# WangWen-Believer/DR-SLAM

Hardware: AMD Instinct MI355X
Metric: RGB-D frames/sec (extract+match) at 640x480 (higher is better)
Workload: dtype u8; 1 GPU; 640x480 synthetic RGB-D (TUM3 intrinsics), ORB extract 1000/1.2/8/20/7 + SearchByProjection(frame k, frame k-1, th=15) on consecutive frames; BASELINE config 2; batch_per_gpu=512, batches_in_flight_per_gpu=3, distinct_resident_input_batches_per_gpu=3, sequence_frames_per_rank=64

## Files before the change

dr_slam_amd/csrc/capi_match.cpp:

```cpp
#include "drfe_internal.h"
#include "match_internal.h"
#include "stage_layout.h"
#include "../../include/drfe_math.h"

#include <algorithm>
#include <cmath>
#include <cstdlib>
#include <cstring>
#include <new>
#include <thread>

template <class T>
static hipError_t dalloc(T** p, size_t n)
{
    *p = nullptr;
    return hipMalloc((void**)p, std::max<size_t>(n, 1) * sizeof(T));
}

void drfe_match_buffers_free(drfe_ctx* c)
{
    MatchBuffers* m = c->mb;
    if (!m) return;
    void* ptrs[] = {m->d_pairs, m->d_queries, m->d_mps, m->d_scale, m->d_candIdx, m->d_candKey, m->d_candCnt, m->d_candBest,
                    m->d_hist, m->d_initObs, m->d_bfIdx, m->d_bfDist, m->d_bfQ, m->d_bfT};
// ... 62 lines not shown
{
    std::memcpy(P->T, Tcw, 64);
    for (int i = 0; i < 3; i++) {
        double s = 0;
        for (int k = 0; k < 3; k++) s += (double)Tcw[k * 4 + i] * (double)Tcw[k * 4 + 3];
        P->Ow[i] = (float)(s * -1.0);
    }
    P->bf = cam->bf;
    P->logScale = drfe_logf(c->cfg.scale_factor);
    P->nLevels = c->cfg.nlevels;
    P->limit = limit;
}

static hipError_t call_scratch(drfe_ctx* c, size_t bytes, uint8_t** out)
{
    if (bytes > c->callScratchBytes) {
        if (c->d_callScratch) (void)hipFree(c->d_callScratch);
        c->d_callScratch = nullptr; c->callScratchBytes = 0;
        const size_t want = (bytes + (bytes >> 1) + 65535) & ~(size_t)65535;
        const hipError_t e = hipMalloc((void**)&c->d_callScratch, want);
        if (e != hipSuccess) return e;
        c->callScratchBytes = want;
    }
    *out = c->d_callScratch;
    return hipSuccess;
}

static void camera_centre_kf(const float* Tcw, float Ow[3])
{
    for (int i = 0; i < 3; i++) {
        const float d = Tcw[0 * 4 + i] * Tcw[3] + Tcw[1 * 4 + i] * Tcw[7] + Tcw[2 * 4 + i] * Tcw[11];
        Ow[i] = (float)((double)d * -1.0);
    }
}

template <class In, class Out, class Launch>
static int frustum_run(drfe_ctx* c, const In* in, int n, Out* out, Launch launch)
{
    if (n == 0) return DRFE_OK;
    HIPCHK(c, hipSetDevice(c->device));
    uint8_t* d = nullptr;
    StageLayout<64> lay;
    const auto sIn = lay.add<In>(n);
    const auto sOut = lay.add<Out>(n);
    HIPCHK(c, call_scratch(c, lay.bytes(), &d));
    hipStream_t s = c->stream;
    hipError_t e = hipMemcpyAsync(sIn.at(d), in, sIn.bytes(), hipMemcpyHostToDevice, s);
    if (e == hipSuccess) e = hipMemcpyAsync(sOut.at(d), out, sOut.bytes(), hipMemcpyHostToDevice, s);
    if (e == hipSuccess) e = launch(sIn.at(d), sOut.at(d), s);
    if (e == hipSuccess) e = hipMemcpyAsync(out, sOut.at(d), sOut.bytes(), hipMemcpyDeviceToHost, s);
    if (e == hipSuccess) e = hipStreamSynchronize(s);
    if (e != hipSuccess) { c->err = std::string("is_in_frustum: ") + hipGetErrorString(e); return DRFE_ERR_HIP; }
    return DRFE_OK;
}


extern "C" {

int drfe_frame_stereo_grid_batch(drfe_ctx* c, const uint16_t* d_depth, size_t frame_stride, size_t row_stride,
                                 const drfe_camera* cam, int nframes, void* stream)
{
    if (!c || !d_depth || !cam) return DRFE_ERR_INVALID;
    if (nframes < 1 || nframes > c->lastBatch) { c->err = "glue: extract the batch first"; return DRFE_ERR_STATE; }
    if (!(cam->max_x > cam->min_x) || !(cam->max_y > cam->min_y)) { c->err = "glue: empty image bounds"; return DRFE_ERR_INVALID; }
    if (row_stride < (size_t)c->geom.imgW || frame_stride < row_stride * (size_t)c->geom.imgH) { c->err = "glue: depth row / frame stride smaller than the image"; return DRFE_ERR_INVALID; }
    HIPCHK(c, hipSetDevice(c->device));
    hipStream_t s = stream ? (hipStream_t)stream : c->stream;
    HIPCHK(c, drfe_launch_glue(c, d_depth, frame_stride, row_stride, *cam, nframes, s));
    c->glueValid = true;
    c->cam = *cam;
    return DRFE_OK;
}

int drfe_frame_set_distortion(drfe_ctx* c, const drfe_camera* cam, const float* dist, int n)
{
    if (!c || (n > 0 && (!dist || !cam)) || n < 0 || n > 5) return DRFE_ERR_INVALID;
    HIPCHK(c, hipSetDevice(c->device));
    int rc = drfe_stream_sync(c);
    if (rc != DRFE_OK) return rc;
    std::memset(&c->dist, 0, sizeof(c->dist));
    c->glueValid = false;
    if (n == 0 || dist[0] == 0.0f) return DRFE_OK;
    if (n < 4) { c->err = "set_distortion: need k1, k2, p1, p2[, k3]"; return DRFE_ERR_INVALID; }
    if (!c->d_kpsUn) {
        void* p = nullptr;
        HIPCHK(c, hipMalloc(&p, sizeof(drfe_keypoint) * (size_t)c->cfg.max_batch * c->maxKp));
        c->d_kpsUn = (drfe_keypoint*)p;
    }
    c->dist.fx = cam->fx; c->dist.fy = cam->fy; c->dist.cx = cam->cx; c->dist.cy = cam->cy;
    for (int i = 0; i < n; i++) c->dist.k[i] = (double)dist[i];
    c->dist.enabled = 1;
    return DRFE_OK;
}

int drfe_frame_image_bounds(const drfe_camera* cam, const float* dist, int n, int cols, int rows, float* bounds)
{
    if (!cam || !bounds || n < 0 || n > 5 || (n > 0 && !dist)) return DRFE_ERR_INVALID;
    if (n >= 4 && dist[0] != 0.0f) {
        DrfeDistortion D;
        std::memset(&D, 0, sizeof(D));
        D.fx = cam->fx; D.fy = cam->fy; D.cx = cam->cx; D.cy = cam->cy; D.enabled = 1;
        for (int i = 0; i < n; i++) D.k[i] = (double)dist[i];
        const float cx[4] = {0.f, (float)cols, 0.f, (float)cols}, cy[4] = {0.f, 0.f, (float)rows, (float)rows};
        float ux[4], uy[4];
        for (int i = 0; i < 4; i++) drfe_undistort_point(D, cx[i], cy[i], &ux[i], &uy[i]);
        bounds[0] = std::min(ux[0], ux[2]); bounds[1] = std::max(ux[1], ux[3]);
        bounds[2] = std::min(uy[0], uy[1]); bounds[3] = std::max(uy[2], uy[3]);
    } else {
        bounds[0] = 0.f; bounds[1] = (float)cols; bounds[2] = 0.f; bounds[3] = (float)rows;
    }
    return DRFE_OK;
}

int drfe_frame_download_keys_un(drfe_ctx* c, int slot, drfe_keypoint* kps, int cap)
{
    if (!c || !kps) return DRFE_ERR_INVALID;
    if (slot < 0 || slot >= c->lastBatch || !c->glueValid) { c->err = "download_keys_un: run the glue first"; return DRFE_ERR_STATE; }
    HIPCHK(c, hipSetDevice(c->device));
    int rc = drfe_stream_sync(c);
    if (rc != DRFE_OK) return rc;
    int n = 0;
    HIPCHK(c, hipMemcpy(&n, c->d_kpCount + slot, sizeof(int), hipMemcpyDeviceToHost));
    if (n > cap) { c->err = "keypoint buffer too small"; return DRFE_ERR_CAPACITY; }
    if (n) HIPCHK(c, hipMemcpy(kps, drfe_kps_un(c) + (size_t)slot * c->maxKp, sizeof(drfe_keypoint) * n, hipMemcpyDeviceToHost));
    return DRFE_OK;
}


int drfe_orb_keypoint_pixels_async(drfe_ctx* c, int nframes, uint32_t* uv, int32_t* counts, void* stream)
{
    if (!c || !uv || !counts) return DRFE_ERR_INVALID;
    if (nframes < 1 || nframes > c->lastBatch) { c->err = "keypoint_pixels: extract the batch first"; return DRFE_ERR_STATE; }
    HIPCHK(c, hipSetDevice(c->device));
    if (!c->d_kpUV) HIPCHK(c, hipMalloc((void**)&c->d_kpUV, sizeof(uint32_t) * (size_t)c->cfg.max_batch * c->maxKp));
    hipStream_t s = stream ? (hipStream_t)stream : c->stream;
    HIPCHK(c, drfe_launch_kp_pixels(c, nframes, c->d_kpUV, s));
    HIPCHK(c, hipMemcpyAsync(uv, c->d_kpUV, sizeof(uint32_t) * (size_t)nframes * c->maxKp, hipMemcpyDeviceToHost, s));
    HIPCHK(c, hipMemcpyAsync(counts, c->d_kpCount, sizeof(int) * (size_t)nframes, hipMemcpyDeviceToHost, s));
    return DRFE_OK;
}

int drfe_gather_keypoint_depth(const uint16_t* depth, size_t frame_stride, size_t row_stride, int nframes, const uint32_t* uv,
                               const int32_t* counts, int max_kp, uint16_t* out, int n_threads)
{
    if (!depth || !uv || !counts || !out || nframes < 0 || max_kp < 1) return DRFE_ERR_INVALID;
    int T = n_threads > 0 ? n_threads : drfe_default_host_threads();
    T = std::max(1, std::min(T, nframes));
    auto work = [&](int f0, int f1) {
        for (int f = f0; f < f1; f++) {
            const uint16_t* img = depth + (size_t)f * frame_stride;
            const uint32_t* p = uv + (size_t)f * max_kp;
            uint16_t* o = out + (size_t)f * max_kp;
            const int n = std::min(counts[f], max_kp);
            const int ahead = 16;
            for (int i = 0; i < std::min(ahead, n); i++)
                if (p[i] != 0xFFFFFFFFu) __builtin_prefetch(&img[(size_t)(p[i] >> 16) * row_stride + (p[i] & 0xFFFFu)]);
            for (int i = 0; i < n; i++) {
                if (i + ahead < n && p[i + ahead] != 0xFFFFFFFFu)
                    __builtin_prefetch(&img[(size_t)(p[i + ahead] >> 16) * row_stride + (p[i + ahead] & 0xFFFFu)]);
                o[i] = p[i] == 0xFFFFFFFFu ? (uint16_t)0 : img[(size_t)(p[i] >> 16) * row_stride + (p[i] & 0xFFFFu)];
            }
        }
    };
    if (T == 1) { work(0, nframes); return DRFE_OK; }
    std::vector<std::thread> th;
    for (int k = 0; k < T; k++) th.emplace_back(work, (int)((int64_t)nframes * k / T), (int)((int64_t)nframes * (k + 1) / T));
    for (std::thread& t : th) t.join();
    return DRFE_OK;
}

int drfe_frame_stereo_grid_batch_kpdepth(drfe_ctx* c, const uint16_t* kp_depth, int kp_depth_on_host, const drfe_camera* cam,
                                         int nframes, void* stream)
{
    if (!c || !kp_depth || !cam) return DRFE_ERR_INVALID;
    if (nframes < 1 || nframes > c->lastBatch) { c->err = "glue: extract the batch first"; return DRFE_ERR_STATE; }
    if (!(cam->max_x > cam->min_x) || !(cam->max_y > cam->min_y)) { c->err = "glue: empty image bounds"; return DRFE_ERR_INVALID; }
    HIPCHK(c, hipSetDevice(c->device));
    hipStream_t s = stream ? (hipStream_t)stream : c->stream;
    const uint16_t* d = kp_depth;
    if (kp_depth_on_host) {
        if (!c->d_kpDepth) HIPCHK(c, hipMalloc((void**)&c->d_kpDepth, sizeof(uint16_t) * (size_t)c->cfg.max_batch * c->maxKp));
        HIPCHK(c, hipMemcpyAsync(c->d_kpDepth, kp_depth, sizeof(uint16_t) * (size_t)nframes * c->maxKp, hipMemcpyHostToDevice, s));
        d = c->d_kpDepth;
    }
    HIPCHK(c, drfe_launch_glue(c, d, (size_t)c->maxKp, 0, *cam, nframes, s));
    c->glueValid = true;
    c->cam = *cam;
    return DRFE_OK;
}

int drfe_frame_load(drfe_ctx* c, int slot, const drfe_keypoint* kps, const drfe_keypoint* kps_un, const uint8_t* desc, const float* u_right,
                    const float* depth_m, int n, const drfe_camera* cam)
{
    if (!c) return DRFE_ERR_INVALID;
    if (slot < 0 || slot >= c->cfg.max_batch || n < 0 || n > c->maxKp || !cam || (n > 0 && (!kps || !desc))) {
        c->err = "drfe_frame_load: invalid argument (slot, keypoint count beyond drfe_orb_max_keypoints, or a missing array)";
        return DRFE_ERR_INVALID;
    }
    if (!(cam->max_x > cam->min_x) || !(cam->max_y > cam->min_y)) { c->err = "drfe_frame_load: empty image bounds"; return DRFE_ERR_INVALID; }
    HIPCHK(c, hipSetDevice(c->device));
    int rc = drfe_stream_sync(c);
    if (rc != DRFE_OK) return rc;
    const size_t K = (size_t)c->maxKp, o = (size_t)slot * K;
    hipStream_t s = c->stream;
    if (n > 0) {
        if (c->dist.enabled) {
            HIPCHK(c, hipMemcpyAsync(c->d_kps + o, kps, sizeof(drfe_keypoint) * (size_t)n, hipMemcpyHostToDevice, s));
            HIPCHK(c, hipMemcpyAsync(c->d_kpsUn + o, kps_un ? kps_un : kps, sizeof(drfe_keypoint) * (size_t)n, hipMemcpyHostToDevice, s));
        } else
            HIPCHK(c, hipMemcpyAsync(c->d_kps + o, kps_un ? kps_un : kps, sizeof(drfe_keypoint) * (size_t)n, hipMemcpyHostToDevice, s));
        HIPCHK(c, hipMemcpyAsync(c->d_desc + o * 32, desc, (size_t)n * 32, hipMemcpyHostToDevice, s));
        if (u_right) HIPCHK(c, hipMemcpyAsync(c->d_uRight + o, u_right, (size_t)n * 4, hipMemcpyHostToDevice, s));
        else HIPCHK(c, drfe_launch_fill_i32(reinterpret_cast<int*>(c->d_uRight + o), n, (int)0xBF800000u , s));
        if (depth_m) HIPCHK(c, hipMemcpyAsync(c->d_depth + o, depth_m, (size_t)n * 4, hipMemcpyHostToDevice, s));
        else HIPCHK(c, drfe_launch_fill_i32(reinterpret_cast<int*>(c->d_depth + o), n, (int)0xBF800000u, s));
    }
    HIPCHK(c, hipMemcpyAsync(c->d_kpCount + slot, &n, sizeof(int), hipMemcpyHostToDevice, s));
    {
        SlotShift shift(c, slot);
        HIPCHK(c, drfe_launch_grid(c, *cam, 1, s));
    }
    HIPCHK(c, hipStreamSynchronize(s));
    c->lastBatch = std::max(c->lastBatch, slot + 1);
    c->glueValid = true;
    c->cam = *cam;
    if (c->bow) drfe_bow_slot_invalidate(c, slot);
    return DRFE_OK;
}

int drfe_frame_download_stereo(drfe_ctx* c, int slot, float* u_right, float* depth, int cap)
{
    if (!c || slot < 0 || slot >= c->lastBatch || !c->glueValid) return c ? DRFE_ERR_STATE : DRFE_ERR_INVALID;
    int rc = drfe_stream_sync(c);
    if (rc != DRFE_OK) return rc;
    int n = 0;
    HIPCHK(c, hipMemcpy(&n, c->d_kpCount + slot, sizeof(int), hipMemcpyDeviceToHost));
    if (n > cap) return DRFE_ERR_CAPACITY;
    if (n && u_right) HIPCHK(c, hipMemcpy(u_right, c->d_uRight + (size_t)slot * c->maxKp, sizeof(float) * n, hipMemcpyDeviceToHost));
    if (n && depth) HIPCHK(c, hipMemcpy(depth, c->d_depth + (size_t)slot * c->maxKp, sizeof(float) * n, hipMemcpyDeviceToHost));
    return DRFE_OK;
}

int drfe_frame_download_grid(drfe_ctx* c, int slot, int32_t* offsets, int32_t* indices, int cap)
{
    if (!c || !offsets || slot < 0 || slot >= c->lastBatch || !c->glueValid) return c ? DRFE_ERR_STATE : DRFE_ERR_INVALID;
    int rc = drfe_stream_sync(c);
    if (rc != DRFE_OK) return rc;
    HIPCHK(c, hipMemcpy(offsets, c->d_gridOff + (size_t)slot * (DRFE_GRID_CELLS + 1), sizeof(int) * (DRFE_GRID_CELLS + 1),
                        hipMemcpyDeviceToHost));
    const int n = offsets[DRFE_GRID_CELLS];
    if (n > cap) return DRFE_ERR_CAPACITY;
    if (n && indices) HIPCHK(c, hipMemcpy(indices, c->d_gridIdx + (size_t)slot * c->maxKp, sizeof(int) * n, hipMemcpyDeviceToHost));
    return DRFE_OK;
}

}

int drfe_match_consecutive_stage(drfe_ctx* c, const float* Tcw, const float* Twc, const drfe_camera* cam, int mono, int nframes, hipStream_t s)
{
    MatchBuffers* m = drfe_match_buffers(c);
    if (!m) return DRFE_ERR_HIP;
    const int np = nframes - 1;
    const size_t pairBytes = sizeof(MatchPair) * (size_t)c->cfg.max_batch, poseBytes = sizeof(float) * 16 * (size_t)c->cfg.max_batch;
    if (!m->h_stage[0]) {
        m->stageBytes = pairBytes + poseBytes;
        for (int k = 0; k < 2; k++) {
            HIPCHK(c, hipHostMalloc(&m->h_stage[k], m->stageBytes, hipHostMallocDefault));
            HIPCHK(c, hipEventCreateWithFlags(&m->stageEv[k], hipEventDisableTiming));
            HIPCHK(c, hipEventRecord(m->stageEv[k], s));
        }
    }
    const int slotK = m->stageNext;
    m->stageNext ^= 1;
    HIPCHK(c, hipEventSynchronize(m->stageEv[slotK]));
    MatchPair* pairs = static_cast<MatchPair*>(m->h_stage[slotK]);
    float* poses = reinterpret_cast<float*>(static_cast<uint8_t*>(m->h_stage[slotK]) + pairBytes);
    std::memcpy(poses, Twc, sizeof(float) * 16 * (size_t)nframes);
    const float mb = cam->bf / cam->fx;
    for (int p = 0; p < np; p++) {
        MatchPair& P = pairs[p];
        P.curSlot = p + 1; P.lastSlot = p; P.mpSlot = p; P.nQueries = 0;
        P.queryBase = p * c->maxKp;
        P.mpBase = p * c->maxKp;
        std::memcpy(P.Tcw, Tcw + (size_t)(p + 1) * 16, sizeof(float) * 16);
        drfe_motion_flags(Tcw + (size_t)(p + 1) * 16, Tcw + (size_t)p * 16, mb, mono, &P.forward, &P.backward);
    }
    HIPCHK(c, hipMemcpyAsync(m->d_pairs, pairs, sizeof(MatchPair) * np, hipMemcpyHostToDevice, s));
    HIPCHK(c, hipMemcpyAsync(c->d_poses, poses, sizeof(float) * 16 * nframes, hipMemcpyHostToDevice, s));
    HIPCHK(c, hipEventRecord(m->stageEv[slotK], s));
    return DRFE_OK;
}

hipError_t drfe_match_consecutive_enqueue(drfe_ctx* c, const drfe_camera* cam, float th, int check_ori, int nframes, hipStream_t s)
{
    MatchBuffers* m = drfe_match_buffers(c);
    if (!m) return hipErrorOutOfMemory;
    hipError_t e = hipMemsetAsync(c->d_match, 0xFF, sizeof(int) * (size_t)nframes * c->maxKp, s);
    if (e == hipSuccess) e = hipMemsetAsync(c->d_matchCount, 0, sizeof(int) * nframes, s);
    if (e == hipSuccess) e = drfe_launch_mappoints_last(c, *m, *cam, c->d_poses, nframes, s);
    if (e == hipSuccess) e = drfe_launch_window_match(c, *m, *cam, nframes - 1, c->maxKp, 0, th, 0.f, check_ori, nullptr, s, 2);
    return e;
}

extern "C" {

int drfe_match_consecutive_batch(drfe_ctx* c, const float* Tcw, const float* Twc, const drfe_camera* cam, float th,
                                 int mono, int check_ori, int nframes, void* stream)
{
    if (!c || !Tcw || !Twc || !cam) return DRFE_ERR_INVALID;
    if (nframes < 2 || nframes > c->lastBatch || !c->glueValid) {
        c->err = "match: needs an extracted batch of >= 2 frames with stereo/grid computed";
        return DRFE_ERR_STATE;
    }
    if (c->maxKp > DRFE_MATCH_LAST_MAX_QUERIES) {
        c->err = "match: the slot size (drfe_orb_max_keypoints = " + std::to_string(c->maxKp) +
                 ") exceeds the 4096 map points the consecutive matcher resolves per pair";
        return DRFE_ERR_CAPACITY;
    }
    HIPCHK(c, hipSetDevice(c->device));
    hipStream_t s = stream ? (hipStream_t)stream : c->stream;
    const int rc = drfe_match_consecutive_stage(c, Tcw, Twc, cam, mono, nframes, s);
    if (rc != DRFE_OK) return rc;
    if (c->profile) { (void)hipEventRecord(c->ev[DRFE_STAGE_MATCH][0], s); c->evUsed[DRFE_STAGE_MATCH] = true; }
    HIPCHK(c, drfe_match_consecutive_enqueue(c, cam, th, check_ori, nframes, s));
    if (c->profile) (void)hipEventRecord(c->ev[DRFE_STAGE_MATCH][1], s);
    return DRFE_OK;
}

int drfe_match_download(drfe_ctx* c, int slot, int32_t* cur_to_last, int cap, int* nmatches)
{
    if (!c || slot < 0 || slot >= c->lastBatch) return c ? DRFE_ERR_STATE : DRFE_ERR_INVALID;
    int rc = drfe_stream_sync(c);
    if (rc != DRFE_OK) return rc;
    rc = match_status(c, 2);
    if (rc != DRFE_OK) return rc;
    int n = 0;
    HIPCHK(c, hipMemcpy(&n, c->d_kpCount + slot, sizeof(int), hipMemcpyDeviceToHost));
    if (n > cap) return DRFE_ERR_CAPACITY;
    if (n && cur_to_last)
        HIPCHK(c, hipMemcpy(cur_to_last, c->d_match + (size_t)slot * c->maxKp, sizeof(int) * n, hipMemcpyDeviceToHost));
    if (nmatches) HIPCHK(c, hipMemcpy(nmatches, c->d_matchCount + slot, sizeof(int), hipMemcpyDeviceToHost));
    return DRFE_OK;
}

int drfe_search_by_projection_last(drfe_ctx* c, int cur_slot, int last_slot, const float* Tcw_cur, const float* Tcw_last,
                                   const drfe_camera* cam, const drfe_map_point* last_mp, int n_last, float th, int mono,
                                   int check_ori, const uint8_t* cur_obs, int32_t* cur_mp, int n_cur, int* nmatches)
{
    if (!c || !Tcw_cur || !Tcw_last || !cam || !last_mp || !cur_mp || !nmatches) return DRFE_ERR_INVALID;
    if (cur_slot < 0 || cur_slot >= c->lastBatch || last_slot < 0 || last_slot >= c->lastBatch || !c->glueValid) {
        c->err = "search_by_projection_last: slots not ready";
        return DRFE_ERR_STATE;
    }
    HIPCHK(c, hipSetDevice(c->device));
    int rc = drfe_stream_sync(c);
    if (rc != DRFE_OK) return rc;
    int counts[2];
    HIPCHK(c, hipMemcpy(&counts[0], c->d_kpCount + cur_slot, sizeof(int), hipMemcpyDeviceToHost));
    HIPCHK(c, hipMemcpy(&counts[1], c->d_kpCount + last_slot, sizeof(int), hipMemcpyDeviceToHost));
    if (n_cur != counts[0] || n_last != counts[1]) { c->err = "search_by_projection_last: N mismatch"; return DRFE_ERR_INVALID; }
    if (n_last > DRFE_MATCH_LAST_MAX_QUERIES) {
        c->err = "search_by_projection_last: more than 4096 map points in the last frame";
        return DRFE_ERR_CAPACITY;
    }
    MatchBuffers* m = drfe_match_buffers(c);
    if (!m) return DRFE_ERR_HIP;
    MatchPair P;
    P.curSlot = cur_slot; P.lastSlot = last_slot; P.mpSlot = -1; P.nQueries = n_last; P.queryBase = 0; P.mpBase = 0;
    std::memcpy(P.Tcw, Tcw_cur, sizeof(float) * 16);
    drfe_motion_flags(Tcw_cur, Tcw_last, cam->bf / cam->fx, mono, &P.forward, &P.backward);
    hipStream_t s = c->stream;
    HIPCHK(c, hipMemcpy(m->d_pairs, &P, sizeof(P), hipMemcpyHostToDevice));
    if (n_last) HIPCHK(c, hipMemcpy(m->d_mps, last_mp, sizeof(drfe_map_point) * n_last, hipMemcpyHostToDevice));
    if (n_cur) HIPCHK(c, hipMemcpy(c->d_match + (size_t)cur_slot * c->maxKp, cur_mp, sizeof(int) * n_cur, hipMemcpyHostToDevice));
    const uint8_t* d_obs = nullptr;
    if (cur_obs && n_cur) {
        HIPCHK(c, hipMemcpy(m->d_initObs, cur_obs, n_cur, hipMemcpyHostToDevice));
        d_obs = m->d_initObs;
    }
    *nmatches = 0;
    if (n_last == 0 || n_cur == 0) return DRFE_OK;
    HIPCHK(c, drfe_launch_window_match(c, *m, *cam, 1, n_last, 0, th, 0.f, check_ori, d_obs, s));
    HIPCHK(c, hipStreamSynchronize(s));
    rc = match_status(c);
    if (rc != DRFE_OK) return rc;
    HIPCHK(c, hipMemcpy(cur_mp, c->d_match + (size_t)cur_slot * c->maxKp, sizeof(int) * n_cur, hipMemcpyDeviceToHost));
    HIPCHK(c, hipMemcpy(nmatches, c->d_matchCount + cur_slot, sizeof(int), hipMemcpyDeviceToHost));
    return DRFE_OK;
}

int drfe_search_by_projection_map(drfe_ctx* c, int slot, const drfe_tracked_point* mps, int mcount, float th,
                                  float nnratio, const uint8_t* claim_obs, int32_t* frame_mp, int n, int* nmatches)
{
    if (!c || !mps || !frame_mp || !nmatches || mcount < 0) return DRFE_ERR_INVALID;
    if (slot < 0 || slot >= c->lastBatch || !c->glueValid) { c->err = "search_by_projection_map: slot not ready"; return DRFE_ERR_STATE; }
    HIPCHK(c, hipSetDevice(c->device));
    int rc = drfe_stream_sync(c);
    if (rc != DRFE_OK) return rc;
    int cnt = 0;
    HIPCHK(c, hipMemcpy(&cnt, c->d_kpCount + slot, sizeof(int), hipMemcpyDeviceToHost));
    if (n != cnt) { c->err = "search_by_projection_map: N mismatch"; return DRFE_ERR_INVALID; }
    MatchBuffers* m = drfe_match_buffers(c);
    if (!m) return DRFE_ERR_HIP;
    if ((size_t)mcount > m->queryCap) { c->err = "search_by_projection_map: too many map points for the scratch"; return DRFE_ERR_CAPACITY; }
    *nmatches = 0;
    if (mcount == 0 || n == 0) return DRFE_OK;
    std::vector<MatchQuery> q(mcount);
    const bool bFactor = th != 1.0;
    for (int i = 0; i < mcount; i++) {
        const drfe_tracked_point& t = mps[i];
        MatchQuery& Q = q[i];
        std::memset(&Q, 0, sizeof(Q));
        Q.valid = (t.track_in_view && !t.bad) ? 1 : 0;
        if (Q.valid && (t.level < 0 || t.level >= c->cfg.nlevels)) { c->err = "tracked point level out of range"; return DRFE_ERR_INVALID; }
        float r = ((double)t.view_cos > 0.998) ? 2.5f : 4.0f;
        if (bFactor) r *= th;
        const float rs = Q.valid ? r * c->scale[t.level] : 0.f;
        Q.u = t.proj_x; Q.v = t.proj_y; Q.radius = rs; Q.ur = t.proj_xr; Q.thrR = rs;
        Q.minLevel = t.level - 1; Q.maxLevel = t.level;
        Q.obs = t.obs_positive;
        std::memcpy(Q.desc, t.desc, 32);
    }
    MatchPair P;
    std::memset(&P, 0, sizeof(P));
    P.curSlot = slot; P.lastSlot = slot; P.mpSlot = -1; P.nQueries = mcount; P.queryBase = 0; P.mpBase = 0;
    const drfe_camera cam = c->cam;
    hipStream_t s = c->stream;
    HIPCHK(c, hipMemcpy(m->d_pairs, &P, sizeof(P), hipMemcpyHostToDevice));
    HIPCHK(c, hipMemcpy(m->d_queries, q.data(), sizeof(MatchQuery) * mcount, hipMemcpyHostToDevice));
    HIPCHK(c, hipMemcpy(c->d_match + (size_t)slot * c->maxKp, frame_mp, sizeof(int) * n, hipMemcpyHostToDevice));
    const uint8_t* d_obs = nullptr;
    if (claim_obs) {
        HIPCHK(c, hipMemcpy(m->d_initObs, claim_obs, n, hipMemcpyHostToDevice));
        d_obs = m->d_initObs;
    }
    HIPCHK(c, drfe_launch_window_match(c, *m, cam, 1, mcount, 1, th, nnratio, 0, d_obs, s));
    HIPCHK(c, hipStreamSynchronize(s));
    rc = match_status(c);
    if (rc != DRFE_OK) return rc;
    HIPCHK(c, hipMemcpy(frame_mp, c->d_match + (size_t)slot * c->maxKp, sizeof(int) * n, hipMemcpyDeviceToHost));
    HIPCHK(c, hipMemcpy(nmatches, c->d_matchCount + slot, sizeof(int), hipMemcpyDeviceToHost));
    return DRFE_OK;
}

int drfe_match_orb_points(drfe_ctx* c, int cur_slot, int last_slot, const int32_t* last_mp, const uint8_t* last_outlier,
                          int n_last, int32_t* cur_mp, int n_cur, int* n_pairs)
{
    if (!c || !last_mp || !last_outlier || !cur_mp || !n_pairs) return DRFE_ERR_INVALID;
    if (cur_slot < 0 || cur_slot >= c->lastBatch || last_slot < 0 || last_slot >= c->lastBatch) {
        c->err = "match_orb_points: slots not ready";
        return DRFE_ERR_STATE;
    }
    HIPCHK(c, hipSetDevice(c->device));
    int rc = drfe_stream_sync(c);
    if (rc != DRFE_OK) return rc;
    int counts[2];
    HIPCHK(c, hipMemcpy(&counts[0], c->d_kpCount + cur_slot, sizeof(int), hipMemcpyDeviceToHost));
    HIPCHK(c, hipMemcpy(&counts[1], c->d_kpCount + last_slot, sizeof(int), hipMemcpyDeviceToHost));
    if (n_cur != counts[0] || n_last != counts[1]) { c->err = "match_orb_points: N mismatch"; return DRFE_ERR_INVALID; }
    *n_pairs = 0;
    if (n_cur == 0 || n_last == 0) return DRFE_OK;
    MatchBuffers* m = drfe_match_buffers(c);
    if (!m) return DRFE_ERR_HIP;
    hipStream_t s = c->stream;
    HIPCHK(c, drfe_launch_bf_knn(c->d_desc + (size_t)cur_slot * c->maxKp * 32, n_cur,
                                 c->d_desc + (size_t)last_slot * c->maxKp * 32, n_last, 1, m->d_bfIdx, m->d_bfDist, s));
    std::vector<int32_t> idx(n_cur), dist(n_cur);
    HIPCHK(c, hipMemcpyAsync(idx.data(), m->d_bfIdx, sizeof(int) * n_cur, hipMemcpyDeviceToHost, s));
    HIPCHK(c, hipMemcpyAsync(dist.data(), m->d_bfDist, sizeof(int) * n_cur, hipMemcpyDeviceToHost, s));
    HIPCHK(c, hipStreamSynchronize(s));
    double min_dist = 1000;
    for (int i = 0; i < n_cur; i++)
        if ((float)dist[i] < min_dist) min_dist = (float)dist[i];
    int npair = 0;
    for (int i = 0; i < n_cur; i++) {
        if (!((float)dist[i] < std::max(2 * min_dist, 15.0))) continue;
        const int mp = last_mp[idx[i]];
        if (mp >= 0 && npair < n_last && !last_outlier[npair]) cur_mp[i] = mp;
        npair++;
    }
    *n_pairs = npair;
    return DRFE_OK;
}

static void line_mad(const int32_t* dist, int nq, double* nnMad, double* nn12Mad)
{
    std::vector<float> d0(nq), gap(nq), s(nq);
    for (int i = 0; i < nq; i++) { d0[i] = (float)dist[2 * i]; gap[i] = (float)dist[2 * i + 1] - (float)dist[2 * i]; }
    s = d0;
    std::nth_element(s.begin(), s.begin() + nq / 2, s.end());
    const double med = s[nq / 2];
    for (int i = 0; i < nq; i++) s[i] = std::fabs((float)(d0[i] - med));
    std::nth_element(s.begin(), s.begin() + nq / 2, s.end());
    *nnMad = 1.4826 * s[nq / 2];
    s = gap;
    std::nth_element(s.begin(), s.begin() + nq / 2, s.end(), [](float a, float b) { return a > b; });
    const double med12 = s[nq / 2];
    for (int i = 0; i < nq; i++) s[i] = std::fabs((float)(gap[i] - med12));
    std::nth_element(s.begin(), s.begin() + nq / 2, s.end());
    *nn12Mad = 1.4826 * s[nq / 2];
}

int drfe_lsd_search_by_descriptor(drfe_ctx* c, const uint8_t* desc_q, int n_q, const uint8_t* desc_t, int n_t,
                                  const uint8_t* has_line, int mode, int32_t* out, int* nmatches)
{
    if (!c || !desc_q || !desc_t || !out || !nmatches || n_q < 0 || n_t < 0 || mode < 0 || mode > 1) return DRFE_ERR_INVALID;
    *nmatches = 0;
    const int n_out = mode == 0 ? n_t : n_q;
    for (int i = 0; i < n_out; i++) out[i] = -1;
    if (n_q == 0 || n_t < 2) return DRFE_OK;
    std::vector<int32_t> idx((size_t)n_q * 2), dist((size_t)n_q * 2);
    int rc = drfe_match_bf_knn(c, desc_q, n_q, desc_t, n_t, 2, idx.data(), dist.data());
    if (rc != DRFE_OK) return rc;
    double nnTh, nn12Th;
    line_mad(dist.data(), n_q, &nnTh, &nn12Th);
    int n = 0;
    if (mode == 0) {
        const float minRatio = 1.0f / 1.5f;
        for (int q = 0; q < n_q; q++) {
            const double r = (float)dist[2 * q] / (float)dist[2 * q + 1];
            if (r < minRatio && (!has_line || has_line[q])) { out[idx[2 * q]] = q; n++; }
        }
    } else {
        const double th = nn12Th * 0.5;
        for (int q = 0; q < n_q; q++) {
            const double gap = (float)dist[2 * q + 1] - (float)dist[2 * q];
            if (gap > th && (!has_line || has_line[idx[2 * q]])) { out[q] = idx[2 * q]; n++; }
        }
    }
    *nmatches = n;
    return DRFE_OK;
}

int drfe_lsd_search_for_triangulation(drfe_ctx* c, const uint8_t* desc1, int n1, const uint8_t* desc2, int n2,
                                      const uint8_t* has1, const uint8_t* has2, int32_t* out12, int* nmatches)
{
    if (!c || !desc1 || !desc2 || !has1 || !has2 || !out12 || !nmatches || n1 < 0 || n2 < 0) return DRFE_ERR_INVALID;
    *nmatches = 0;
    for (int i = 0; i < n1; i++) out12[i] = -1;
    if (n1 == 0 || n2 < 2) return DRFE_OK;
    std::vector<int32_t> idx((size_t)n1 * 2), dist((size_t)n1 * 2);
    int rc = drfe_match_bf_knn(c, desc1, n1, desc2, n2, 2, idx.data(), dist.data());
    if (rc != DRFE_OK) return rc;
    double nnTh, nn12Th;
    line_mad(dist.data(), n1, &nnTh, &nn12Th);
    const double th = nn12Th * 0.1;
    int n = 0;
    for (int q = 0; q < n1; q++) {
        const int t = idx[2 * q];
        if (has1[q] || has2[t]) continue;
        const double gap = (float)dist[2 * q + 1] - (float)dist[2 * q];
        if (gap > th) { out12[q] = t; n++; }
    }
    *nmatches = n;
    return DRFE_OK;
}

int drfe_match_bf_knn(drfe_ctx* c, const uint8_t* q, int nq, const uint8_t* t, int nt, int k, int32_t* idx, int32_t* dist)
{
    if (!c || !q || !t || !idx || !dist || nq < 0 || nt < 0 || k < 1 || k > 2) return DRFE_ERR_INVALID;
    if (nq == 0) return DRFE_OK;
    HIPCHK(c, hipSetDevice(c->device));
    MatchBuffers* m = drfe_match_buffers(c);
    if (!m) return DRFE_ERR_HIP;
    if ((size_t)nq > m->bfCap || (size_t)nt > m->bfCap) { c->err = "bf_knn: descriptor set larger than the scratch"; return DRFE_ERR_CAPACITY; }
    hipStream_t s = c->stream;
    HIPCHK(c, hipMemcpyAsync(m->d_bfQ, q, (size_t)nq * 32, hipMemcpyHostToDevice, s));
    if (nt) HIPCHK(c, hipMemcpyAsync(m->d_bfT, t, (size_t)nt * 32, hipMemcpyHostToDevice, s));
    HIPCHK(c, drfe_launch_bf_knn(m->d_bfQ, nq, m->d_bfT, nt, k, m->d_bfIdx, m->d_bfDist, s));
    HIPCHK(c, hipMemcpyAsync(idx, m->d_bfIdx, sizeof(int) * (size_t)nq * k, hipMemcpyDeviceToHost, s));
    HIPCHK(c, hipMemcpyAsync(dist, m->d_bfDist, sizeof(int) * (size_t)nq * k, hipMemcpyDeviceToHost, s));
    HIPCHK(c, hipStreamSynchronize(s));
    return DRFE_OK;
}



static int line_search_run(drfe_ctx* c, const std::vector<LineQuery>* hostQ, const drfe_map_line* last, int n,
                           const float* TcwCur, const drfe_camera* cam, int fwd, int bwd, float th,
                           const drfe_keyline* cur_lines, const uint8_t* cur_desc, int n_cur, float nnratio,
                           const uint8_t* cur_obs, int32_t* cur_ml, int* nmatches)
{
    *nmatches = 0;
    if (n == 0 || n_cur == 0) return DRFE_OK;
    if (n_cur > 4096 || n > 65536) { c->err = "lsd_search_by_projection: too many lines"; return DRFE_ERR_CAPACITY; }
    HIPCHK(c, hipSetDevice(c->device));
    MatchBuffers* m = drfe_match_buffers(c);
    if (!m) return DRFE_ERR_HIP;
    std::vector<LineCur> lc(n_cur);
    std::vector<uint8_t> claim(n_cur);
    for (int i = 0; i < n_cur; i++) {
        lc[i].ptX = cur_lines[i].pt_x; lc[i].ptY = cur_lines[i].pt_y; lc[i].angle = cur_lines[i].angle;
        lc[i].octave = cur_lines[i].octave;
        claim[i] = cur_ml[i] >= 0 ? (uint8_t)(1 | ((cur_obs ? cur_obs[i] : 1) ? 2 : 0)) : 0;
    }
    StageLayout<64> lay;
    const auto sQ = lay.add<LineQuery>(n);
    const auto sL = lay.add<drfe_map_line>(hostQ ? 0 : n);
    const auto sT = lay.add<float>(hostQ ? 0 : 16);
    const auto sC = lay.add<LineCur>(n_cur);
    const auto sD = lay.add<uint8_t>((size_t)n_cur * 32), sK = lay.add<uint8_t>(n_cur);
    const auto sM = lay.add<int>(n_cur), sN = lay.add<int>(1);
    uint8_t* d = nullptr;
    HIPCHK(c, call_scratch(c, lay.bytes(), &d));
    hipStream_t s = c->stream;
    hipError_t e = hipSuccess;
    auto up = [&](const auto& sec, const void* src) { if (e == hipSuccess && sec.n) e = hipMemcpyAsync(sec.at(d), src, sec.bytes(), hipMemcpyHostToDevice, s); };
    if (hostQ) up(sQ, hostQ->data());
    up(sL, last);
    up(sT, TcwCur);
    up(sC, lc.data());
    up(sD, cur_desc);
    up(sK, claim.data());
    up(sM, cur_ml);
    if (e == hipSuccess && !hostQ)
        e = drfe_launch_line_projection(sL.at(d), n, sT.at(d), *cam, fwd, bwd, m->d_scale, th, sQ.at(d), s);
    if (e == hipSuccess)
        e = drfe_launch_line_search(sQ.at(d), n, sC.at(d), sD.at(d), n_cur, nnratio, sK.at(d), sM.at(d), sN.at(d), s);
    if (e == hipSuccess) e = hipMemcpyAsync(cur_ml, sM.at(d), sM.bytes(), hipMemcpyDeviceToHost, s);
    if (e == hipSuccess) e = hipMemcpyAsync(nmatches, sN.at(d), sN.bytes(), hipMemcpyDeviceToHost, s);
    if (e == hipSuccess) e = hipStreamSynchronize(s);
    if (e != hipSuccess) { c->err = std::string("lsd_search_by_projection: ") + hipGetErrorString(e); return DRFE_ERR_HIP; }
    return DRFE_OK;
}

int drfe_lsd_search_by_projection_last(drfe_ctx* c, const float* Tcw_cur, const float* Tcw_last, const drfe_camera* cam,
                                       const drfe_map_line* last_lines, int n_last, const drfe_keyline* cur_lines,
                                       const uint8_t* cur_desc, int n_cur, float th, int mono, float nnratio,
                                       const uint8_t* cur_obs, int32_t* cur_ml, int* nmatches)
// ... 579 lines not shown
```

dr_slam_amd/csrc/capi_pipeline.cpp:

```cpp
#include "drfe_internal.h"

#include <new>
#include <vector>

struct drfe_pipeline {
    std::vector<drfe_ctx*> ctx;
    unsigned long long submitted = 0;
    std::string err;
};

extern "C" {

int drfe_pipeline_create(const drfe_config* cfg, int depth, drfe_pipeline** out)
{
    if (!cfg || !out || depth < 1 || depth > 16) return DRFE_ERR_INVALID;
    *out = nullptr;
    drfe_pipeline* p = new (std::nothrow) drfe_pipeline();
    if (!p) return DRFE_ERR_INVALID;
    for (int k = 0; k < depth; k++) {
        drfe_ctx* c = nullptr;
        const int rc = drfe_create(cfg, &c);
        if (rc != DRFE_OK) {
            for (drfe_ctx* d : p->ctx) drfe_destroy(d);
            delete p;
            return rc;
        }
        p->ctx.push_back(c);
    }
    *out = p;
    return DRFE_OK;
}

void drfe_pipeline_destroy(drfe_pipeline* p)
{
    if (!p) return;
    for (drfe_ctx* c : p->ctx) drfe_destroy(c);
    delete p;
}

int drfe_pipeline_depth(const drfe_pipeline* p) { return p ? (int)p->ctx.size() : 0; }

drfe_ctx* drfe_pipeline_context(drfe_pipeline* p, int k)
{
    return (p && k >= 0 && k < (int)p->ctx.size()) ? p->ctx[(size_t)k] : nullptr;
}

const char* drfe_pipeline_last_error(const drfe_pipeline* p) { return p ? p->err.c_str() : ""; }

int drfe_pipeline_submit(drfe_pipeline* p, const uint8_t* d_gray, const uint16_t* d_depth, size_t frame_stride, size_t row_stride,
                         int w, int h, const float* Tcw, const float* Twc, const drfe_camera* cam, float th, int mono, int check_ori,
                         int nframes)
{
    if (!p || !d_gray || p->ctx.empty()) return DRFE_ERR_INVALID;
    const int k = (int)(p->submitted % p->ctx.size());
    drfe_ctx* c = p->ctx[(size_t)k];
    int rc = drfe_orb_extract_batch(c, d_gray, frame_stride, row_stride, w, h, nframes, nullptr);
    if (rc == DRFE_OK && d_depth) {
        if (!cam) { p->err = "drfe_pipeline_submit: a depth batch needs the camera"; return DRFE_ERR_INVALID; }
        rc = drfe_frame_stereo_grid_batch(c, d_depth, frame_stride, row_stride, cam, nframes, nullptr);
        if (rc == DRFE_OK && Tcw && Twc && nframes >= 2)
            rc = drfe_match_consecutive_batch(c, Tcw, Twc, cam, th, mono, check_ori, nframes, nullptr);
    }
    if (rc != DRFE_OK) { p->err = drfe_last_error(c); return rc; }
    p->submitted++;
    return k;
}

int drfe_pipeline_sync(drfe_pipeline* p, int k)
{
    if (!p || k >= (int)p->ctx.size()) return DRFE_ERR_INVALID;
    for (int i = 0; i < (int)p->ctx.size(); i++) {
        if (k >= 0 && i != k) continue;
        drfe_ctx* c = p->ctx[(size_t)i];
        if (hipSetDevice(c->device) != hipSuccess || hipStreamSynchronize(c->stream) != hipSuccess) {
            p->err = "drfe_pipeline_sync: stream synchronisation failed";
            return DRFE_ERR_HIP;
        }
        const int rc = drfe_batch_check(c);
        if (rc != DRFE_OK) { p->err = drfe_last_error(c); return rc; }
    }
    return DRFE_OK;
}

}
```

dr_slam_amd/csrc/match_internal.h:

```cpp
#ifndef DRFE_MATCH_INTERNAL_H
#define DRFE_MATCH_INTERNAL_H
#include "drfe_internal.h"

#define DRFE_MATCH_LAST_MAX_QUERIES 4096

struct MatchPair {
    int curSlot, lastSlot;
    int mpSlot;
    int nQueries;
    int queryBase;
    int mpBase;
    int forward, backward;
    float Tcw[16];
};

struct MatchQuery {
    float u, v, radius;
    float ur, thrR;
    int minLevel, maxLevel;
    int valid;
    int obs;
    uint32_t desc[8];
};

struct MatchBuffers {
    MatchPair* d_pairs = nullptr;
    MatchQuery* d_queries = nullptr;
    drfe_map_point* d_mps = nullptr;
    float* d_scale = nullptr;
    uint32_t* d_candIdx = nullptr;
    uint32_t* d_candKey = nullptr;
    int* d_candCnt = nullptr;
    uint2* d_candBest = nullptr;
    uint16_t* d_hist = nullptr;
    uint8_t* d_initObs = nullptr;
    int32_t* d_bfIdx = nullptr; int32_t* d_bfDist = nullptr; uint8_t* d_bfQ = nullptr; uint8_t* d_bfT = nullptr; size_t bfCap = 0;
    size_t queryCap = 0;
    void* h_stage[2] = {nullptr, nullptr}; hipEvent_t stageEv[2] = {nullptr, nullptr}; size_t stageBytes = 0; int stageNext = 0;
};

hipError_t drfe_launch_window_match(drfe_ctx* c, const MatchBuffers& mb, const drfe_camera& cam, int npairs,
                                    int maxQueries, int mode, float th, float nnratio, int checkOri,
                                    const uint8_t* d_initObs, hipStream_t s, int statusWord = 1);
hipError_t drfe_launch_fill_i32(int* d_p, int n, int v, hipStream_t s);
hipError_t drfe_launch_fill_i32_and_word(int* d_p, int n, int v, int* d_q, int w, hipStream_t s);
struct DrfePackArgs { const uint32_t* src[10]; uint32_t dwords[10]; int n; };
hipError_t drfe_launch_pack_segments(const DrfePackArgs& A, uint32_t* d_dst, hipStream_t s);
void drfe_motion_flags(const float* TcwCur, const float* TcwLast, float mb, int mono, int* fwd, int* bwd);
hipError_t drfe_launch_window_candidates(drfe_ctx* c, const MatchBuffers& mb, const drfe_camera& cam, int npairs, int maxQueries,
                                         hipStream_t s);
hipError_t drfe_launch_mappoints_last(drfe_ctx* c, const MatchBuffers& mb, const drfe_camera& cam, const float* d_Twc,
                                      int nframes, hipStream_t s);
hipError_t drfe_launch_bf_knn(const uint8_t* dQ, int nq, const uint8_t* dT, int nt, int k, int* dIdx, int* dDist,
                              hipStream_t s);

struct LineQuery {
    int valid, obs;
    int minLevel, maxLevel;
    float x1, y1, x2, y2, r;
    uint32_t desc[8];
};
struct LineCur { float ptX, ptY, angle; int octave; };

hipError_t drfe_launch_line_projection(const drfe_map_line* d_lines, int n, const float* d_TcwCur, const drfe_camera& cam,
                                       int forward, int backward, const float* d_scale, float th, LineQuery* d_q,
                                       hipStream_t s);
hipError_t drfe_launch_line_search(const LineQuery* d_q, int n, const LineCur* d_cur, const uint8_t* d_desc, int nCur,
                                   float nnratio, uint8_t* d_claim, int* d_curMl, int* d_nmatches, hipStream_t s);

struct FrustumPose { float T[16]; float Ow[3]; float bf; float logScale; int nLevels; float limit; };
hipError_t drfe_launch_frustum_points(const drfe_frustum_point* d_pts, int n, const FrustumPose& P, const drfe_camera& cam,
                                      drfe_tracked_point* d_out, hipStream_t s);
hipError_t drfe_launch_frustum_lines(const drfe_frustum_line* d_lines, int n, const FrustumPose& P, const drfe_camera& cam,
                                     drfe_tracked_line* d_out, hipStream_t s);

struct LineSim3 { float sR[9], t[3]; };
hipError_t drfe_launch_line_fuse_search(const drfe_frustum_line* d_lines, const uint8_t* d_descs, const uint8_t* d_skip, int n,
                                        const FrustumPose& P, const drfe_camera& cam, const float* d_scale, float th,
                                        const LineCur* d_kf, const uint8_t* d_kfDesc, int nKF, int* d_bestIdx, int* d_bestDist,
                                        hipStream_t s, const LineSim3* sim3 = nullptr, int* d_distRow = nullptr);

struct FuseParams { float T[16]; float Ow[3]; float bf, logScale, th; int nLevels; float scale[16], invSigma2[16];
                    int sim3;
                    float sR2[9], t2[3];
                    int listTh; };
#define FUSE_LIST_K 8
hipError_t drfe_launch_fuse_search(drfe_ctx* c, int slot, const drfe_frustum_point* d_pts, const uint8_t* d_descs,
                                   const uint8_t* d_skip, int n, const FuseParams& P, const drfe_camera& cam, int* d_bestIdx,
                                   int* d_bestDist, hipStream_t s, const uint8_t* d_taken = nullptr, int2* d_list = nullptr,
                                   int* d_listCount = nullptr);

MatchBuffers* drfe_match_buffers(drfe_ctx* c);
int drfe_match_consecutive_stage(drfe_ctx* c, const float* Tcw, const float* Twc, const drfe_camera* cam, int mono, int nframes, hipStream_t s);
hipError_t drfe_match_consecutive_enqueue(drfe_ctx* c, const drfe_camera* cam, float th, int check_ori, int nframes, hipStream_t s);
void drfe_match_buffers_free(drfe_ctx* c);
#endif
```

dr_slam_amd/csrc/match_kernels.hip:

```cpp
#include "drfe_internal.h"
#include "match_internal.h"
#include "../../include/drfe_math.h"

#define WAVE 64


__global__ __launch_bounds__(256) void k_undistort(const drfe_keypoint* __restrict__ kps, const int* __restrict__ kpCount,
                                                   int maxKp, DrfeDistortion D, drfe_keypoint* __restrict__ kpsUn)
{
    const int slot = blockIdx.y;
    const int i = blockIdx.x * 256 + threadIdx.x;
    if (i >= kpCount[slot]) return;
    drfe_keypoint kp = kps[(size_t)slot * maxKp + i];
    float ux, uy;
    drfe_undistort_point(D, kp.x, kp.y, &ux, &uy);
    kp.x = ux; kp.y = uy;
    kpsUn[(size_t)slot * maxKp + i] = kp;
}

__global__ __launch_bounds__(256) void k_stereo(const drfe_keypoint* __restrict__ kps, const drfe_keypoint* __restrict__ kpsUn,
                                                const int* __restrict__ kpCount,
                                                int maxKp, const uint16_t* __restrict__ depth, size_t frameStride,
                                                size_t rowStride, int w, int h, drfe_camera cam,
                                                float* __restrict__ uRight, float* __restrict__ zDepth)
{
    const int slot = blockIdx.y;
    const int i = blockIdx.x * 256 + threadIdx.x;
    if (i >= kpCount[slot]) return;
    const drfe_keypoint kp = kps[(size_t)slot * maxKp + i];
    const int v = (int)kp.y, u = (int)kp.x;
    float d = 0.f;
    if (u >= 0 && u < w && v >= 0 && v < h)
        d = (float)depth[rowStride ? (size_t)slot * frameStride + (size_t)v * rowStride + u : (size_t)slot * frameStride + i] * cam.depth_factor;
    float ur = -1.f, z = -1.f;
    if (d > 0) { z = d; ur = kpsUn[(size_t)slot * maxKp + i].x - cam.bf / d; }
    uRight[(size_t)slot * maxKp + i] = ur;
    zDepth[(size_t)slot * maxKp + i] = z;
}

__device__ __forceinline__ int grid_cell(const drfe_keypoint& kp, const drfe_camera& cam, float invW, float invH)
{
    const int px = (int)roundf((kp.x - cam.min_x) * invW);
    const int py = (int)roundf((kp.y - cam.min_y) * invH);
    if (px < 0 || px >= DRFE_GRID_COLS || py < 0 || py >= DRFE_GRID_ROWS) return -1;
    return px * DRFE_GRID_ROWS + py;
}

__global__ __launch_bounds__(256) void k_grid(const drfe_keypoint* __restrict__ kps, const int* __restrict__ kpCount,
                                              int maxKp, drfe_camera cam, float invW, float invH,
                                              const float* __restrict__ uRight, const uint8_t* __restrict__ desc,
                                              int* __restrict__ gridOff, int* __restrict__ gridIdx,
                                              uint4* __restrict__ cellKp, uint4* __restrict__ cellDesc)
{
    __shared__ int cnt[DRFE_GRID_CELLS];
    __shared__ int off[DRFE_GRID_CELLS + 1];
    __shared__ int part[256];
    const int slot = blockIdx.x, tid = threadIdx.x;
    const int n = kpCount[slot];
    const drfe_keypoint* K = kps + (size_t)slot * maxKp;
    int* gIdx = gridIdx + (size_t)slot * maxKp;
    int* gOff = gridOff + (size_t)slot * (DRFE_GRID_CELLS + 1);
    for (int c = tid; c < DRFE_GRID_CELLS; c += 256) cnt[c] = 0;
    __syncthreads();
    for (int i = tid; i < n; i += 256) {
        const int c = grid_cell(K[i], cam, invW, invH);
        if (c >= 0) atomicAdd(&cnt[c], 1);
    }
    __syncthreads();
    const int per = DRFE_GRID_CELLS / 256;
    int s = 0;
    for (int k = 0; k < per; k++) s += cnt[tid * per + k];
    part[tid] = s;
    __syncthreads();
    for (int o = 1; o < 256; o <<= 1) {
        const int v = (tid >= o) ? part[tid - o] : 0;
        __syncthreads();
        part[tid] += v;
        __syncthreads();
    }
    int run = part[tid] - s;
    for (int k = 0; k < per; k++) { off[tid * per + k] = run; run += cnt[tid * per + k]; }
    if (tid == 255) off[DRFE_GRID_CELLS] = run;
    __syncthreads();
    for (int c = tid; c <= DRFE_GRID_CELLS; c += 256) gOff[c] = off[c];
    for (int c = tid; c < DRFE_GRID_CELLS; c += 256) cnt[c] = 0;
    __syncthreads();
    for (int i = tid; i < n; i += 256) {
        const int c = grid_cell(K[i], cam, invW, invH);
        if (c >= 0) gIdx[off[c] + atomicAdd(&cnt[c], 1)] = i;
    }
    __syncthreads();
    for (int c = tid; c < DRFE_GRID_CELLS; c += 256) {
        const int b = off[c], e = off[c + 1];
        for (int a = b + 1; a < e; a++) {
            const int v = gIdx[a];
            int j = a - 1;
            while (j >= b && gIdx[j] > v) { gIdx[j + 1] = gIdx[j]; j--; }
            gIdx[j + 1] = v;
        }
    }
    __syncthreads();
    const int nIn = off[DRFE_GRID_CELLS];
    uint4* cK = cellKp + (size_t)slot * maxKp;
    uint4* cD = cellDesc + (size_t)slot * maxKp * 2;
    const uint4* D4 = reinterpret_cast<const uint4*>(desc + (size_t)slot * maxKp * 32);
    const float* UR = uRight + (size_t)slot * maxKp;
    for (int p = tid; p < nIn; p += 256) {
        const int idx = gIdx[p];
        const drfe_keypoint kp = K[idx];
        cK[p] = make_uint4(__float_as_uint(kp.x), __float_as_uint(kp.y), __float_as_uint(UR[idx]),
                           (uint32_t)idx | ((uint32_t)kp.octave << 24));
        cD[2 * p] = D4[2 * idx];
        cD[2 * p + 1] = D4[2 * idx + 1];
    }
}


__device__ __forceinline__ void mat3_mul_add(const float* T , const float x[3], float out[3])
{
#pragma unroll
    for (int r = 0; r < 3; r++) {
        const float d = T[r * 4 + 0] * x[0] + T[r * 4 + 1] * x[1] + T[r * 4 + 2] * x[2];
        out[r] = d + T[r * 4 + 3];
    }
}

__global__ __launch_bounds__(256) void k_mappoints_last(const drfe_keypoint* __restrict__ kps,
                                                        const uint8_t* __restrict__ desc,
                                                        const int* __restrict__ kpCount, int maxKp,
                                                        const float* __restrict__ zDepth, drfe_camera cam,
                                                        const float* __restrict__ Twc ,
                                                        drfe_map_point* __restrict__ mps)
{
    const int slot = blockIdx.y;
    const int i = blockIdx.x * 256 + threadIdx.x;
    if (i >= kpCount[slot]) return;
    const size_t o = (size_t)slot * maxKp + i;
    drfe_map_point mp;
    const float z = zDepth[o];
    mp.valid = z > 0 ? 1 : 0;
    mp.obs_positive = 1;
    mp.pad[0] = mp.pad[1] = 0;
    mp.world[0] = mp.world[1] = mp.world[2] = 0.f;
    if (z > 0) {
        const float invfx = 1.0f / cam.fx, invfy = 1.0f / cam.fy;
        const drfe_keypoint kp = kps[o];
        float p[3];
        p[0] = (kp.x - cam.cx) * z * invfx;
        p[1] = (kp.y - cam.cy) * z * invfy;
        p[2] = z;
        mat3_mul_add(Twc + (size_t)slot * 16, p, mp.world);
    }
    const uint32_t* d = reinterpret_cast<const uint32_t*>(desc + o * 32);
    uint32_t* md = reinterpret_cast<uint32_t*>(mp.desc);
#pragma unroll
    for (int k = 0; k < 8; k++) md[k] = d[k];
    mps[o] = mp;
}

__global__ __launch_bounds__(256) void k_queries_last(const MatchPair* __restrict__ pairs,
                                                      const drfe_keypoint* __restrict__ kps,
                                                      const int* __restrict__ kpCount, int maxKp,
                                                      const drfe_map_point* __restrict__ mps, drfe_camera cam,
                                                      const float* __restrict__ scaleFactors, float th,
                                                      MatchQuery* __restrict__ queries)
{
    const MatchPair P = pairs[blockIdx.y];
    const int i = blockIdx.x * 256 + threadIdx.x;
    const int nLast = P.mpSlot >= 0 ? kpCount[P.lastSlot] : P.nQueries;
    if (i >= nLast) return;
    MatchQuery q;
    q.valid = 0;
    q.u = q.v = q.radius = q.ur = q.thrR = 0.f;
    q.minLevel = q.maxLevel = -1;
    q.obs = 0;
    const drfe_map_point mp = mps[(size_t)P.mpBase + i];
#pragma unroll
    for (int k = 0; k < 8; k++) q.desc[k] = reinterpret_cast<const uint32_t*>(mp.desc)[k];
    q.obs = mp.obs_positive;
    if (mp.valid) {
        float xc[3];
        mat3_mul_add(P.Tcw, mp.world, xc);
        const float invzc = (float)(1.0 / (double)xc[2]);
        if (!(invzc < 0)) {
            const float u = cam.fx * xc[0] * invzc + cam.cx;
            const float v = cam.fy * xc[1] * invzc + cam.cy;
            if (!(u < cam.min_x || u > cam.max_x) && !(v < cam.min_y || v > cam.max_y)) {
                const int oct = kps[(size_t)P.lastSlot * maxKp + i].octave;
                const float radius = th * scaleFactors[oct];
                q.u = u; q.v = v; q.radius = radius; q.thrR = radius;
                q.ur = u - cam.bf * invzc;
                if (P.forward) { q.minLevel = oct; q.maxLevel = -1; }
                else if (P.backward) { q.minLevel = 0; q.maxLevel = oct; }
                else { q.minLevel = oct - 1; q.maxLevel = oct + 1; }
                q.valid = 1;
            }
        }
    }
    queries[(size_t)P.queryBase + i] = q;
}


__device__ __forceinline__ bool window_cells(const MatchQuery& q, const drfe_camera& cam, float invW, float invH, int& minX,
                                             int& maxX, int& minY, int& maxY)
{
    const float x = q.u, y = q.v, r = q.radius;
    minX = max(0, (int)floorf((x - cam.min_x - r) * invW));
    maxX = min(DRFE_GRID_COLS - 1, (int)ceilf((x - cam.min_x + r) * invW));
    minY = max(0, (int)floorf((y - cam.min_y - r) * invH));
    maxY = min(DRFE_GRID_ROWS - 1, (int)ceilf((y - cam.min_y + r) * invH));
    return !(minX >= DRFE_GRID_COLS || maxX < 0 || minY >= DRFE_GRID_ROWS || maxY < 0);
}

__device__ __forceinline__ bool window_candidate(const MatchQuery& q, bool bCheckLevels, const uint4* __restrict__ cK,
                                                 const uint4* __restrict__ cD, int p, int sq, uint64_t q0, uint64_t q1,
                                                 uint64_t q2, uint64_t q3, uint32_t& key, uint32_t& id)
{
    const uint4 k4 = cK[p];
    const uint4 da = cD[2 * p], db = cD[2 * p + 1];
    const float kx = __uint_as_float(k4.x), ky = __uint_as_float(k4.y), ur = __uint_as_float(k4.z);
    const int oct = (int)(k4.w >> 24);
    bool ok = true;
    if (bCheckLevels) {
        if (oct < q.minLevel) ok = false;
        if (q.maxLevel >= 0 && oct > q.maxLevel) ok = false;
    }
    const float dx = kx - q.u, dy = ky - q.v;
    if (!(fabsf(dx) < q.radius && fabsf(dy) < q.radius)) ok = false;
    if (ur > 0) {
        const float er = fabsf(q.ur - ur);
        if (er > q.thrR) ok = false;
    }
    if (!ok) return false;
    const int dist = __popcll(q0 ^ ((uint64_t)da.x | ((uint64_t)da.y << 32))) + __popcll(q1 ^ ((uint64_t)da.z | ((uint64_t)da.w << 32))) +
                     __popcll(q2 ^ ((uint64_t)db.x | ((uint64_t)db.y << 32))) + __popcll(q3 ^ ((uint64_t)db.z | ((uint64_t)db.w << 32)));
    key = ((uint32_t)dist << 22) | (uint32_t)min(sq, (1 << 22) - 1);
    id = k4.w;
    return true;
}

__device__ void window_query_wave(const MatchQuery& q, size_t qo, int lane, int nMinCellX, int nMaxCellX, int nMinCellY, int nMaxCellY,
                                  const int* __restrict__ gOff, const uint4* __restrict__ cK, const uint4* __restrict__ cD,
                                  uint32_t* __restrict__ candIdx, uint32_t* __restrict__ candKey, int* __restrict__ candCnt,
                                  uint2* __restrict__ candBest, int* __restrict__ status)
{
    const bool bCheckLevels = (q.minLevel > 0) || (q.maxLevel >= 0);
    uint32_t* oIdx = candIdx + qo * DRFE_MATCH_MAX_CAND;
    uint32_t* oKey = candKey + qo * DRFE_MATCH_MAX_CAND;
    const uint64_t q0 = (uint64_t)q.desc[0] | ((uint64_t)q.desc[1] << 32), q1 = (uint64_t)q.desc[2] | ((uint64_t)q.desc[3] << 32),
                   q2 = (uint64_t)q.desc[4] | ((uint64_t)q.desc[5] << 32), q3 = (uint64_t)q.desc[6] | ((uint64_t)q.desc[7] << 32);
    const int ncol = nMaxCellX - nMinCellX + 1;
    int runB = 0, runN = 0;
    if (lane < ncol) {
        const int cb = (nMinCellX + lane) * DRFE_GRID_ROWS;
        runB = gOff[cb + nMinCellY];
        runN = gOff[cb + nMaxCellY + 1] - runB;
    }
    const int incl = drfe_wave_incl_scan(runN, lane);
    const int T = __builtin_amdgcn_readlane(incl, 63);
    int nOut = 0;
    bool overflow = false;
    uint32_t myKey = 0xFFFFFFFFu, myIdx = 0;
    for (int s0 = 0; s0 < T; s0 += WAVE) {
        const int sq = s0 + lane;
        bool pass = false;
        uint32_t key = 0xFFFFFFFFu, id = 0;
        int base = __builtin_amdgcn_readfirstlane(runB);
        for (int j = 0; j + 1 < ncol; j++) {
            const int inclJ = __builtin_amdgcn_readlane(incl, j), nextB = __builtin_amdgcn_readlane(runB, j + 1);
            if (inclJ <= sq) base = nextB - inclJ;
        }
        if (sq < T) pass = window_candidate(q, bCheckLevels, cK, cD, base + sq, sq, q0, q1, q2, q3, key, id);
        const unsigned long long m = __ballot(pass);
        const int pos = nOut + __popcll(m & ((1ull << lane) - 1ull));
        if (pass) {
            if (pos < DRFE_MATCH_MAX_CAND) {
                oIdx[pos] = id;
                oKey[pos] = key;
                if (key < myKey) { myKey = key; myIdx = id; }
            } else overflow = true;
        }
        nOut += __popcll(m);
    }
    if (__any(overflow) && lane == 0) atomicOr(status, 4);
    const uint32_t mn = drfe_wave_min_u32(myKey);
    const unsigned long long who = __ballot(myKey == mn);
    const uint32_t bIdx = (uint32_t)__builtin_amdgcn_readlane((int)myIdx, __ffsll((long long)who) - 1);
    if (lane == 0) {
        candCnt[qo] = min(nOut, DRFE_MATCH_MAX_CAND);
        candBest[qo] = make_uint2(mn, bIdx);
    }
}

#define WQ_TAB 64
#ifndef WQ_THREADS
#define WQ_THREADS 64
#endif
#define WQ_PER_BLOCK (WQ_THREADS / WAVE * 4)
__global__ __launch_bounds__(WQ_THREADS) void k_window_candidates(const MatchPair* __restrict__ pairs,
                                                           const MatchQuery* __restrict__ queries,
                                                           const int* __restrict__ kpCount, int maxKp,
                                                           const int* __restrict__ gridOff,
                                                           const uint4* __restrict__ cellKp,
                                                           const uint4* __restrict__ cellDesc, drfe_camera cam,
                                                           float invW, float invH,
                                                           uint32_t* __restrict__ candIdx,
                                                           uint32_t* __restrict__ candKey,
                                                           int* __restrict__ candCnt, uint2* __restrict__ candBest,
                                                           int* __restrict__ status, uint32_t gxMagic)
{
    __shared__ int sTab[WQ_THREADS / WAVE][4][WQ_TAB];
    int bx, by;
    drfe_xcd_swizzle_2d(gxMagic, bx, by);
    const MatchPair P = pairs[by];
    const int wv = __builtin_amdgcn_readfirstlane((int)(threadIdx.x >> 6)), lane = threadIdx.x & 63;
    const int g = lane >> 4, l = lane & 15;
    const int qbase = (bx * (WQ_THREADS / WAVE) + wv) * 4;
    const int nQ = P.mpSlot >= 0 ? kpCount[P.lastSlot] : P.nQueries;
    if (qbase >= nQ) return;
    const int cur = P.curSlot;
    const int* gOff = gridOff + (size_t)cur * (DRFE_GRID_CELLS + 1);
    const uint4* cK = cellKp + (size_t)cur * maxKp;
    const uint4* cD = cellDesc + (size_t)cur * maxKp * 2;
    const bool have = qbase + g < nQ;
    const size_t qo = (size_t)P.queryBase + (have ? qbase + g : qbase);
    const MatchQuery q = queries[qo];
    int nMinCellX = 0, nMaxCellX = 0, nMinCellY = 0, nMaxCellY = 0;
    const bool inRange = have && q.valid && window_cells(q, cam, invW, invH, nMinCellX, nMaxCellX, nMinCellY, nMaxCellY);
    const int ncol = nMaxCellX - nMinCellX + 1;
    int runB = 0, runN = 0;
    const bool narrow = inRange && ncol <= 16;
    if (narrow && l < ncol) {
        const int cb = (nMinCellX + l) * DRFE_GRID_ROWS;
        runB = gOff[cb + nMinCellY];
        runN = gOff[cb + nMaxCellY + 1] - runB;
    }
    int incl = runN;
    incl += __builtin_amdgcn_update_dpp(0, incl, 0x111, 0xf, 0xf, true);
    incl += __builtin_amdgcn_update_dpp(0, incl, 0x112, 0xf, 0xf, true);
    incl += __builtin_amdgcn_update_dpp(0, incl, 0x114, 0xf, 0xf, true);
    incl += __builtin_amdgcn_update_dpp(0, incl, 0x118, 0xf, 0xf, true);
    const int T = __shfl(incl, 15, 16);
    const bool small = narrow && T <= WQ_TAB;
    {
        const int excl = incl - runN;
        const int n = small ? runN : 0;
        for (int k = 0; __any(k < n); k++)
            if (k < n) sTab[wv][g][excl + k] = runB + k;
    }
    const bool bCheckLevels = (q.minLevel > 0) || (q.maxLevel >= 0);
    const uint64_t q0 = (uint64_t)q.desc[0] | ((uint64_t)q.desc[1] << 32), q1 = (uint64_t)q.desc[2] | ((uint64_t)q.desc[3] << 32),
                   q2 = (uint64_t)q.desc[4] | ((uint64_t)q.desc[5] << 32), q3 = (uint64_t)q.desc[6] | ((uint64_t)q.desc[7] << 32);
    uint32_t* oIdx = candIdx + qo * DRFE_MATCH_MAX_CAND;
    uint32_t* oKey = candKey + qo * DRFE_MATCH_MAX_CAND;
    const int Tg = small ? T : 0;
    int nOut = 0;
    uint32_t myKey = 0xFFFFFFFFu, myIdx = 0;
    for (int s0 = 0; __any(s0 < Tg); s0 += 16) {
        const int sq = s0 + l;
        bool pass = false;
        uint32_t key = 0xFFFFFFFFu, id = 0;
        if (sq < Tg) pass = window_candidate(q, bCheckLevels, cK, cD, sTab[wv][g][sq], sq, q0, q1, q2, q3, key, id);
        const uint32_t m16 = (uint32_t)(__ballot(pass) >> (g * 16)) & 0xFFFFu;
        const int pos = nOut + __popc(m16 & ((1u << l) - 1u));
        if (pass) {
            oIdx[pos] = id;
            oKey[pos] = key;
            if (key < myKey) { myKey = key; myIdx = id; }
        }
        nOut += __popc(m16);
    }
    uint32_t mn = myKey;
    mn = min(mn, (uint32_t)__builtin_amdgcn_update_dpp((int)mn, (int)mn, 0xB1, 0xf, 0xf, false));
    mn = min(mn, (uint32_t)__builtin_amdgcn_update_dpp((int)mn, (int)mn, 0x4E, 0xf, 0xf, false));
    mn = min(mn, (uint32_t)__builtin_amdgcn_update_dpp((int)mn, (int)mn, 0x141, 0xf, 0xf, false));
    mn = min(mn, (uint32_t)__builtin_amdgcn_update_dpp((int)mn, (int)mn, 0x140, 0xf, 0xf, false));
    const uint32_t who16 = (uint32_t)(__ballot(myKey == mn) >> (g * 16)) & 0xFFFFu;
    const uint32_t bIdx = (uint32_t)__shfl((int)myIdx, __ffs((int)who16) - 1, 16);
    if (have && l == 0 && (small || !inRange)) {
        candCnt[qo] = nOut;
        candBest[qo] = small ? make_uint2(mn, bIdx) : make_uint2(0xFFFFFFFFu, 0u);
    }
    unsigned long long wide = __ballot(inRange && !small && l == 0);
    while (wide) {
        const int gg = (__ffsll((long long)wide) - 1) >> 4;
        wide &= wide - 1;
        const size_t qw = (size_t)P.queryBase + qbase + gg;
        const MatchQuery qq = queries[qw];
        int x0, x1, y0, y1;
        window_cells(qq, cam, invW, invH, x0, x1, y0, y1);
        window_query_wave(qq, qw, lane, x0, x1, y0, y1, gOff, cK, cD, candIdx, candKey, candCnt, candBest, status);
    }
}


__device__ __forceinline__ uint32_t wave_min_u32(uint32_t v) { return drfe_wave_min_u32(v); }

#define RS_THREADS 512
#define RS_MAX_T 8
static_assert(RS_THREADS * RS_MAX_T == DRFE_MATCH_LAST_MAX_QUERIES, "the C-ABI checks this limit before launching");
__global__ __launch_bounds__(RS_THREADS) void k_resolve_last(const MatchPair* __restrict__ pairs,
                                                             const MatchQuery* __restrict__ queries,
                                                             const drfe_keypoint* __restrict__ kps,
                                                             const int* __restrict__ kpCount, int maxKp,
                                                             const uint32_t* __restrict__ candIdx,
                                                             const uint32_t* __restrict__ candKey,
                                                             const int* __restrict__ candCnt,
                                                             const uint2* __restrict__ candBest, int checkOri,
                                                             int* __restrict__ match ,
                                                             const uint8_t* __restrict__ initObs,
                                                             int* __restrict__ matchCount,
                                                             uint16_t* __restrict__ histScratch )
{
    extern __shared__ int rs_smem[];
    int* owner = rs_smem;
    unsigned char* claim = reinterpret_cast<unsigned char*>(rs_smem + maxKp);
    __shared__ int hist[30];
    __shared__ int sNm, sEnt, sInd[3], sChanged[3];
    const MatchPair P = pairs[blockIdx.x];
    const int tid = threadIdx.x;
    const int nQ = P.mpSlot >= 0 ? kpCount[P.lastSlot] : P.nQueries;
    const int nCur = kpCount[P.curSlot];
    int* M = match + (size_t)P.curSlot * maxKp;
    const drfe_keypoint* Kc = kps + (size_t)P.curSlot * maxKp;
    const drfe_keypoint* Kl = kps + (size_t)P.lastSlot * maxKp;
    uint16_t* hs = histScratch + (size_t)blockIdx.x * 2 * maxKp;
    for (int i = tid; i < nCur; i += RS_THREADS) {
        unsigned char c = 0;
        if (M[i] >= 0) c = 1 | ((initObs ? initObs[i] : 1) ? 2 : 0);
        claim[i] = c;
    }
    if (tid < 30) hist[tid] = 0;
    if (tid == 0) { sNm = 0; sEnt = 0; sChanged[0] = 0; }
    const float factor = 1.0f / 30;
    int cnt[RS_MAX_T], obs[RS_MAX_T];
    uint32_t bKey[RS_MAX_T], bIdx[RS_MAX_T], pKey[RS_MAX_T], pIdx[RS_MAX_T];
#pragma unroll
    for (int t = 0; t < RS_MAX_T; t++) {
        const int i = tid + t * RS_THREADS;
        cnt[t] = 0; obs[t] = 0; bKey[t] = 0xFFFFFFFFu; bIdx[t] = 0; pKey[t] = 0xFFFFFFFFu; pIdx[t] = 0;
        if (i < nQ) {
            const size_t qo = (size_t)P.queryBase + i;
            cnt[t] = candCnt[qo];
            if (cnt[t] > 0) { const uint2 b = candBest[qo]; bKey[t] = b.x; bIdx[t] = b.y; obs[t] = queries[qo].obs; }
        }
    }
    for (int sweep = 0;; sweep++) {
        for (int k = tid; k < nCur; k += RS_THREADS) owner[k] = 0x7FFFFFFF;
        if (tid == 0) sChanged[(sweep + 1) % 3] = 0;
        __syncthreads();
#pragma unroll
        for (int t = 0; t < RS_MAX_T; t++)
            if (obs[t] && pKey[t] != 0xFFFFFFFFu && (int)(pKey[t] >> 22) <= 100)
                atomicMin(&owner[pIdx[t] & 0xFFFFFF], tid + t * RS_THREADS);
        __syncthreads();
        bool changed = false;
#pragma unroll
        for (int t = 0; t < RS_MAX_T; t++) {
            if (cnt[t] == 0) continue;
            const int i = tid + t * RS_THREADS;
            uint32_t key = 0xFFFFFFFFu, idx = 0;
            const int kb = (int)(bIdx[t] & 0xFFFFFF);
            if ((claim[kb] & 3) != 3 && owner[kb] >= i) { key = bKey[t]; idx = bIdx[t]; }
            else {
                const size_t qo = ((size_t)P.queryBase + i) * DRFE_MATCH_MAX_CAND;
                for (int j0 = 0; j0 < cnt[t]; j0 += 8) {
                    const uint4 ka = *reinterpret_cast<const uint4*>(candKey + qo + j0);
                    const uint4 kb2 = *reinterpret_cast<const uint4*>(candKey + qo + j0 + 4);
                    const uint4 ia = *reinterpret_cast<const uint4*>(candIdx + qo + j0);
                    const uint4 ib = *reinterpret_cast<const uint4*>(candIdx + qo + j0 + 4);
                    const uint32_t kv[8] = {ka.x, ka.y, ka.z, ka.w, kb2.x, kb2.y, kb2.z, kb2.w};
                    const uint32_t iv[8] = {ia.x, ia.y, ia.z, ia.w, ib.x, ib.y, ib.z, ib.w};
#pragma unroll
                    for (int u = 0; u < 8; u++) {
                        if (j0 + u >= cnt[t] || kv[u] >= key) continue;
                        const int kk = (int)(iv[u] & 0xFFFFFF);
                        if ((claim[kk] & 3) != 3 && owner[kk] >= i) { key = kv[u]; idx = iv[u]; }
                    }
                }
            }
            if (key != pKey[t] || idx != pIdx[t]) { changed = true; pKey[t] = key; pIdx[t] = idx; }
        }
        if (changed) sChanged[sweep % 3] = 1;
        __syncthreads();
        if (!__builtin_amdgcn_readfirstlane(sChanged[sweep % 3])) break;
    }
    for (int k = tid; k < nCur; k += RS_THREADS) owner[k] = -1;
    __syncthreads();
#pragma unroll
    for (int t = 0; t < RS_MAX_T; t++) {
        if (pKey[t] == 0xFFFFFFFFu || (int)(pKey[t] >> 22) > 100) continue;
        const int i = tid + t * RS_THREADS;
        const int i2 = (int)(pIdx[t] & 0xFFFFFF);
        atomicMax(&owner[i2], i);
        atomicAdd(&sNm, 1);
        if (checkOri) {
            float rot = Kl[i].angle - Kc[i2].angle;
            if (rot < 0.0f) rot += 360.0f;
            int bin = (int)roundf(rot * factor);
            if (bin == 30) bin = 0;
            const int e = atomicAdd(&sEnt, 1);
            hs[2 * e] = (uint16_t)bin;
            hs[2 * e + 1] = (uint16_t)i2;
            atomicAdd(&hist[bin], 1);
        }
    }
    __syncthreads();
    for (int k = tid; k < nCur; k += RS_THREADS)
        if (owner[k] >= 0) M[k] = owner[k];
    __syncthreads();
    if (checkOri) {
        if (tid == 0) {
            int max1 = 0, max2 = 0, max3 = 0, ind1 = -1, ind2 = -1, ind3 = -1;
            for (int i = 0; i < 30; i++) {
                const int s = hist[i];
                if (s > max1) { max3 = max2; max2 = max1; max1 = s; ind3 = ind2; ind2 = ind1; ind1 = i; }
                else if (s > max2) { max3 = max2; max2 = s; ind3 = ind2; ind2 = i; }
                else if (s > max3) { max3 = s; ind3 = i; }
            }
            if (max2 < 0.1f * (float)max1) { ind2 = -1; ind3 = -1; }
            else if (max3 < 0.1f * (float)max1) { ind3 = -1; }
            sInd[0] = ind1; sInd[1] = ind2; sInd[2] = ind3;
        }
        __syncthreads();
        const int nEnt = sEnt;
        for (int e = tid; e < nEnt; e += RS_THREADS) {
            const int bin = hs[2 * e];
            if (bin != sInd[0] && bin != sInd[1] && bin != sInd[2]) { M[hs[2 * e + 1]] = -1; atomicSub(&sNm, 1); }
        }
        __syncthreads();
    }
    if (tid == 0) matchCount[P.curSlot] = sNm;
}

__global__ __launch_bounds__(WAVE) void k_resolve_map(const MatchPair* __restrict__ pairs,
                                                      const MatchQuery* __restrict__ queries,
                                                      const int* __restrict__ kpCount, int maxKp,
                                                      const uint32_t* __restrict__ candIdx,
                                                      const uint32_t* __restrict__ candKey,
                                                      const int* __restrict__ candCnt, float nnratio,
                                                      int* __restrict__ match, const uint8_t* __restrict__ initObs,
                                                      int* __restrict__ matchCount)
{
    extern __shared__ unsigned char claim[];
    const MatchPair P = pairs[blockIdx.x];
    const int lane = threadIdx.x;
    const int nQ = P.nQueries;
    const int nCur = kpCount[P.curSlot];
    int* M = match + (size_t)P.curSlot * maxKp;
    for (int i = lane; i < nCur; i += WAVE) {
        unsigned char c = 0;
        if (M[i] >= 0) c = 1 | ((initObs ? initObs[i] : 1) ? 2 : 0);
        claim[i] = c;
    }
    __syncthreads();
    int nmatches = 0;
    for (int i = 0; i < nQ; i++) {
        const size_t qo = (size_t)P.queryBase + i;
        const int cnt = candCnt[qo];
        if (cnt == 0) continue;
        uint32_t k1 = 0xFFFFFFFFu, i1 = 0, k2 = 0xFFFFFFFFu, i2 = 0;
        for (int c0 = 0; c0 < cnt; c0 += WAVE) {
            uint32_t key = 0xFFFFFFFFu, idx = 0;
            if (c0 + lane < cnt) {
                idx = candIdx[qo * DRFE_MATCH_MAX_CAND + c0 + lane];
                key = candKey[qo * DRFE_MATCH_MAX_CAND + c0 + lane];
                if ((claim[idx & 0xFFFFFF] & 3) == 3) key = 0xFFFFFFFFu;
            }
            for (int pass = 0; pass < 2; pass++) {
                const uint32_t mn = wave_min_u32(key);
                if (mn == 0xFFFFFFFFu) break;
                const unsigned long long who = __ballot(key == mn);
                const int src = __ffsll((long long)who) - 1;
                const uint32_t ix = (uint32_t)__shfl((int)idx, src);
                if (mn < k1) { k2 = k1; i2 = i1; k1 = mn; i1 = ix; }
                else if (mn < k2) { k2 = mn; i2 = ix; }
                if (lane == src) key = 0xFFFFFFFFu;
            }
        }
        if (k1 == 0xFFFFFFFFu) continue;
        const int bestDist = (int)(k1 >> 22);
        const int bestDist2 = (k2 == 0xFFFFFFFFu) ? 256 : (int)(k2 >> 22);
        const int bestLevel = (int)(i1 >> 24);
        const int bestLevel2 = (k2 == 0xFFFFFFFFu) ? -1 : (int)(i2 >> 24);
        if (bestDist <= 100) {
            if (bestLevel == bestLevel2 && (float)bestDist > nnratio * (float)bestDist2) continue;
            const int bi = (int)(i1 & 0xFFFFFF);
            if (lane == 0) { M[bi] = i; claim[bi] = 1 | (queries[qo].obs ? 2 : 0); }
            nmatches++;
            __syncthreads();
        }
    }
    if (lane == 0) matchCount[P.curSlot] = nmatches;
}


__global__ __launch_bounds__(64) void k_bf_knn(const uint8_t* __restrict__ Q, int nq, const uint8_t* __restrict__ T,
                                               int nt, int k, int* __restrict__ outIdx, int* __restrict__ outDist)
{
    __shared__ uint64_t tile[64 * 4];
    const int lane = threadIdx.x;
    const int qi = blockIdx.x * 64 + lane;
    uint64_t q[4] = {0, 0, 0, 0};
    if (qi < nq) {
        const uint64_t* p = reinterpret_cast<const uint64_t*>(Q + (size_t)qi * 32);
        q[0] = p[0]; q[1] = p[1]; q[2] = p[2]; q[3] = p[3];
    }
    int d1 = 1 << 30, i1 = -1, d2 = 1 << 30, i2 = -1;
    for (int t0 = 0; t0 < nt; t0 += 64) {
        __syncthreads();
        if (t0 + lane < nt) {
            const uint64_t* p = reinterpret_cast<const uint64_t*>(T + (size_t)(t0 + lane) * 32);
            tile[lane * 4 + 0] = p[0]; tile[lane * 4 + 1] = p[1]; tile[lane * 4 + 2] = p[2]; tile[lane * 4 + 3] = p[3];
        }
        __syncthreads();
        const int m = min(64, nt - t0);
        for (int j = 0; j < m; j++) {
            const int d = __popcll(q[0] ^ tile[j * 4]) + __popcll(q[1] ^ tile[j * 4 + 1]) +
                          __popcll(q[2] ^ tile[j * 4 + 2]) + __popcll(q[3] ^ tile[j * 4 + 3]);
            if (d < d1) { d2 = d1; i2 = i1; d1 = d; i1 = t0 + j; }
            else if (d < d2) { d2 = d; i2 = t0 + j; }
        }
    }
    if (qi < nq) {
        outIdx[(size_t)qi * k] = i1;
        outDist[(size_t)qi * k] = i1 >= 0 ? d1 : -1;
        if (k > 1) {
            outIdx[(size_t)qi * k + 1] = i2;
            outDist[(size_t)qi * k + 1] = i2 >= 0 ? d2 : -1;
        }
    }
}



__global__ __launch_bounds__(256) void k_kp_pixels(const drfe_keypoint* __restrict__ kps, const int* __restrict__ kpCount, int maxKp,
                                                   int w, int h, uint32_t* __restrict__ uv)
{
    const int slot = blockIdx.y;
    const int i = blockIdx.x * 256 + threadIdx.x;
    if (i >= maxKp) return;
    uint32_t o = 0xFFFFFFFFu;
    if (i < kpCount[slot]) {
        const drfe_keypoint kp = kps[(size_t)slot * maxKp + i];
        const int v = (int)kp.y, u = (int)kp.x;
        if (u >= 0 && u < w && v >= 0 && v < h) o = (uint32_t)u | ((uint32_t)v << 16);
    }
    uv[(size_t)slot * maxKp + i] = o;
}

hipError_t drfe_launch_kp_pixels(drfe_ctx* c, int nframes, uint32_t* d_uv, hipStream_t s)
{
    hipLaunchKernelGGL(k_kp_pixels, dim3((c->maxKp + 255) / 256, nframes), dim3(256), 0, s, c->d_kps, c->d_kpCount, c->maxKp,
                       c->geom.imgW, c->geom.imgH, d_uv);
    return hipGetLastError();
}

hipError_t drfe_launch_glue(drfe_ctx* c, const uint16_t* d_depth, size_t frameStride, size_t rowStride,
                            const drfe_camera& cam, int nframes, hipStream_t s)
{
    const float invW = (float)DRFE_GRID_COLS / (float)(cam.max_x - cam.min_x);
    const float invH = (float)DRFE_GRID_ROWS / (float)(cam.max_y - cam.min_y);
    prof_begin(c, DRFE_STAGE_GLUE, s);
    if (c->dist.enabled)
        hipLaunchKernelGGL(k_undistort, dim3((c->maxKp + 255) / 256, nframes), dim3(256), 0, s, c->d_kps, c->d_kpCount,
                           c->maxKp, c->dist, c->d_kpsUn);
    hipLaunchKernelGGL(k_stereo, dim3((c->maxKp + 255) / 256, nframes), dim3(256), 0, s, c->d_kps, drfe_kps_un(c), c->d_kpCount,
                       c->maxKp, d_depth, frameStride, rowStride, c->geom.imgW, c->geom.imgH, cam, c->d_uRight,
                       c->d_depth);
    hipLaunchKernelGGL(k_grid, dim3(nframes), dim3(256), 0, s, drfe_kps_un(c), c->d_kpCount, c->maxKp, cam, invW, invH,
                       c->d_uRight, c->d_desc, c->d_gridOff, c->d_gridIdx, c->d_cellKp, c->d_cellDesc);
    prof_end(c, DRFE_STAGE_GLUE, s);
    return hipGetLastError();
}

hipError_t drfe_launch_grid(drfe_ctx* c, const drfe_camera& cam, int nframes, hipStream_t s)
{
    const float invW = (float)DRFE_GRID_COLS / (float)(cam.max_x - cam.min_x);
    const float invH = (float)DRFE_GRID_ROWS / (float)(cam.max_y - cam.min_y);
    hipLaunchKernelGGL(k_grid, dim3(nframes), dim3(256), 0, s, drfe_kps_un(c), c->d_kpCount, c->maxKp, cam, invW, invH,
                       c->d_uRight, c->d_desc, c->d_gridOff, c->d_gridIdx, c->d_cellKp, c->d_cellDesc);
    return hipGetLastError();
}

__global__ __launch_bounds__(256) void k_fill_i32(int* __restrict__ p, int n, int v)
{
    const int i = blockIdx.x * 256 + threadIdx.x;
    if (i < n) p[i] = v;
}
hipError_t drfe_launch_fill_i32(int* d_p, int n, int v, hipStream_t s)
{
    if (n <= 0) return hipSuccess;
    hipLaunchKernelGGL(k_fill_i32, dim3((n + 255) / 256), dim3(256), 0, s, d_p, n, v);
    return hipGetLastError();
}

__global__ __launch_bounds__(256) void k_fill_i32_and_word(int* __restrict__ p, int n, int v, int* __restrict__ q, int w)
{
    const int i = blockIdx.x * 256 + threadIdx.x;
    if (i < n) p[i] = v;
    if (i == 0) *q = w;
}
hipError_t drfe_launch_fill_i32_and_word(int* d_p, int n, int v, int* d_q, int w, hipStream_t s)
{
    hipLaunchKernelGGL(k_fill_i32_and_word, dim3((n > 0 ? n + 255 : 256) / 256), dim3(256), 0, s, d_p, n, v, d_q, w);
    return hipGetLastError();
}

__global__ __launch_bounds__(256) void k_pack_segments(DrfePackArgs A, uint32_t* __restrict__ dst)
{
    uint32_t total = 0;
    for (int k = 0; k < A.n; k++) total += A.dwords[k];
    for (uint32_t i = blockIdx.x * 256 + threadIdx.x; i < total; i += gridDim.x * 256) {
        uint32_t base = 0;
        int k = 0;
        while (i - base >= A.dwords[k]) { base += A.dwords[k]; k++; }
        if (A.src[k]) dst[i] = A.src[k][i - base];
    }
}
hipError_t drfe_launch_pack_segments(const DrfePackArgs& A, uint32_t* d_dst, hipStream_t s)
{
    uint32_t total = 0;
    for (int k = 0; k < A.n; k++) total += A.dwords[k];
    if (!total) return hipSuccess;
    const unsigned blocks = (total + 1023) / 1024;
    hipLaunchKernelGGL(k_pack_segments, dim3(blocks), dim3(256), 0, s, A, d_dst);
    return hipGetLastError();
}

hipError_t drfe_launch_window_match(drfe_ctx* c, const MatchBuffers& mb, const drfe_camera& cam, int npairs,
                                    int maxQueries, int mode, float th, float nnratio, int checkOri,
                                    const uint8_t* d_initObs, hipStream_t s, int statusWord)
{
    const float invW = (float)DRFE_GRID_COLS / (float)(cam.max_x - cam.min_x);
    const float invH = (float)DRFE_GRID_ROWS / (float)(cam.max_y - cam.min_y);
    if (mode == 0 && maxQueries > RS_THREADS * RS_MAX_T) return hipErrorInvalidValue;
    (void)drfe_launch_fill_i32(c->d_status + statusWord, 1, 0, s);
    if (mode == 0)
        hipLaunchKernelGGL(k_queries_last, dim3((maxQueries + 255) / 256, npairs), dim3(256), 0, s, mb.d_pairs,
                           drfe_kps_un(c), c->d_kpCount, c->maxKp, mb.d_mps, cam, mb.d_scale, th, mb.d_queries);
    hipLaunchKernelGGL(k_window_candidates, dim3((maxQueries + WQ_PER_BLOCK - 1) / WQ_PER_BLOCK, npairs), dim3(WQ_THREADS), 0, s, mb.d_pairs,
                       mb.d_queries, c->d_kpCount, c->maxKp, c->d_gridOff, c->d_cellKp, c->d_cellDesc, cam, invW, invH,
                       mb.d_candIdx, mb.d_candKey, mb.d_candCnt, mb.d_candBest, c->d_status + statusWord,
                       drfe_div_magic((uint32_t)((maxQueries + WQ_PER_BLOCK - 1) / WQ_PER_BLOCK)));
    const size_t lds = (size_t)c->maxKp;
    if (mode == 0)
        hipLaunchKernelGGL(k_resolve_last, dim3(npairs), dim3(RS_THREADS), (size_t)c->maxKp * 5 + 16, s, mb.d_pairs,
                           mb.d_queries, drfe_kps_un(c), c->d_kpCount, c->maxKp, mb.d_candIdx, mb.d_candKey, mb.d_candCnt,
                           mb.d_candBest, checkOri, c->d_match, d_initObs, c->d_matchCount, mb.d_hist);
    else
        hipLaunchKernelGGL(k_resolve_map, dim3(npairs), dim3(WAVE), lds, s, mb.d_pairs, mb.d_queries, c->d_kpCount,
                           c->maxKp, mb.d_candIdx, mb.d_candKey, mb.d_candCnt, nnratio, c->d_match, d_initObs,
                           c->d_matchCount);
    return hipGetLastError();
}

hipError_t drfe_launch_window_candidates(drfe_ctx* c, const MatchBuffers& mb, const drfe_camera& cam, int npairs, int maxQueries,
                                         hipStream_t s)
{
    const float invW = (float)DRFE_GRID_COLS / (float)(cam.max_x - cam.min_x);
    const float invH = (float)DRFE_GRID_ROWS / (float)(cam.max_y - cam.min_y);
    (void)hipMemsetAsync(c->d_status + 1, 0, sizeof(int), s);
    hipLaunchKernelGGL(k_window_candidates, dim3((maxQueries + WQ_PER_BLOCK - 1) / WQ_PER_BLOCK, npairs), dim3(WQ_THREADS), 0, s, mb.d_pairs,
                       mb.d_queries, c->d_kpCount, c->maxKp, c->d_gridOff, c->d_cellKp, c->d_cellDesc, cam, invW, invH,
                       mb.d_candIdx, mb.d_candKey, mb.d_candCnt, mb.d_candBest, c->d_status + 1,
                       drfe_div_magic((uint32_t)((maxQueries + WQ_PER_BLOCK - 1) / WQ_PER_BLOCK)));
    return hipGetLastError();
}

hipError_t drfe_launch_mappoints_last(drfe_ctx* c, const MatchBuffers& mb, const drfe_camera& cam, const float* d_Twc,
                                      int nframes, hipStream_t s)
{
    hipLaunchKernelGGL(k_mappoints_last, dim3((c->maxKp + 255) / 256, nframes), dim3(256), 0, s, drfe_kps_un(c), c->d_desc,
                       c->d_kpCount, c->maxKp, c->d_depth, cam, d_Twc, mb.d_mps);
    return hipGetLastError();
}

hipError_t drfe_launch_bf_knn(const uint8_t* dQ, int nq, const uint8_t* dT, int nt, int k, int* dIdx, int* dDist,
                              hipStream_t s)
{
    hipLaunchKernelGGL(k_bf_knn, dim3((nq + 63) / 64), dim3(64), 0, s, dQ, nq, dT, nt, k, dIdx, dDist);
    return hipGetLastError();
}


__global__ __launch_bounds__(64) void k_line_queries_last(const drfe_map_line* __restrict__ lines, int n,
                                                          const float* __restrict__ TcwCur, drfe_camera cam, int forward,
                                                          int backward, const float* __restrict__ scale, float th,
                                                          LineQuery* __restrict__ out)
{
    const int i = blockIdx.x * 64 + threadIdx.x;
    if (i >= n) return;
    const drfe_map_line ml = lines[i];
    LineQuery q;
    q.valid = 0; q.obs = ml.obs_positive ? 1 : 0; q.minLevel = 0; q.maxLevel = 0;
    q.x1 = q.y1 = q.x2 = q.y2 = q.r = 0.f;
#pragma unroll
    for (int k = 0; k < 8; k++) q.desc[k] = reinterpret_cast<const uint32_t*>(ml.desc)[k];
    if (ml.valid) {
        const float SP[3] = {(float)ml.world[0], (float)ml.world[1], (float)ml.world[2]};
        const float EP[3] = {(float)ml.world[3], (float)ml.world[4], (float)ml.world[5]};
        float T[16];
#pragma unroll
        for (int k = 0; k < 16; k++) T[k] = TcwCur[k];
        float SPc[3], EPc[3];
        mat3_mul_add(T, SP, SPc);
        mat3_mul_add(T, EP, EPc);
        bool ok = !(SPc[2] < 0.0f || EPc[2] < 0.0f);
        const float invz1 = 1.0f / SPc[2];
        const float u1 = cam.fx * SPc[0] * invz1 + cam.cx, v1 = cam.fy * SPc[1] * invz1 + cam.cy;
        if (u1 < cam.min_x || u1 > cam.max_x || v1 < cam.min_y || v1 > cam.max_y) ok = false;
        const float invz2 = 1.0f / EPc[2];
        const float u2 = cam.fx * EPc[0] * invz2 + cam.cx, v2 = cam.fy * EPc[1] * invz2 + cam.cy;
        if (u2 < cam.min_x || u2 > cam.max_x || v2 < cam.min_y || v2 > cam.max_y) ok = false;
        if (ok) {
            const int oct = ml.octave;
            q.valid = 1;
            q.x1 = u1; q.y1 = v1; q.x2 = u2; q.y2 = v2;
            q.r = th * scale[oct];
            if (forward) { q.minLevel = oct; q.maxLevel = -1; }
            else if (backward) { q.minLevel = 0; q.maxLevel = oct; }
            else { q.minLevel = oct - 1; q.maxLevel = oct + 1; }
        }
    }
    out[i] = q;
}

__global__ __launch_bounds__(64) void k_line_search(const LineQuery* __restrict__ queries, int n,
                                                    const LineCur* __restrict__ cur, const uint8_t* __restrict__ desc,
                                                    int nCur, float nnratio, const uint8_t* __restrict__ claimIn ,
                                                    int* __restrict__ curMl, int* __restrict__ nmatchesOut)
{
    extern __shared__ unsigned char claim[];
    const int lane = threadIdx.x;
    for (int k = lane; k < nCur; k += WAVE) claim[k] = claimIn[k];
    __syncthreads();
    int nmatches = 0;
    for (int i = 0; i < n; i++) {
        const LineQuery q = queries[i];
        if (!q.valid) continue;
        const bool bCheckLevels = (q.minLevel > 0) || (q.maxLevel > 0);
        const float r2 = q.r * q.r;
        const double rs = (double)q.r * 0.01;
        const float sl0 = (q.y1 - q.y2) / (q.x1 - q.x2);
        const double mxq = 0.5 * (double)(q.x1 + q.x2), myq = 0.5 * (double)(q.y1 + q.y2);
        const uint64_t q0 = (uint64_t)q.desc[0] | ((uint64_t)q.desc[1] << 32), q1 = (uint64_t)q.desc[2] | ((uint64_t)q.desc[3] << 32),
                       q2 = (uint64_t)q.desc[4] | ((uint64_t)q.desc[5] << 32), q3 = (uint64_t)q.desc[6] | ((uint64_t)q.desc[7] << 32);
        uint32_t k1 = 0xFFFFFFFFu, k2 = 0xFFFFFFFFu;
        for (int idx = lane; idx < nCur; idx += WAVE) {
            const LineCur kl = cur[idx];
            const double mx = mxq - (double)kl.ptX, my = myq - (double)kl.ptY;
            const float distance = (float)(mx * mx + my * my);
            if (distance > r2) continue;
            const float slope = sl0 - kl.angle;
            if ((double)slope > rs) continue;
            if (bCheckLevels) {
                if (kl.octave < q.minLevel) continue;
                if (q.maxLevel >= 0 && kl.octave > q.maxLevel) continue;
            }
            if ((claim[idx] & 3) == 3) continue;
            const uint64_t* d = reinterpret_cast<const uint64_t*>(desc + (size_t)idx * 32);
            const int dist = __popcll(q0 ^ d[0]) + __popcll(q1 ^ d[1]) + __popcll(q2 ^ d[2]) + __popcll(q3 ^ d[3]);
            const uint32_t key = ((uint32_t)dist << 16) | (uint32_t)idx;
            if (key < k1) { k2 = k1; k1 = key; }
            else if (key < k2) k2 = key;
        }
        const uint32_t b1 = wave_min_u32(k1);
        if (b1 == 0xFFFFFFFFu) continue;
        const uint32_t b2 = wave_min_u32(k1 == b1 ? k2 : k1);
        const int bestDist = (int)(b1 >> 16), bestIdx = (int)(b1 & 0xFFFF);
        int bestDist2 = 256, bestLevel2 = -1;
        if (b2 != 0xFFFFFFFFu) { bestDist2 = (int)(b2 >> 16); bestLevel2 = cur[b2 & 0xFFFF].octave; }
        const int bestLevel = cur[bestIdx].octave;
        if (bestDist <= 100) {
            if (bestLevel == bestLevel2 && (float)bestDist > nnratio * (float)bestDist2) continue;
            if (lane == 0) {
                curMl[bestIdx] = i;
                claim[bestIdx] = (uint8_t)(1 | (q.obs ? 2 : 0));
            }
            __syncthreads();
            nmatches++;
        }
    }
    if (lane == 0) *nmatchesOut = nmatches;
}

hipError_t drfe_launch_line_projection(const drfe_map_line* d_lines, int n, const float* d_TcwCur, const drfe_camera& cam,
                                       int forward, int backward, const float* d_scale, float th, LineQuery* d_q,
                                       hipStream_t s)
{
    hipLaunchKernelGGL(k_line_queries_last, dim3((n + 63) / 64), dim3(64), 0, s, d_lines, n, d_TcwCur, cam, forward,
                       backward, d_scale, th, d_q);
    return hipGetLastError();
}

hipError_t drfe_launch_line_search(const LineQuery* d_q, int n, const LineCur* d_cur, const uint8_t* d_desc, int nCur,
                                   float nnratio, uint8_t* d_claim, int* d_curMl, int* d_nmatches, hipStream_t s)
{
    hipLaunchKernelGGL(k_line_search, dim3(1), dim3(64), (size_t)((nCur + 15) & ~15), s, d_q, n, d_cur, d_desc, nCur, nnratio, d_claim, d_curMl,
                       d_nmatches);
    return hipGetLastError();
}


__device__ __forceinline__ float norm3_f(const float v[3]) { return (float)sqrt((double)v[0] * v[0] + (double)v[1] * v[1] + (double)v[2] * v[2]); }
__device__ __forceinline__ double dot3_d(const float a[3], const float b[3]) { return (double)a[0] * b[0] + (double)a[1] * b[1] + (double)a[2] * b[2]; }

__global__ __launch_bounds__(256) void k_frustum_points(const drfe_frustum_point* __restrict__ pts, int n, FrustumPose P,
                                                        drfe_camera cam, drfe_tracked_point* __restrict__ out)
{
    const int i = blockIdx.x * 256 + threadIdx.x;
    if (i >= n) return;
    const drfe_frustum_point p = pts[i];
    drfe_tracked_point o = out[i];
    o.track_in_view = 0; o.level = 0; o.proj_x = o.proj_y = o.proj_xr = o.view_cos = 0.f;
    float Pc[3];
    mat3_mul_add(P.T, p.world, Pc);
    bool ok = !(Pc[2] < 0.0f);
    const float invz = 1.0f / Pc[2];
    const float u = cam.fx * Pc[0] * invz + cam.cx, v = cam.fy * Pc[1] * invz + cam.cy;
    if (u < cam.min_x || u > cam.max_x || v < cam.min_y || v > cam.max_y) ok = false;
    const float maxDistance = 1.2f * p.max_distance, minDistance = 0.8f * p.min_distance;
    const float PO[3] = {p.world[0] - P.Ow[0], p.world[1] - P.Ow[1], p.world[2] - P.Ow[2]};
    const float dist = norm3_f(PO);
    if (dist < minDistance || dist > maxDistance) ok = false;
    const float viewCos = (float)(dot3_d(PO, p.normal) / (double)dist);
    if (viewCos < P.limit) ok = false;
    if (ok) {
        const float ratio = p.max_distance / dist;
        int nScale = (int)ceilf(drfe_logf(ratio) / P.logScale);
        if (nScale < 0) nScale = 0;
        else if (nScale >= P.nLevels) nScale = P.nLevels - 1;
        o.track_in_view = 1; o.proj_x = u; o.proj_xr = u - P.bf * invz; o.proj_y = v; o.level = nScale; o.view_cos = viewCos;
    }
    out[i] = o;
}

__global__ __launch_bounds__(256) void k_frustum_lines(const drfe_frustum_line* __restrict__ lines, int n, FrustumPose P,
                                                       drfe_camera cam, drfe_tracked_line* __restrict__ out)
{
    const int i = blockIdx.x * 256 + threadIdx.x;
    if (i >= n) return;
    const drfe_frustum_line l = lines[i];
    drfe_tracked_line o = out[i];
    o.in_view = 0; o.level = 0; o.x1 = o.y1 = o.x2 = o.y2 = o.view_cos = 0.f;
    const float SP[3] = {(float)l.world[0], (float)l.world[1], (float)l.world[2]};
    const float EP[3] = {(float)l.world[3], (float)l.world[4], (float)l.world[5]};
    float SPc[3], EPc[3];
    mat3_mul_add(P.T, SP, SPc);
    mat3_mul_add(P.T, EP, EPc);
    bool ok = !(SPc[2] < 0.0f || EPc[2] < 0.0f);
    const float invz1 = 1.0f / SPc[2];
    const float u1 = cam.fx * SPc[0] * invz1 + cam.cx, v1 = cam.fy * SPc[1] * invz1 + cam.cy;
    if (u1 < cam.min_x || u1 > cam.max_x || v1 < cam.min_y || v1 > cam.max_y) ok = false;
    const float invz2 = 1.0f / EPc[2];
    const float u2 = cam.fx * EPc[0] * invz2 + cam.cx, v2 = cam.fy * EPc[1] * invz2 + cam.cy;
    if (u2 < cam.min_x || u2 > cam.max_x || v2 < cam.min_y || v2 > cam.max_y) ok = false;
    const float maxDistance = 1.2f * l.max_distance, minDistance = 0.8f * l.min_distance;
    float OM[3];
#pragma unroll
    for (int k = 0; k < 3; k++) OM[k] = (SP[k] + EP[k]) * 0.5f - P.Ow[k];
    const float dist = norm3_f(OM);
    if (dist < minDistance || dist > maxDistance) ok = false;
    const float pn[3] = {(float)l.normal[0], (float)l.normal[1], (float)l.normal[2]};
    const float viewCos = (float)(dot3_d(OM, pn) / (double)dist);
    if (viewCos < P.limit) ok = false;
    if (ok) {
        const float ratio = l.max_distance / dist;
        o.in_view = 1; o.x1 = u1; o.y1 = v1; o.x2 = u2; o.y2 = v2; o.view_cos = viewCos;
        o.level = (int)ceilf(drfe_logf(ratio) / P.logScale);
    }
    out[i] = o;
}

hipError_t drfe_launch_frustum_points(const drfe_frustum_point* d_pts, int n, const FrustumPose& P, const drfe_camera& cam,
                                      drfe_tracked_point* d_out, hipStream_t s)
{
    hipLaunchKernelGGL(k_frustum_points, dim3((n + 255) / 256), dim3(256), 0, s, d_pts, n, P, cam, d_out);
    return hipGetLastError();
}
hipError_t drfe_launch_frustum_lines(const drfe_frustum_line* d_lines, int n, const FrustumPose& P, const drfe_camera& cam,
                                     drfe_tracked_line* d_out, hipStream_t s)
{
    hipLaunchKernelGGL(k_frustum_lines, dim3((n + 255) / 256), dim3(256), 0, s, d_lines, n, P, cam, d_out);
    return hipGetLastError();
}


__global__ __launch_bounds__(256) void k_line_fuse_search(const drfe_frustum_line* __restrict__ lines, const uint8_t* __restrict__ descs,
                                                          const uint8_t* __restrict__ skip, int n, FrustumPose P, drfe_camera cam,
                                                          const float* __restrict__ scale, float th,
                                                          const LineCur* __restrict__ kf, const uint8_t* __restrict__ kfDesc, int nKF,
                                                          int* __restrict__ bestIdx, int* __restrict__ bestDist, int sim3,
                                                          LineSim3 C, int* __restrict__ distRow)
{
    const int lane = threadIdx.x & 63;
    const int i = blockIdx.x * (256 / WAVE) + __builtin_amdgcn_readfirstlane((int)(threadIdx.x >> 6));
    if (i >= n) return;
    int outIdx = -1, outDist = 0x7FFFFFFF;
    bool ok = !(skip && skip[i]);
    const drfe_frustum_line l = lines[i];
    const float SP[3] = {(float)l.world[0], (float)l.world[1], (float)l.world[2]};
    const float EP[3] = {(float)l.world[3], (float)l.world[4], (float)l.world[5]};
    float SPc[3], EPc[3];
    mat3_mul_add(P.T, SP, SPc);
    mat3_mul_add(P.T, EP, EPc);
    if (sim3) {
        float a[3];
#pragma unroll
        for (int r = 0; r < 3; r++) a[r] = (C.sR[r * 3] * SPc[0] + C.sR[r * 3 + 1] * SPc[1] + C.sR[r * 3 + 2] * SPc[2]) + C.t[r];
#pragma unroll
        for (int r = 0; r < 3; r++) SPc[r] = a[r];
#pragma unroll
        for (int r = 0; r < 3; r++) a[r] = (C.sR[r * 3] * EPc[0] + C.sR[r * 3 + 1] * EPc[1] + C.sR[r * 3 + 2] * EPc[2]) + C.t[r];
#pragma unroll
        for (int r = 0; r < 3; r++) EPc[r] = a[r];
    }
    if (SPc[2] < 0.0f || EPc[2] < 0.0f) ok = false;
    const float invz1 = 1.0f / SPc[2];
    const float u1 = cam.fx * SPc[0] * invz1 + cam.cx, v1 = cam.fy * SPc[1] * invz1 + cam.cy;
    const float invz2 = 1.0f / EPc[2];
    const float u2 = cam.fx * EPc[0] * invz2 + cam.cx, v2 = cam.fy * EPc[1] * invz2 + cam.cy;
    const float maxDistance = 1.2f * l.max_distance, minDistance = 0.8f * l.min_distance;
    float dist;
    if (sim3) {
        if (!(u1 >= cam.min_x && u1 < cam.max_x && v1 >= cam.min_y && v1 < cam.max_y)) ok = false;
        if (!(u2 >= cam.min_x && u2 < cam.max_x && v2 >= cam.min_y && v2 < cam.max_y)) ok = false;
        const float mid[3] = {(SPc[0] + EPc[0]) * 0.5f, (SPc[1] + EPc[1]) * 0.5f, (SPc[2] + EPc[2]) * 0.5f};
        dist = norm3_f(mid);
        if (dist < minDistance || dist > maxDistance) ok = false;
    } else {
        if (u1 < cam.min_x || u1 > cam.max_x || v1 < cam.min_y || v1 > cam.max_y) ok = false;
        if (u2 < cam.min_x || u2 > cam.max_x || v2 < cam.min_y || v2 > cam.max_y) ok = false;
        float OM[3];
#pragma unroll
        for (int k = 0; k < 3; k++) OM[k] = (SP[k] + EP[k]) * 0.5f - P.Ow[k];
        dist = norm3_f(OM);
        if (dist < minDistance || dist > maxDistance) ok = false;
        const float pn[3] = {(float)l.normal[0], (float)l.normal[1], (float)l.normal[2]};
        if (dot3_d(OM, pn) < 0.5 * (double)dist) ok = false;
    }
    if (distRow)
        for (int idx = lane; idx < nKF; idx += WAVE) distRow[(size_t)i * nKF + idx] = -1;
    if (ok) {
        const float ratio = l.max_distance / dist;
        const int level = (int)ceilf(drfe_logf(ratio) / P.logScale);
        if (level < 0 || level >= P.nLevels) {
            outIdx = -2;
        } else {
            const float r = th * scale[level];
            const float r2 = r * r;
            const double rs = (double)r * 0.01;
            const float sl0 = (v1 - v2) / (u1 - u2);
            const double mxq = 0.5 * (double)(u1 + u2), myq = 0.5 * (double)(v1 + v2);
            const uint64_t* q = reinterpret_cast<const uint64_t*>(descs + (size_t)i * 32);
            const uint64_t q0 = q[0], q1 = q[1], q2 = q[2], q3 = q[3];
            uint32_t best = 0xFFFFFFFFu;
            for (int idx = lane; idx < nKF; idx += WAVE) {
                const LineCur kl = kf[idx];
                const double mx = mxq - (double)kl.ptX, my = myq - (double)kl.ptY;
                const float distance = (float)(mx * mx + my * my);
                if (distance > r2) continue;
                const float slope = sl0 - kl.angle;
                if ((double)slope > rs) continue;
                if (kl.octave < level - 1 || kl.octave > level) continue;
                const uint64_t* d = reinterpret_cast<const uint64_t*>(kfDesc + (size_t)idx * 32);
                const int hd = __popcll(q0 ^ d[0]) + __popcll(q1 ^ d[1]) + __popcll(q2 ^ d[2]) + __popcll(q3 ^ d[3]);
                const uint32_t key = ((uint32_t)hd << 16) | (uint32_t)idx;
                if (key < best) best = key;
                if (distRow) distRow[(size_t)i * nKF + idx] = hd;
            }
            const uint32_t mn = wave_min_u32(best);
            if (mn != 0xFFFFFFFFu) { outIdx = (int)(mn & 0xFFFF); outDist = (int)(mn >> 16); }
        }
    }
    if (lane == 0) { bestIdx[i] = outIdx; bestDist[i] = outDist; }
}
// ... 166 lines not shown
```

dr_slam_amd/lib.py:

```python
from __future__ import annotations

import ctypes as C
import os

import numpy as np

_HERE = os.path.dirname(os.path.abspath(__file__))
LIB_PATH = os.environ.get("DRFE_LIB") or os.path.join(_HERE, "csrc", "libdrfe.so")

KP_DTYPE = np.dtype([("x", "<f4"), ("y", "<f4"), ("size", "<f4"), ("angle", "<f4"), ("response", "<f4"),
                     ("octave", "<i4"), ("class_id", "<i4")])
MAPPOINT_DTYPE = np.dtype([("valid", "u1"), ("obs_positive", "u1"), ("pad", "u1", (2,)), ("world", "<f4", (3,)),
                           ("desc", "u1", (32,))])
TRACKED_DTYPE = np.dtype([("track_in_view", "u1"), ("bad", "u1"), ("obs_positive", "u1"), ("pad", "u1"),
                          ("level", "<i4"), ("proj_x", "<f4"), ("proj_y", "<f4"), ("proj_xr", "<f4"),
                          ("view_cos", "<f4"), ("desc", "u1", (32,))])

STAGES = ("pyramid", "fast", "quadtree", "blur", "desc", "glue", "match", "fast_b")

SYMBOLS = (
    "drfe_create", "drfe_destroy", "drfe_last_error", "drfe_version", "drfe_orb_scale_tables",
    "drfe_orb_max_keypoints", "drfe_orb_extract", "drfe_orb_extract_batch", "drfe_orb_download", "drfe_orb_counts",
    "drfe_orb_pyramid_level", "drfe_orb_blurred_level", "drfe_orb_candidates", "drfe_frame_stereo_grid_batch",
    "drfe_fuse_search", "drfe_fuse_search_sim3", "drfe_search_by_sim3", "drfe_search_by_projection_kf", "drfe_search_by_projection_reloc", "drfe_lsd_fuse_search", "drfe_frame_is_in_frustum", "drfe_frame_is_in_frustum_lines", "drfe_frame_set_distortion", "drfe_frame_image_bounds", "drfe_frame_download_keys_un",
    "drfe_frame_download_stereo", "drfe_frame_download_grid", "drfe_match_consecutive_batch", "drfe_match_download",
    "drfe_search_by_projection_last", "drfe_search_by_projection_map", "drfe_match_bf_knn", "drfe_profile_enable",
    "drfe_profile_stage_ms", "drfe_stream_sync", "drfe_planes_ahc", "drfe_planes_ahc_batch", "drfe_planes_ahc_blocks",
    "drfe_match_orb_points", "drfe_planes_cape", "drfe_voc_upload", "drfe_bow_transform_batch", "drfe_bow_download",
    "drfe_search_by_bow", "drfe_search_by_bow_kf", "drfe_search_for_triangulation", "drfe_lsd_extract", "drfe_lsd_extract_batch", "drfe_lsd_stages", "drfe_lines_is_good", "drfe_lsd_search_by_descriptor", "drfe_lsd_search_for_triangulation", "drfe_lsd_search_by_projection_last",
    "drfe_lsd_search_by_projection_map", "drfe_plane_voxel_grid", "drfe_plane_refit", "drfe_planes_ahc_postprocess",
    "drfe_planes_cape_postprocess", "drfe_surface_normals", "drfe_surface_normals_batch", "drfe_surface_normals_download", "drfe_batch_download_async", "drfe_orb_fast_partition", "drfe_lsd_segments_host", "drfe_orb_keypoint_pixels_async", "drfe_gather_keypoint_depth",
    "drfe_frame_stereo_grid_batch_kpdepth", "drfe_planes_ahc_post_batch", "drfe_planes_ahc_from_blocks", "drfe_debug_ahc_trials", "drfe_debug_order_sort", "drfe_search_for_initialization", "drfe_lsd_fuse_search_sim3", "drfe_lsd_search_by_projection_kf",
    "drfe_lsd_search_by_sim3", "drfe_frame_submit", "drfe_frame_collect", "drfe_pipeline_create", "drfe_pipeline_destroy",
    "drfe_pipeline_depth", "drfe_pipeline_context", "drfe_pipeline_last_error", "drfe_pipeline_submit", "drfe_pipeline_sync",
    "drfe_lsd_configure", "drfe_lsd_configure_rect", "drfe_shard_unique_id", "drfe_shard_create", "drfe_shard_destroy", "drfe_shard_broadcast", "drfe_shard_reduce_report", "drfe_shard_sequences_of_rank", "drfe_shard_last_error", "drfe_planes_configure_cape", "drfe_planes_cape_stats", "drfe_lsd_configure_nfa", "drfe_lsd_stats", "drfe_lsd_segments_host_mode", "drfe_debug_cr_sincos", "drfe_debug_device_order_sort", "drfe_debug_device_order_sort_depth", "drfe_batch_status_async", "drfe_batch_check", "drfe_frame_submit_tracked", "drfe_frame_collect_tracked", "drfe_planes_cape_batch", "drfe_planes_configure", "drfe_planes_configure_extractor", "drfe_planes_ahc_stats", "drfe_planes_configure_refit", "drfe_planes_refit_stats", "drfe_frame_load", "drfe_bow_transform_slot", "drfe_long_kernel_clock", "drfe_long_kernel_ms",
    "drfe_manhattan_track_host", "drfe_manhattan_track_batch", "drfe_manhattan_download", "drfe_debug_manhattan_math",
    "drfe_plane_match_host", "drfe_plane_flag_points_host", "drfe_plane_match_status_host", "drfe_plane_map_upload",
    "drfe_plane_match_batch", "drfe_plane_match_download", "drfe_plane_flags_download",
    "drfe_map_plane_update_host", "drfe_map_plane_rebuild_host", "drfe_plane_map_update_batch", "drfe_plane_map_rebuild_batch",
    "drfe_plane_map_edit", "drfe_plane_map_cloud_download", "drfe_plane_map_update_stats",
    "drfe_map_point_upkeep_host", "drfe_map_line_upkeep_host", "drfe_map_point_upkeep_batch", "drfe_map_line_upkeep_batch",
    "drfe_map_upkeep_stats",
    "drfe_triangulate_points_host", "drfe_triangulate_lines_host", "drfe_triangulate_points_batch", "drfe_triangulate_lines_batch",
    "drfe_triangulate_stats", "drfe_debug_triangulate_math",
    "drfe_sim3_ransac_host", "drfe_sim3_ransac_batch", "drfe_sim3_stats", "drfe_debug_sim3_atan2", "drfe_debug_sim3_rand",
    "drfe_debug_sim3_horn", "drfe_debug_sim3_hand_back",
    "drfe_init_ransac_host", "drfe_init_ransac_batch", "drfe_init_stats",
    "drfe_debug_init_cos_keys", "drfe_debug_init_null_vectors", "drfe_debug_init_check_rt",
    "drfe_pnp_ransac_host", "drfe_pnp_ransac_batch", "drfe_pnp_stats", "drfe_debug_pnp_svd", "drfe_debug_pnp_inliers", "drfe_debug_pnp_inliers_device",
    "drfe_lines_is_good_batch", "drfe_line3d_chunk_frames", "drfe_line3d_stats",
    "drfe_pose_opt_host", "drfe_pose_opt_batch", "drfe_pose_opt_stats", "drfe_debug_cr_cube", "drfe_debug_pose_opt_ldlt",
    "drfe_debug_pose_opt_hand_back", "drfe_debug_pose_opt_plane_error",
)

FRUSTUM_POINT_DTYPE = np.dtype([("world", "<f4", (3,)), ("normal", "<f4", (3,)), ("min_distance", "<f4"),
                                ("max_distance", "<f4")])
FRUSTUM_LINE_DTYPE = np.dtype([("world", "<f8", (6,)), ("normal", "<f8", (3,)), ("min_distance", "<f4"),
                               ("max_distance", "<f4")])
MAPLINE_DTYPE = np.dtype([("valid", "<i4"), ("octave", "<i4"), ("obs_positive", "<i4"), ("pad", "<i4"),
                          ("world", "<f8", (6,)), ("desc", "u1", (32,))])
TRACKED_LINE_DTYPE = np.dtype([("in_view", "<i4"), ("level", "<i4"), ("obs_positive", "<i4"), ("x1", "<f4"),
                               ("y1", "<f4"), ("x2", "<f4"), ("y2", "<f4"), ("view_cos", "<f4"),
                               ("desc", "u1", (32,))])
KEYLINE_DTYPE = np.dtype([("angle", "<f4"), ("class_id", "<i4"), ("octave", "<i4"), ("pt_x", "<f4"), ("pt_y", "<f4"),
                          ("response", "<f4"), ("size", "<f4"), ("start_point_x", "<f4"), ("start_point_y", "<f4"),
                          ("end_point_x", "<f4"), ("end_point_y", "<f4"), ("s_point_in_octave_x", "<f4"),
                          ("s_point_in_octave_y", "<f4"), ("e_point_in_octave_x", "<f4"), ("e_point_in_octave_y", "<f4"),
                          ("line_length", "<f4"), ("num_of_pixels", "<i4")])

CAPE_PLANE_DTYPE = np.dtype([("normal", "<f8", (3,)), ("mean", "<f8", (3,)), ("d", "<f8"), ("mse", "<f4"),
                             ("score", "<f4"), ("n_points", "<i4"), ("pad", "<i4")])

PLANE_POST_DTYPE = np.dtype([("coef", "<f4", (4,)), ("accepted", "<i4"), ("n_voxels", "<i4")])
SURFACE_NORMAL_DTYPE = np.dtype([("normal", "<f4", (3,)), ("camera_position", "<f4", (3,)), ("frame_x", "<i4"),
                                 ("frame_y", "<i4")])

MANHATTAN_CALL_DTYPE = np.dtype([("in_cone", "<i4", (3,)), ("n_selected", "<i4", (3,)), ("threshold", "<i4"),
                                 ("deficient", "<i4"), ("found", "<i4"), ("svd", "<i4"), ("density", "<f4", (3,)),
                                 ("pad", "<i4")])
MANHATTAN_MAX_CALLS = 5
MANHATTAN_INLINE_BIT = 0x8000
MANHATTAN_INFO_DTYPE = np.dtype([("n_calls", "<i4"), ("pad", "<i4"),
                                 ("call", MANHATTAN_CALL_DTYPE, (MANHATTAN_MAX_CALLS,))])

PLANE_MATCH_DEFAULTS = np.array([0.1, 0.86, 0.08716, 0.9962], np.float32)

PLANE_DTYPE = np.dtype([("normal", "<f8", (3,)), ("center", "<f8", (3,)), ("mse", "<f8"), ("curvature", "<f8"),
                        ("n_points", "<i4"), ("rid", "<i4")])


class DrfeError(RuntimeError):
    pass


class Config(C.Structure):
    _fields_ = [("device", C.c_int32), ("max_width", C.c_int32), ("max_height", C.c_int32),
                ("max_batch", C.c_int32), ("nfeatures", C.c_int32), ("scale_factor", C.c_float),
                ("nlevels", C.c_int32), ("ini_th_fast", C.c_int32), ("min_th_fast", C.c_int32)]


class UpkeepKeyframes(C.Structure):
    _fields_ = [("n", C.c_int32), ("n_levels", C.c_int32), ("center", C.c_void_p), ("bad", C.c_void_p),
                ("scale_factors", C.c_void_p)]


class UpkeepItems(C.Structure):
    _fields_ = [("n", C.c_int32), ("pad", C.c_int32), ("bad", C.c_void_p), ("obs_offsets", C.c_void_p), ("obs_kf", C.c_void_p),
                ("obs_desc", C.c_void_p), ("world", C.c_void_p), ("ref_kf", C.c_void_p), ("ref_level", C.c_void_p)]


class UpkeepOut(C.Structure):
    _fields_ = [("best_obs", C.c_void_p), ("desc", C.c_void_p), ("normal", C.c_void_p), ("max_distance", C.c_void_p),
                ("min_distance", C.c_void_p), ("status", C.c_void_p), ("frustum", C.c_void_p)]


UPKEEP_DESCRIPTOR, UPKEEP_NORMAL = 1, 2
UPKEEP_DEVICE_ROWS = 2048
UPKEEP_STATS = ("calls", "items", "desc_b4", "desc_b16", "desc_b64", "desc_wg", "desc_host", "normals")

TRI_KF_DTYPE = np.dtype([("Tcw", np.float32, 12), ("Twc", np.float32, 12), ("Ow", np.float32, 3), ("fx", np.float32),
                         ("fy", np.float32), ("cx", np.float32), ("cy", np.float32), ("invfx", np.float32), ("invfy", np.float32),
                         ("mb", np.float32), ("mbf", np.float32), ("scale_factor", np.float32)])


class TriKeyframes(C.Structure):
    _fields_ = [("n", C.c_int32), ("n_levels", C.c_int32), ("kf", C.c_void_p), ("scale_factors", C.c_void_p),
                ("level_sigma2", C.c_void_p)]


class TriKeypoints(C.Structure):
    _fields_ = [("offsets", C.c_void_p), ("un", C.c_void_p), ("raw", C.c_void_p), ("octave", C.c_void_p),
                ("u_right", C.c_void_p), ("depth", C.c_void_p)]


class TriKeylines(C.Structure):
    _fields_ = [("offsets", C.c_void_p), ("ends", C.c_void_p), ("octave", C.c_void_p), ("depth", C.c_void_p),
                ("lines3d", C.c_void_p)]


class TriPairs(C.Structure):
    _fields_ = [("n", C.c_int32), ("pad", C.c_int32), ("kf1", C.c_void_p), ("kf2", C.c_void_p), ("match_offsets", C.c_void_p),
                ("matches", C.c_void_p)]


class TriOut(C.Structure):
    _fields_ = [("status", C.c_void_p), ("branch", C.c_void_p), ("x3d", C.c_void_p), ("pair_skipped", C.c_void_p),
                ("accepted", C.c_void_p)]


TRI_ACCEPTED, TRI_BASELINE, TRI_NO_PARALLAX = 0, 1, 2
TRI_POINT_CODES = ("accepted", "baseline", "no_parallax", "w_zero", "z1", "z2", "reproj1", "reproj2", "dist", "scale")
TRI_LINE_CODES = ("accepted", "baseline", "no_stereo", "z_sp1", "z_ep1", "z_sp2", "z_ep2", "reproj_sp1", "reproj_ep1",
                  "reproj_sp2", "reproj_ep2", "dist", "scale")
TRI_IDX2_PAST_KF1 = 0x80
TRI_BRANCH_NONE, TRI_BRANCH_SVD, TRI_BRANCH_STEREO1, TRI_BRANCH_STEREO2 = 0, 1, 2, 3
TRI_STATS = ("calls", "pairs", "pairs_skipped", "matches", "svd", "stereo1", "stereo2", "accepted")


class Sim3Problems(C.Structure):
    _fields_ = [("n", C.c_int32), ("pad", C.c_int32), ("Tcw1", C.c_void_p), ("Tcw2", C.c_void_p), ("K1", C.c_void_p),
                ("K2", C.c_void_p), ("fix_scale", C.c_void_p), ("probability", C.c_void_p), ("min_inliers", C.c_void_p),
                ("max_iterations", C.c_void_p), ("seed", C.c_void_p), ("offsets", C.c_void_p), ("Xw1", C.c_void_p),
                ("Xw2", C.c_void_p), ("sigma2_1", C.c_void_p), ("sigma2_2", C.c_void_p)]


class PnpProblems(C.Structure):
    _fields_ = [("n", C.c_int32), ("pad", C.c_int32)] + [(k, C.c_void_p) for k in (
        "K", "probability", "min_inliers", "max_iterations", "epsilon", "th2", "tail", "seed", "offsets", "p2d", "Xw",
        "sigma2")]


PNP_OUT_FIELDS = ("iterations", "min_inliers", "hypotheses", "refines", "sample", "R", "t", "inliers", "mask", "best", "returns",
                  "refined_R", "refined_t", "refined_inliers", "refined_mask")


class PnpOut(C.Structure):
    _fields_ = [(k, C.c_void_p) for k in PNP_OUT_FIELDS]


class PoseOptProblems(C.Structure):
    _fields_ = [("n", C.c_int32), ("pad", C.c_int32)] + [(k, C.c_void_p) for k in (
        "Tcw", "K", "bf", "b_struct", "point_offsets", "obs", "u_right", "inv_sigma2", "Xw", "line_offsets", "line_fn",
        "line_ends", "plane_offsets", "plane_meas", "plane_world", "plane_mask")] + [
        ("plane_settings", C.c_double * 7)]


POSE_OPT_OUT_FIELDS = ("Tcw", "returns", "rounds", "iterations", "trials", "diag", "point_outlier", "line_outlier", "plane_outlier",
                       "par_plane_outlier", "ver_plane_outlier")
POSE_OPT_DIAG = ("rejected", "last_rejected", "nbad_stops", "small_theta", "big_theta", "empty_rounds")
POSE_OPT_MAX_FRAMES, POSE_OPT_MAX_POINTS, POSE_OPT_MAX_LINES, POSE_OPT_MAX_PLANES = 4096, 8192, 1024, 64
POSE_OPT_PLANE_MATCHED, POSE_OPT_PLANE_PARALLEL, POSE_OPT_PLANE_VERTICAL = 1, 2, 4
POSEOPT_DEVICE_FROM = 64
POSE_OPT_STATS = ("calls", "frames", "point_edges", "line_plane_edges", "iterations", "trials", "handed_back", "frames_too_few")


class PoseOptOut(C.Structure):
    _fields_ = [(k, C.c_void_p) for k in POSE_OPT_OUT_FIELDS]


class InitProblems(C.Structure):
    _fields_ = [("n", C.c_int32), ("pad", C.c_int32)] + [(k, C.c_void_p) for k in (
        "K", "sigma", "max_iterations", "seed", "key1_offsets", "key2_offsets", "keys1", "keys2",
        "matches12")]


INIT_OUT_FIELDS = ("N", "iterations", "hypotheses", "SH", "SF", "RH", "branch", "motions", "ok", "flags", "R21", "t21", "vP3D",
                   "vbTriangulated", "sample", "H21", "F21", "score_h", "score_f", "best_h", "best_f", "mask_h", "mask_f",
                   "motion_R", "motion_t", "motion_good", "motion_cos", "motion_parallax", "motion_status", "motion_vbGood",
                   "motion_vP3D")
INIT_BRANCH_NONE, INIT_BRANCH_H, INIT_BRANCH_F = 0, 1, 2
INIT_TOO_FEW, INIT_NO_MODEL, INIT_H_DEGENERATE = 1, 2, 4
INIT_MOTION_NAN_COS = 1
INIT_MAX_KEYS, INIT_MAX_ITERATIONS, INIT_MAX_SOLVERS, INIT_MAX_ROWS, INIT_MAX_MASK_WORDS = 4096, 300, 65535, 1 << 20, 1 << 24
INIT_STATS = ("calls", "solvers", "rows", "matches", "branch_h", "branch_f", "ok", "empty")


class InitOut(C.Structure):
    _fields_ = [(k, C.c_void_p) for k in INIT_OUT_FIELDS]


class Sim3Out(C.Structure):
    _fields_ = [("iterations", C.c_void_p), ("hypotheses", C.c_void_p), ("sample", C.c_void_p), ("R12", C.c_void_p),
                ("t12", C.c_void_p), ("s12", C.c_void_p), ("T12", C.c_void_p), ("inliers", C.c_void_p), ("returns", C.c_void_p),
                ("best", C.c_void_p), ("mask", C.c_void_p)]


SIM3_MAX_CORR, SIM3_MAX_ITERATIONS = 4096, 300
SIM3_STATS = ("calls", "solvers", "hypotheses", "correspondences", "solvers_lds", "solvers_global", "uncertified", "solvers_empty")
PNP_STATS = ("calls", "solvers", "hypotheses", "correspondences", "refine_jobs", "refine_points", "solvers_global", "solvers_empty")
LINE3D_STATS = ("calls", "frames", "lines", "ransac_lines", "iterations", "coincident_pairs", "verify_rejections", "accepted")
LINE3D_MAX_CAP = 4096


class Line3dFrames(C.Structure):
    _fields_ = [("nframes", C.c_int32), ("cap", C.c_int32), ("lines", C.c_void_p), ("n_lines", C.c_void_p), ("depth", C.c_void_p),
                ("frame_stride", C.c_size_t), ("stride", C.c_size_t), ("w", C.c_int32), ("h", C.c_int32),
                ("depth_on_device", C.c_int32), ("k_as_f64", C.c_int32), ("K", C.c_float * 9), ("cx", C.c_float),
                ("cy", C.c_float), ("invfx", C.c_float), ("invfy", C.c_float), ("seeds", C.c_void_p)]


class Line3dOut(C.Structure):
    _fields_ = [(k, C.c_void_p) for k in ("depth_line", "lines3d", "n_inliers", "n_good")]


class Camera(C.Structure):
    _fields_ = [("fx", C.c_float), ("fy", C.c_float), ("cx", C.c_float), ("cy", C.c_float), ("bf", C.c_float),
                ("depth_factor", C.c_float), ("min_x", C.c_float), ("max_x", C.c_float), ("min_y", C.c_float),
                ("max_y", C.c_float)]


_lib = None


def load() -> C.CDLL:
    global _lib
    if _lib is not None:
        return _lib
    if not os.path.exists(LIB_PATH):
        raise DrfeError(f"{LIB_PATH} not found: build it with `make -C dr_slam_amd/csrc` "
                        "(there is no CPU fallback for the feature path)")
    try:
        import torch
    except Exception:
        pass
    L = C.CDLL(LIB_PATH)
    vp, i32, f32, sz = C.c_void_p, C.c_int, C.c_float, C.c_size_t
    L.drfe_create.argtypes = [C.POINTER(Config), C.POINTER(vp)]
    L.drfe_destroy.argtypes = [vp]
    L.drfe_destroy.restype = None
    L.drfe_last_error.argtypes = [vp]
    L.drfe_last_error.restype = C.c_char_p
    L.drfe_version.restype = C.c_char_p
    L.drfe_orb_scale_tables.argtypes = [vp, vp, vp, vp, vp]
    L.drfe_orb_max_keypoints.argtypes = [vp]
    L.drfe_orb_extract.argtypes = [vp, vp, i32, i32, sz, vp, vp, i32, C.POINTER(i32)]
    L.drfe_orb_extract_batch.argtypes = [vp, vp, sz, sz, i32, i32, i32, vp]
    L.drfe_pipeline_create.argtypes = [C.POINTER(Config), i32, C.POINTER(vp)]
    L.drfe_pipeline_destroy.argtypes = [vp]
    L.drfe_pipeline_destroy.restype = None
    L.drfe_pipeline_depth.argtypes = [vp]
    L.drfe_pipeline_context.argtypes = [vp, i32]
    L.drfe_pipeline_context.restype = vp
    L.drfe_pipeline_last_error.argtypes = [vp]
    L.drfe_pipeline_last_error.restype = C.c_char_p
    L.drfe_pipeline_submit.argtypes = [vp, vp, vp, sz, sz, i32, i32, vp, vp, C.POINTER(Camera), C.c_float, i32, i32, i32]
    L.drfe_pipeline_sync.argtypes = [vp, i32]
    L.drfe_frame_submit.argtypes = [vp, i32, vp, i32, i32, sz, vp, sz, C.POINTER(Camera)]
    L.drfe_frame_collect.argtypes = [vp, i32, vp, vp, vp, vp, i32, C.POINTER(i32)]
    L.drfe_frame_submit_tracked.argtypes = [vp, i32, vp, i32, i32, sz, vp, sz, C.POINTER(Camera), i32, vp, vp, vp, vp, i32, f32, i32, i32]
    L.drfe_frame_collect_tracked.argtypes = [vp, i32, vp, vp, vp, vp, i32, C.POINTER(i32), vp, C.POINTER(i32)]
    L.drfe_orb_download.argtypes = [vp, i32, vp, vp, i32, C.POINTER(i32)]
    L.drfe_orb_counts.argtypes = [vp, i32, vp]
    L.drfe_orb_fast_partition.argtypes = [vp, i32, i32, vp, vp]
    L.drfe_orb_keypoint_pixels_async.argtypes = [vp, i32, vp, vp, vp]
    L.drfe_gather_keypoint_depth.argtypes = [vp, sz, sz, i32, vp, vp, i32, vp, i32]
    L.drfe_frame_stereo_grid_batch_kpdepth.argtypes = [vp, vp, i32, C.POINTER(Camera), i32, vp]
    L.drfe_batch_download_async.argtypes = [vp, i32, vp, vp, vp, vp, vp, vp]
    L.drfe_orb_pyramid_level.argtypes = [vp, i32, i32, vp, C.POINTER(i32), C.POINTER(i32)]
    L.drfe_orb_blurred_level.argtypes = [vp, i32, i32, vp, C.POINTER(i32), C.POINTER(i32)]
    L.drfe_orb_candidates.argtypes = [vp, i32, i32, vp, i32, C.POINTER(i32)]
    L.drfe_frame_stereo_grid_batch.argtypes = [vp, vp, sz, sz, C.POINTER(Camera), i32, vp]
    L.drfe_frame_download_stereo.argtypes = [vp, i32, vp, vp, i32]
    L.drfe_frame_download_grid.argtypes = [vp, i32, vp, vp, i32]
    L.drfe_match_consecutive_batch.argtypes = [vp, vp, vp, C.POINTER(Camera), f32, i32, i32, i32, vp]
    L.drfe_match_download.argtypes = [vp, i32, vp, i32, C.POINTER(i32)]
    L.drfe_search_by_projection_last.argtypes = [vp, i32, i32, vp, vp, C.POINTER(Camera), vp, i32, f32, i32, i32,
                                                 vp, vp, i32, C.POINTER(i32)]
    L.drfe_search_by_projection_map.argtypes = [vp, i32, vp, i32, f32, f32, vp, vp, i32, C.POINTER(i32)]
    L.drfe_match_bf_knn.argtypes = [vp, vp, i32, vp, i32, i32, vp, vp]
    L.drfe_match_orb_points.argtypes = [vp, i32, i32, vp, vp, i32, vp, i32, C.POINTER(i32)]
    L.drfe_search_by_bow_kf.argtypes = [vp, i32, i32, vp, i32, vp, i32, C.c_float, i32, vp, C.POINTER(i32)]
    L.drfe_search_for_triangulation.argtypes = [vp, i32, i32, vp, i32, vp, i32, vp, vp, vp, vp, i32, i32, vp, C.POINTER(i32)]
    L.drfe_planes_ahc_batch.argtypes = [vp, vp, C.c_size_t, i32, i32, C.c_size_t, i32, vp, C.c_float, vp, i32, vp, vp, vp, vp, i32]
    L.drfe_lsd_extract_batch.argtypes = [vp, vp, C.c_size_t, i32, i32, C.c_size_t, i32, i32, vp, vp, vp, i32, vp, vp, i32]
    L.drfe_lines_is_good.argtypes = [vp, i32, vp, i32, i32, C.c_size_t, vp, i32, C.c_float, C.c_float, C.c_float, C.c_float,
                                     C.c_uint32, vp, vp, vp, C.POINTER(i32)]
    L.drfe_lsd_fuse_search.argtypes = [vp, vp, vp, vp, vp, vp, i32, vp, vp, i32, C.c_float, vp, vp]
    L.drfe_lsd_fuse_search_sim3.argtypes = [vp, vp, vp, vp, vp, vp, i32, vp, vp, i32, C.c_float, vp, vp]
    L.drfe_lsd_search_by_projection_kf.argtypes = [vp, vp, vp, vp, vp, vp, i32, vp, vp, i32, vp, i32, vp, C.POINTER(i32)]
    L.drfe_lsd_search_by_sim3.argtypes = [vp, vp, vp, vp, C.c_float, vp, vp, vp, vp, vp, vp, vp, i32, vp, vp, vp, vp, vp, i32, C.c_float,
                                          vp, C.POINTER(i32)]
    L.drfe_search_by_projection_reloc.argtypes = [vp, i32, vp, vp, vp, vp, vp, i32, vp, i32, C.c_float, i32, i32, vp, C.POINTER(i32)]
    L.drfe_search_for_initialization.argtypes = [vp, i32, i32, vp, i32, i32, C.c_float, i32, vp, C.POINTER(i32)]
    L.drfe_search_by_projection_kf.argtypes = [vp, i32, vp, vp, vp, vp, i32, vp, i32, C.c_float, vp, C.POINTER(i32)]
    L.drfe_search_by_sim3.argtypes = [vp, i32, i32, vp, vp, C.c_float, vp, vp, vp, vp, vp, i32, vp, vp, vp, i32, C.c_float, vp,
                                      C.POINTER(i32)]
    L.drfe_fuse_search_sim3.argtypes = [vp, i32, vp, vp, vp, vp, i32, C.c_float, vp, vp]
    L.drfe_fuse_search.argtypes = [vp, i32, vp, vp, vp, vp, i32, C.c_float, vp, vp]
    L.drfe_frame_is_in_frustum.argtypes = [vp, vp, vp, vp, i32, C.c_float, vp]
    L.drfe_frame_is_in_frustum_lines.argtypes = [vp, vp, vp, vp, i32, C.c_float, vp]
    L.drfe_frame_set_distortion.argtypes = [vp, vp, vp, i32]
    L.drfe_frame_image_bounds.argtypes = [vp, vp, i32, i32, i32, vp]
    L.drfe_frame_download_keys_un.argtypes = [vp, i32, vp, i32]
    L.drfe_lsd_search_for_triangulation.argtypes = [vp, vp, i32, vp, i32, vp, vp, vp, C.POINTER(i32)]
    L.drfe_lsd_search_by_descriptor.argtypes = [vp, vp, i32, vp, i32, vp, i32, vp, C.POINTER(i32)]
    L.drfe_lsd_search_by_projection_last.argtypes = [vp, vp, vp, vp, vp, i32, vp, vp, i32, C.c_float, i32, C.c_float, vp, vp,
                                                     C.POINTER(i32)]
    L.drfe_lsd_search_by_projection_map.argtypes = [vp, vp, i32, vp, vp, i32, C.c_float, C.c_float, vp, vp, C.POINTER(i32)]
    L.drfe_lsd_extract.argtypes = [vp, vp, i32, i32, sz, i32, vp, vp, vp, i32, C.POINTER(i32), C.POINTER(i32)]
    L.drfe_lsd_stages.argtypes = [vp, vp, vp, vp, vp, vp, C.POINTER(i32), C.POINTER(i32)]
    L.drfe_voc_upload.argtypes = [vp, i32, i32, i32, i32, i32, vp, vp, vp, vp]
    L.drfe_bow_transform_batch.argtypes = [vp, i32, i32, vp]
    L.drfe_bow_download.argtypes = [vp, i32, vp, vp, vp, i32]
    L.drfe_search_by_bow.argtypes = [vp, i32, i32, vp, i32, f32, i32, vp, i32, C.POINTER(i32)]
    L.drfe_planes_ahc.argtypes = [vp, vp, i32, i32, sz, vp, f32, vp, i32, C.POINTER(i32), vp, vp, vp]
    L.drfe_planes_ahc_blocks.argtypes = [vp, vp, i32, i32, sz, vp, f32, vp, vp, i32]
    L.drfe_planes_cape.argtypes = [vp, vp, i32, i32, sz, vp, i32, f32, f32, vp, i32, C.POINTER(i32), vp, vp, vp, vp]
    f64 = C.c_double
    L.drfe_plane_voxel_grid.argtypes = [vp, i32, f32, vp, i32, C.POINTER(i32)]
    L.drfe_plane_refit.argtypes = [vp, vp, i32, f64, C.POINTER(i32)]
    L.drfe_planes_ahc_postprocess.argtypes = [vp, vp, i32, i32, sz, vp, f32, vp, i32, vp, vp, f32, f64, vp, vp, vp, i32,
                                              C.POINTER(i32), C.POINTER(i32)]
    L.drfe_planes_ahc_post_batch.argtypes = [vp, vp, sz, i32, i32, sz, i32, vp, f32, f32, f64, vp, i32, vp, vp, vp, vp, vp, i32]
    L.drfe_debug_ahc_trials.argtypes = [vp, vp, i32, i32, vp]
    L.drfe_debug_order_sort.argtypes = [vp, sz, i32, i32, i32, C.c_uint32]
    L.drfe_planes_ahc_from_blocks.argtypes = [vp, vp, vp, i32, i32, sz, vp, f32, vp, i32, C.POINTER(i32), vp, vp, vp]
    L.drfe_planes_cape_postprocess.argtypes = [vp, vp, i32, i32, sz, vp, vp, vp, i32, f32, f64, vp, vp, vp, i32,
                                               C.POINTER(i32), C.POINTER(i32)]
    L.drfe_surface_normals.argtypes = [vp, vp, i32, i32, sz, vp, f32, vp, i32, C.POINTER(i32), vp, vp, vp]
    L.drfe_surface_normals_batch.argtypes = [vp, vp, sz, sz, i32, i32, vp, f32, f32, i32, vp]
    L.drfe_surface_normals_download.argtypes = [vp, i32, vp, i32, C.POINTER(i32)]
    L.drfe_manhattan_track_host.argtypes = [vp, vp, i32, vp, i32, i32, vp, vp, vp, vp]
    L.drfe_manhattan_track_batch.argtypes = [vp, vp, i32, i32, vp, vp, i32, vp]
    L.drfe_manhattan_download.argtypes = [vp, i32, vp, vp, vp, vp]
    L.drfe_debug_manhattan_math.argtypes = [i32, vp, i32, vp]
    L.drfe_plane_match_host.argtypes = [vp, vp, vp, i32, vp, vp, vp, vp, i32, vp, vp, vp, C.POINTER(i32)]
    L.drfe_plane_flag_points_host.argtypes = [vp, vp, i32, vp, vp, i32, vp, C.POINTER(i32)]
    L.drfe_plane_match_status_host.argtypes = [vp, vp, vp, i32, vp, vp, i32, vp, C.POINTER(i32)]
    L.drfe_plane_map_upload.argtypes = [vp, i32, vp, vp, vp, vp, vp, vp, vp]
    L.drfe_plane_match_batch.argtypes = [vp, vp, i32, vp, vp, vp, vp, vp, vp, vp, i32, vp]
    L.drfe_plane_match_download.argtypes = [vp, i32, vp, vp, vp, C.POINTER(i32), C.POINTER(i32)]
    L.drfe_plane_flags_download.argtypes = [vp, i32, vp]
    L.drfe_map_plane_update_host.argtypes = [vp, vp, i32, vp, i32, vp, i32, C.POINTER(i32)]
    L.drfe_map_plane_rebuild_host.argtypes = [i32, vp, vp, vp, vp, i32, C.POINTER(i32)]
    L.drfe_plane_map_update_batch.argtypes = [vp, i32, vp, vp, vp, vp, vp, vp, vp]
    L.drfe_plane_map_rebuild_batch.argtypes = [vp, i32, vp, vp, vp, vp, vp, vp, vp]
    L.drfe_plane_map_edit.argtypes = [vp, i32, i32, vp, vp, vp]
    L.drfe_plane_map_cloud_download.argtypes = [vp, i32, i32, vp, i32, C.POINTER(i32)]
    L.drfe_plane_map_update_stats.argtypes = [vp, vp]
    L.drfe_map_point_upkeep_host.argtypes = [i32, vp, vp, vp]
    L.drfe_map_line_upkeep_host.argtypes = [i32, vp, vp, vp]
    L.drfe_map_point_upkeep_batch.argtypes = [vp, i32, vp, vp, vp, vp]
    L.drfe_map_line_upkeep_batch.argtypes = [vp, i32, vp, vp, vp, vp]
    L.drfe_map_upkeep_stats.argtypes = [vp, vp]
    L.drfe_triangulate_points_host.argtypes = [i32, vp, vp, vp, vp]
    L.drfe_triangulate_lines_host.argtypes = [i32, vp, vp, vp, vp]
    L.drfe_triangulate_points_batch.argtypes = [vp, i32, vp, vp, vp, vp, vp]
    L.drfe_triangulate_lines_batch.argtypes = [vp, i32, vp, vp, vp, vp, vp]
    L.drfe_triangulate_stats.argtypes = [vp, vp]
    L.drfe_debug_triangulate_math.argtypes = [i32, vp, vp, i32, vp]
    L.drfe_sim3_ransac_host.argtypes = [vp, vp]
    L.drfe_sim3_ransac_batch.argtypes = [vp, vp, vp, vp]
    L.drfe_sim3_stats.argtypes = [vp, vp]
    L.drfe_debug_sim3_atan2.argtypes = [vp, vp, i32, vp, vp]
    L.drfe_debug_sim3_rand.argtypes = [C.c_uint32, i32, vp]
    L.drfe_debug_sim3_horn.argtypes = [vp, vp, i32, i32, i32, vp, vp]
    L.drfe_debug_sim3_hand_back.argtypes = [vp, i32]
    L.drfe_pnp_ransac_host.argtypes = [vp, vp]
    L.drfe_init_ransac_host.argtypes = [vp, vp]
    L.drfe_init_ransac_batch.argtypes = [vp, vp, vp, vp]
    L.drfe_init_stats.argtypes = [vp, vp]
    L.drfe_debug_init_cos_keys.argtypes = [vp, i32, vp, vp]
    L.drfe_debug_init_null_vectors.argtypes = [vp, i32, vp, vp]
    L.drfe_debug_init_check_rt.argtypes = [vp, vp, vp, vp, C.c_float, vp, i32, vp, vp, vp, vp, vp, vp]
    L.drfe_pnp_ransac_batch.argtypes = [vp, vp, vp, vp]
    L.drfe_pose_opt_host.argtypes = [vp, vp]
    L.drfe_pose_opt_batch.argtypes = [vp, vp, vp, vp]
    L.drfe_pose_opt_stats.argtypes = [vp, vp]
    L.drfe_debug_cr_cube.argtypes = [vp, i32, vp, vp]
    L.drfe_debug_pose_opt_ldlt.argtypes = [vp, vp, vp, vp]
    L.drfe_debug_pose_opt_hand_back.argtypes = [vp, i32]
    L.drfe_debug_pose_opt_plane_error.argtypes = [i32, vp, vp, vp, vp]
    L.drfe_pnp_stats.argtypes = [vp, vp]
    L.drfe_lines_is_good_batch.argtypes = [vp, vp, vp, vp]
    L.drfe_line3d_chunk_frames.argtypes = [i32]
    L.drfe_line3d_stats.argtypes = [vp, vp]
    L.drfe_debug_pnp_svd.argtypes = [vp, i32, i32, vp, vp, vp]
    L.drfe_debug_pnp_inliers.argtypes = [vp, vp, vp, vp, vp, vp, i32, vp]
    L.drfe_debug_pnp_inliers_device.argtypes = [vp, vp, vp, vp, vp, vp, vp, i32, vp]
    L.drfe_lsd_segments_host.argtypes = [vp, vp, vp, i32, i32, f64, vp, i32, C.POINTER(i32)]
    L.drfe_lsd_configure.argtypes = [vp, i32]
    L.drfe_lsd_configure_rect.argtypes = [vp, i32]
    L.drfe_shard_unique_id.argtypes = [vp]
    L.drfe_shard_create.argtypes = [vp, i32, i32, i32, C.POINTER(vp)]
    L.drfe_shard_destroy.argtypes = [vp]
    L.drfe_shard_destroy.restype = None
    L.drfe_shard_broadcast.argtypes = [vp, vp, sz, i32]
    L.drfe_shard_reduce_report.argtypes = [vp, vp, i32, vp, i32]
    L.drfe_shard_sequences_of_rank.argtypes = [i32, i32, i32, vp, i32]
    L.drfe_shard_last_error.argtypes = [vp]
    L.drfe_shard_last_error.restype = C.c_char_p
    L.drfe_planes_configure_cape.argtypes = [vp, i32]
    L.drfe_planes_cape_stats.argtypes = [vp, vp]
    L.drfe_planes_ahc_stats.argtypes = [vp, vp]
    L.drfe_planes_configure_refit.argtypes = [vp, i32]
    L.drfe_planes_refit_stats.argtypes = [vp, vp]
    L.drfe_frame_load.argtypes = [vp, i32, vp, vp, vp, vp, vp, i32, vp]
    L.drfe_bow_transform_slot.argtypes = [vp, i32, i32, vp]
    L.drfe_lsd_configure_nfa.argtypes = [vp, i32]
    L.drfe_lsd_stats.argtypes = [vp, vp]
    L.drfe_long_kernel_clock.argtypes = [vp, i32]
    L.drfe_long_kernel_ms.argtypes = [vp, vp]
    L.drfe_lsd_segments_host_mode.argtypes = [vp, vp, vp, i32, i32, f64, i32, vp, i32, C.POINTER(i32)]
    L.drfe_planes_configure.argtypes = [vp, i32]
    L.drfe_planes_configure_extractor.argtypes = [vp, i32]
    L.drfe_planes_cape_batch.argtypes = [vp, vp, sz, i32, i32, sz, i32, vp, i32, f32, f32, vp, i32, vp, vp, i32]
    L.drfe_batch_status_async.argtypes = [vp, vp, vp]
    L.drfe_batch_check.argtypes = [vp]
    L.drfe_debug_cr_sincos.argtypes = [vp, i32, vp, vp, vp]
    L.drfe_debug_device_order_sort.argtypes = [vp, vp, sz, C.POINTER(i32)]
    L.drfe_debug_device_order_sort_depth.argtypes = [vp, vp, sz, i32, C.POINTER(i32)]
    L.drfe_profile_enable.argtypes = [vp, i32]
    L.drfe_profile_stage_ms.argtypes = [vp, vp]
    L.drfe_stream_sync.argtypes = [vp]
    _lib = L
    return L


def _p(a):
    return None if a is None else a.ctypes.data_as(C.c_void_p)


def lsd_segments_host(modgrad, angles, cs, max_grad, rect_mode=0):
    L = load()
    m = np.ascontiguousarray(modgrad, np.float64)
    a = np.ascontiguousarray(angles, np.float64)
    c = np.ascontiguousarray(cs, np.float32)
    H, W = m.shape
    out = np.zeros((20000, 4), np.float32)
    n = C.c_int()
    rc = L.drfe_lsd_segments_host_mode(_p(m), _p(a), _p(c), W, H, float(max_grad), int(rect_mode), _p(out), len(out), C.byref(n))
    if rc != 0:
        raise DrfeError(f"drfe_lsd_segments_host failed ({rc})")
    return out[:n.value].copy()


def planes_ahc_from_blocks(blocks17, valid, N, depth16, K4, depth_factor, cap=64):
    L = load()
    d = np.ascontiguousarray(depth16, np.uint16)
    h, w = d.shape
    b = np.ascontiguousarray(blocks17, np.float64)
    vn = np.ascontiguousarray(np.stack([valid, N], 1), np.int32)
    planes = np.zeros(cap, PLANE_DTYPE)
    n = C.c_int()
    seg = np.zeros((h, w), np.uint8)
    off = np.zeros(cap + 1, np.int32)
    idx = np.zeros(h * w, np.int32)
    rc = L.drfe_planes_ahc_from_blocks(_p(b), _p(vn), _p(d), w, h, w, _p(np.ascontiguousarray(K4, np.float32)), np.float32(depth_factor),
                                       _p(planes), cap, C.byref(n), _p(seg), _p(off), _p(idx))
    if rc != 0:
        raise DrfeError(f"drfe_planes_ahc_from_blocks failed ({rc})")
    return dict(planes=planes[:n.value].copy(), seg=seg, members=[idx[off[i]:off[i + 1]].copy() for i in range(n.value)])


def plane_voxel_grid(xyz, leaf=0.05):
    L = load()
    p = np.ascontiguousarray(xyz, np.float32).reshape(-1, 3)
    out = np.zeros_like(p)
    n = C.c_int()
    rc = L.drfe_plane_voxel_grid(_p(p), len(p), np.float32(leaf), _p(out), len(p), C.byref(n))
    if rc != 0:
        raise DrfeError(f"drfe_plane_voxel_grid failed ({rc})")
    return out[:n.value].copy()


def plane_refit(coef4, xyz, dist_threshold):
    L = load()
    c = np.ascontiguousarray(coef4, np.float32).copy()
    p = np.ascontiguousarray(xyz, np.float32).reshape(-1, 3)
    v = C.c_int()
    rc = L.drfe_plane_refit(_p(c), _p(p), len(p), float(dist_threshold), C.byref(v))
    if rc != 0:
        raise DrfeError(f"drfe_plane_refit failed ({rc})")
    return bool(v.value), c


def manhattan_track_host(R, recs, line_dirs=None, n_calls=3):
    L = load()
    R = np.ascontiguousarray(R, np.float32).reshape(3, 3)
    recs = np.ascontiguousarray(recs, SURFACE_NORMAL_DTYPE)
    dirs = np.ascontiguousarray(np.zeros((0, 3)) if line_dirs is None else line_dirs, np.float64).reshape(-1, 3)
    out = np.zeros((3, 3), np.float32)
    info = np.zeros((), MANHATTAN_INFO_DTYPE)
    rb = np.zeros(len(recs), np.uint16)
    lb = np.zeros(len(dirs), np.uint16)
    rc = L.drfe_manhattan_track_host(_p(R), _p(recs), len(recs), _p(dirs), len(dirs), n_calls, _p(out), _p(info), _p(rb), _p(lb))
    if rc != 0:
        raise DrfeError(f"drfe_manhattan_track_host failed ({rc})")
    return out, info, rb, lb


def _plane_params(params):
    return np.ascontiguousarray(PLANE_MATCH_DEFAULTS if params is None else params, np.float32).reshape(4)


def _clouds_csr(clouds):
    off = np.zeros(len(clouds) + 1, np.int32)
    off[1:] = np.cumsum([len(c) for c in clouds]) if len(clouds) else []
    xyz = np.concatenate([np.asarray(c, np.float32).reshape(-1, 3) for c in clouds]) if len(clouds) else np.zeros((0, 3), np.float32)
    return off, np.ascontiguousarray(xyz, np.float32)


def _priors(p, n):
    return np.full(n, -1, np.int32) if p is None else np.array(p, np.int32).reshape(n)


def plane_match_host(Tcw, coefs, map_coefs, map_bad, clouds, map_idx=None, par_idx=None, ver_idx=None, params=None):
    L = load()
    T = np.ascontiguousarray(Tcw, np.float32).reshape(16)
    cf = np.ascontiguousarray(coefs, np.float32).reshape(-1, 4)
    mc = np.ascontiguousarray(map_coefs, np.float32).reshape(-1, 4)
    bad = np.ascontiguousarray(map_bad, np.uint8).reshape(len(mc))
    off, xyz = _clouds_csr(clouds)
    assert len(off) == len(mc) + 1
    P = len(cf)
    mi, pi, vi = _priors(map_idx, P), _priors(par_idx, P), _priors(ver_idx, P)
    n = C.c_int()
    prm = _plane_params(params)
    rc = L.drfe_plane_match_host(_p(prm), _p(T), _p(cf), P, _p(mc), _p(bad), _p(off), _p(xyz), len(mc), _p(mi), _p(pi), _p(vi),
                                 C.byref(n))
    if rc != 0:
        raise DrfeError(f"drfe_plane_match_host failed ({rc})")
    return mi, pi, vi, n.value


def plane_flag_points_host(Tcw, coefs, map_idx, points, flags=None):
    L = load()
    T = np.ascontiguousarray(Tcw, np.float32).reshape(16)
    cf = np.ascontiguousarray(coefs, np.float32).reshape(-1, 4)
    mi = np.ascontiguousarray(map_idx, np.int32).reshape(len(cf))
    pts = np.ascontiguousarray(points, np.float32).reshape(-1, 3)
    fl = np.zeros(len(pts), np.uint8) if flags is None else np.array(flags, np.uint8).reshape(len(pts))
    n = C.c_int()
    rc = L.drfe_plane_flag_points_host(_p(T), _p(cf), len(cf), _p(mi), _p(pts), len(pts), _p(fl), C.byref(n))
    if rc != 0:
        raise DrfeError(f"drfe_plane_flag_points_host failed ({rc})")
    return fl, n.value


def plane_match_status_host(Tcw, coefs, matched_coefs, matched, mf_contrast, Rwc_MF=None, params=None):
    L = load()
    T = np.ascontiguousarray(Tcw, np.float32).reshape(16)
    cf = np.ascontiguousarray(coefs, np.float32).reshape(-1, 4)
    mc = np.ascontiguousarray(matched_coefs, np.float32).reshape(len(cf), 4)
    m = np.ascontiguousarray(matched, np.uint8).reshape(len(cf))
    R = None if Rwc_MF is None else np.ascontiguousarray(Rwc_MF, np.float32).reshape(9)
    st = C.c_int()
    prm = _plane_params(params)
    rc = L.drfe_plane_match_status_host(_p(prm), _p(T), _p(cf), len(cf), _p(mc), _p(m), int(bool(mf_contrast)), _p(R), C.byref(st))
    if rc != 0:
        raise DrfeError(f"drfe_plane_match_status_host failed ({rc})")
    return bool(st.value)


def map_plane_update_host(Tcw, frame_xyz, map_xyz):
    L = load()
    T = np.ascontiguousarray(Tcw, np.float32).reshape(16)
    fx = np.ascontiguousarray(frame_xyz, np.float32).reshape(-1, 3)
    mx = np.ascontiguousarray(map_xyz, np.float32).reshape(-1, 3)
    out = np.zeros((len(fx) + len(mx), 3), np.float32)
    n = C.c_int()
    rc = L.drfe_map_plane_update_host(_p(T), _p(fx), len(fx), _p(mx), len(mx), _p(out), len(out), C.byref(n))
    if rc != 0:
        raise DrfeError(f"drfe_map_plane_update_host failed ({rc})")
    return out[:n.value].copy()


def map_plane_rebuild_host(Twc, clouds):
    L = load()
    T = np.ascontiguousarray(np.asarray(Twc, np.float32).reshape(-1, 16), np.float32)
    off, xyz = _clouds_csr(clouds)
    assert len(T) == len(clouds)
    out = np.zeros((max(len(xyz), 1), 3), np.float32)
    n = C.c_int()
    rc = L.drfe_map_plane_rebuild_host(len(clouds), _p(T), _p(off), _p(xyz), _p(out), len(xyz), C.byref(n))
    if rc != 0:
        raise DrfeError(f"drfe_map_plane_rebuild_host failed ({rc})")
    return out[:n.value].copy()


def _upkeep_call(fn, head, line, scene, what, frustum):
    a = {}

    def arr(key, dt, shape=None):
        v = scene.get(key)
        if v is None:
            return None
        v = np.ascontiguousarray(v, dt)
        a[key] = v if shape is None else v.reshape(shape)
        return a[key]
    off = arr("obs_offsets", np.int32, -1)
    n = len(off) - 1 if off is not None else 0
    cen = arr("kf_center", np.float32, (-1, 3))
    sc = arr("scale_factors", np.float32, -1)
    kfb = arr("kf_bad", np.uint8, -1)
    kfs = UpkeepKeyframes(len(cen), len(sc), _p(cen), _p(kfb), _p(sc))
    items = UpkeepItems(n, 0, _p(arr("bad", np.uint8, -1)), _p(off), _p(arr("obs_kf", np.int32, -1)),
                        _p(arr("obs_desc", np.uint8, (-1, 32))),
                        _p(arr("world", np.float64 if line else np.float32, (-1, 6 if line else 3))),
                        _p(arr("ref_kf", np.int32, -1)), _p(arr("ref_level", np.int32, -1)))
    r = dict(best_obs=np.zeros(n, np.int32), desc=np.zeros((n, 32), np.uint8),
             normal=np.zeros((n, 3), np.float64 if line else np.float32), max_distance=np.zeros(n, np.float32),
             min_distance=np.zeros(n, np.float32), status=np.zeros(n, np.uint8))
    if frustum:
        r["frustum"] = np.zeros(n, FRUSTUM_LINE_DTYPE if line else FRUSTUM_POINT_DTYPE)
    out = UpkeepOut(_p(r["best_obs"]), _p(r["desc"]), _p(r["normal"]), _p(r["max_distance"]), _p(r["min_distance"]),
                    _p(r["status"]), _p(r.get("frustum")))
    rc = fn(*head, int(what), C.byref(kfs), C.byref(items), C.byref(out), *([None] if head else []))
    return rc, r


def map_point_upkeep_host(scene, what=3, frustum=True):
    L = load()
    rc, r = _upkeep_call(L.drfe_map_point_upkeep_host, (), False, scene, what, frustum)
    if rc != 0:
        raise DrfeError(f"drfe_map_point_upkeep_host failed ({rc})")
    return r

# ... 1473 lines not shown
```

include/drfe_debug.h:

```cpp
#ifndef DRFE_DEBUG_H
#define DRFE_DEBUG_H
#include "drfe.h"
#ifdef __cplusplus
extern "C" {
#endif

int drfe_debug_cr_sincos(const double* x, int n, double* s, double* c, int32_t* ok);

int drfe_debug_device_order_sort(drfe_ctx* ctx, uint32_t* keys, size_t n, int* status);
int drfe_debug_device_order_sort_depth(drfe_ctx* ctx, uint32_t* keys, size_t n, int depth_limit, int* status);

int drfe_debug_ahc_trials(const double* sums9, const int32_t* N, int n, int mode, double* out8);

int drfe_debug_order_sort(void* recs, size_t n, int kind, int mode, int depth_limit, uint32_t skip_below);

int drfe_debug_manhattan_math(int which, const double* x, int n, double* out);

int drfe_debug_triangulate_math(int which, const float* y, const float* x, int n, float* out);

int drfe_debug_sim3_atan2(const double* y, const double* x, int n, double* out, int32_t* ok);
int drfe_debug_sim3_rand(uint32_t seed, int n, int32_t* out);
int drfe_debug_sim3_horn(const float* P1, const float* P2, int n, int fix_scale, int libm, float* out, int32_t* ok);
int drfe_debug_sim3_hand_back(drfe_ctx* ctx, int every);
int drfe_debug_pnp_svd(const double* A, int m, int n, double* w, double* ut, double* vt);
int drfe_debug_pnp_inliers(const double* R, const double* t, const float* K, const float* p2d, const float* Xw, const float* max_err,
                           int n, uint8_t* out);
int drfe_debug_pnp_inliers_device(drfe_ctx* ctx, const double* R, const double* t, const float* K, const float* p2d, const float* Xw,
                                  const float* max_err, int n, uint8_t* out);
int drfe_debug_init_cos_keys(const float* c, int n, uint32_t* key, float* value);
int drfe_debug_init_null_vectors(const float* points, int n, float* h, float* fpre);
int drfe_debug_init_check_rt(drfe_ctx* ctx, const float* K, const float* R, const float* t, float sigma, const float* matches, int n,
                             int32_t* good, float* cos_selected, float* parallax, int32_t* status, uint8_t* vbGood, float* vP3D);
int drfe_debug_cr_cube(const double* x, int n, double* out, uint8_t* ok);
int drfe_debug_pose_opt_ldlt(const double* A, const double* b, double* x, int32_t* positive);
int drfe_debug_pose_opt_plane_error(int kind, const float* meas, const float* world, const float* Tcw, double* e);
int drfe_debug_pose_opt_hand_back(drfe_ctx* ctx, int every);

#ifdef __cplusplus
}
#endif
#endif
```

Baseline: 281,700 frames/s.

## Fuse stereo, grid, mappoint projection, window match and resolve into one kernel

```diff
diff --git a/dr_slam_amd/csrc/capi_match.cpp b/dr_slam_amd/csrc/capi_match.cpp
--- a/dr_slam_amd/csrc/capi_match.cpp
+++ b/dr_slam_amd/csrc/capi_match.cpp
@@ -388,6 +388,27 @@
     return e;
 }
 
+int drfe_tail_fused_batch(drfe_ctx* c, const uint16_t* d_depth, size_t frame_stride, size_t row_stride, const float* Tcw, const float* Twc,
+                          const drfe_camera* cam, float th, int mono, int check_ori, int nframes, hipStream_t s)
+{
+    if (!c || !d_depth || !cam || !Tcw || !Twc) return DRFE_ERR_INVALID;
+    if (nframes < 2 || nframes > c->lastBatch) { c->err = "glue: extract the batch first"; return DRFE_ERR_STATE; }
+    if (!(cam->max_x > cam->min_x) || !(cam->max_y > cam->min_y)) { c->err = "glue: empty image bounds"; return DRFE_ERR_INVALID; }
+    if (row_stride == 0 ? frame_stride != (size_t)c->maxKp
+                        : (row_stride < (size_t)c->geom.imgW || frame_stride < row_stride * (size_t)c->geom.imgH)) {
+        c->err = "glue: depth row / frame stride smaller than the image";
+        return DRFE_ERR_INVALID;
+    }
+    if (!drfe_tail_fused_lds(c->maxKp)) { c->err = "fused tail: the slot size does not fit the launch"; return DRFE_ERR_CAPACITY; }
+    HIPCHK(c, hipSetDevice(c->device));
+    const int rc = drfe_match_consecutive_stage(c, Tcw, Twc, cam, mono, nframes, s);
+    if (rc != DRFE_OK) return rc;
+    HIPCHK(c, drfe_launch_tail_fused(c, *drfe_match_buffers(c), d_depth, frame_stride, row_stride, *cam, th, check_ori, nframes, s));
+    c->glueValid = true;
+    c->cam = *cam;
+    return DRFE_OK;
+}
+
 extern "C" {
 
 int drfe_match_consecutive_batch(drfe_ctx* c, const float* Tcw, const float* Twc, const drfe_camera* cam, float th,
@@ -411,6 +432,15 @@
     HIPCHK(c, drfe_match_consecutive_enqueue(c, cam, th, check_ori, nframes, s));
     if (c->profile) (void)hipEventRecord(c->ev[DRFE_STAGE_MATCH][1], s);
     return DRFE_OK;
+}
+
+int drfe_debug_tail_fused_lds_bytes(int max_keypoints) { return (int)drfe_tail_fused_lds(max_keypoints); }
+
+int drfe_debug_tail_fused_batch(drfe_ctx* c, const uint16_t* d_depth, size_t frame_stride, size_t row_stride, const float* Tcw,
+                                const float* Twc, const drfe_camera* cam, float th, int mono, int check_ori, int nframes)
+{
+    if (!c) return DRFE_ERR_INVALID;
+    return drfe_tail_fused_batch(c, d_depth, frame_stride, row_stride, Tcw, Twc, cam, th, mono, check_ori, nframes, c->stream);
 }
 
 int drfe_match_download(drfe_ctx* c, int slot, int32_t* cur_to_last, int cap, int* nmatches)
diff --git a/dr_slam_amd/csrc/capi_pipeline.cpp b/dr_slam_amd/csrc/capi_pipeline.cpp
--- a/dr_slam_amd/csrc/capi_pipeline.cpp
+++ b/dr_slam_amd/csrc/capi_pipeline.cpp
@@ -1,4 +1,5 @@
 #include "drfe_internal.h"
+#include "match_internal.h"
 
 #include <new>
 #include <vector>
@@ -8,6 +9,8 @@
     unsigned long long submitted = 0;
     std::string err;
 };
+
+static bool drfe_pipeline_tail_is_fused(int maxKp) { return drfe_tail_fused_lds(maxKp) != 0; }
 
 extern "C" {
 
@@ -57,9 +60,13 @@
     int rc = drfe_orb_extract_batch(c, d_gray, frame_stride, row_stride, w, h, nframes, nullptr);
     if (rc == DRFE_OK && d_depth) {
         if (!cam) { p->err = "drfe_pipeline_submit: a depth batch needs the camera"; return DRFE_ERR_INVALID; }
-        rc = drfe_frame_stereo_grid_batch(c, d_depth, frame_stride, row_stride, cam, nframes, nullptr);
-        if (rc == DRFE_OK && Tcw && Twc && nframes >= 2)
-            rc = drfe_match_consecutive_batch(c, Tcw, Twc, cam, th, mono, check_ori, nframes, nullptr);
+        if (Tcw && Twc && nframes >= 2 && drfe_pipeline_tail_is_fused(c->maxKp))
+            rc = drfe_tail_fused_batch(c, d_depth, frame_stride, row_stride, Tcw, Twc, cam, th, mono, check_ori, nframes, c->stream);
+        else {
+            rc = drfe_frame_stereo_grid_batch(c, d_depth, frame_stride, row_stride, cam, nframes, nullptr);
+            if (rc == DRFE_OK && Tcw && Twc && nframes >= 2)
+                rc = drfe_match_consecutive_batch(c, Tcw, Twc, cam, th, mono, check_ori, nframes, nullptr);
+        }
     }
     if (rc != DRFE_OK) { p->err = drfe_last_error(c); return rc; }
     p->submitted++;
diff --git a/dr_slam_amd/csrc/match_internal.h b/dr_slam_amd/csrc/match_internal.h
--- a/dr_slam_amd/csrc/match_internal.h
+++ b/dr_slam_amd/csrc/match_internal.h
@@ -90,6 +90,23 @@
                                    int* d_bestDist, hipStream_t s, const uint8_t* d_taken = nullptr, int2* d_list = nullptr,
                                    int* d_listCount = nullptr);
 
+#define DRFE_TAIL_FUSED_THREADS 512
+#define DRFE_TAIL_FUSED_MAX_LDS 65536
+static inline size_t drfe_tail_fused_lds(int maxKp)
+{
+    if (maxKp < 1 || maxKp > DRFE_MATCH_LAST_MAX_QUERIES || maxKp > 65535) return 0;
+    const size_t grid = sizeof(int) * (size_t)(DRFE_GRID_CELLS + (DRFE_GRID_CELLS + 4) + DRFE_TAIL_FUSED_THREADS / 64) + 4 * (size_t)maxKp;
+    const size_t window = sizeof(int) * (size_t)(DRFE_TAIL_FUSED_THREADS / 64) * 4 * 64;
+    const size_t resolve = 5 * (size_t)maxKp + 16;
+    size_t b = grid > window ? grid : window;
+    if (resolve > b) b = resolve;
+    b = (b + 15) & ~(size_t)15;
+    return b <= DRFE_TAIL_FUSED_MAX_LDS ? b : 0;
+}
+hipError_t drfe_launch_tail_fused(drfe_ctx* c, const MatchBuffers& mb, const uint16_t* d_depth, size_t frameStride, size_t rowStride,
+                                  const drfe_camera& cam, float th, int checkOri, int nframes, hipStream_t s);
+int drfe_tail_fused_batch(drfe_ctx* c, const uint16_t* d_depth, size_t frame_stride, size_t row_stride, const float* Tcw, const float* Twc,
+                          const drfe_camera* cam, float th, int mono, int check_ori, int nframes, hipStream_t s);
 MatchBuffers* drfe_match_buffers(drfe_ctx* c);
 int drfe_match_consecutive_stage(drfe_ctx* c, const float* Tcw, const float* Twc, const drfe_camera* cam, int mono, int nframes, hipStream_t s);
 hipError_t drfe_match_consecutive_enqueue(drfe_ctx* c, const drfe_camera* cam, float th, int check_ori, int nframes, hipStream_t s);
diff --git a/dr_slam_amd/csrc/match_kernels.hip b/dr_slam_amd/csrc/match_kernels.hip
--- a/dr_slam_amd/csrc/match_kernels.hip
+++ b/dr_slam_amd/csrc/match_kernels.hip
@@ -18,6 +18,28 @@
     kpsUn[(size_t)slot * maxKp + i] = kp;
 }
 
+__device__ __forceinline__ float stereo_depth(const drfe_keypoint& kp, int slot, int i, const uint16_t* depth, size_t frameStride,
+                                              size_t rowStride, int w, int h, const drfe_camera& cam)
+{
+    const int v = (int)kp.y, u = (int)kp.x;
+    float d = 0.f;
+    if (u >= 0 && u < w && v >= 0 && v < h)
+        d = (float)depth[rowStride ? (size_t)slot * frameStride + (size_t)v * rowStride + u : (size_t)slot * frameStride + i] * cam.depth_factor;
+    return d;
+}
+
+__device__ __forceinline__ void stereo_keypoint(const drfe_keypoint* kps, const drfe_keypoint* kpsUn, int maxKp, int slot, int i,
+                                                const uint16_t* depth, size_t frameStride, size_t rowStride, int w, int h,
+                                                const drfe_camera& cam, float* uRight, float* zDepth)
+{
+    const drfe_keypoint kp = kps[(size_t)slot * maxKp + i];
+    const float d = stereo_depth(kp, slot, i, depth, frameStride, rowStride, w, h, cam);
+    float ur = -1.f, z = -1.f;
+    if (d > 0) { z = d; ur = kpsUn[(size_t)slot * maxKp + i].x - cam.bf / d; }
+    uRight[(size_t)slot * maxKp + i] = ur;
+    zDepth[(size_t)slot * maxKp + i] = z;
+}
+
 __global__ __launch_bounds__(256) void k_stereo(const drfe_keypoint* __restrict__ kps, const drfe_keypoint* __restrict__ kpsUn,
                                                 const int* __restrict__ kpCount,
                                                 int maxKp, const uint16_t* __restrict__ depth, size_t frameStride,
@@ -27,15 +49,7 @@
     const int slot = blockIdx.y;
     const int i = blockIdx.x * 256 + threadIdx.x;
     if (i >= kpCount[slot]) return;
-    const drfe_keypoint kp = kps[(size_t)slot * maxKp + i];
-    const int v = (int)kp.y, u = (int)kp.x;
-    float d = 0.f;
-    if (u >= 0 && u < w && v >= 0 && v < h)
-        d = (float)depth[rowStride ? (size_t)slot * frameStride + (size_t)v * rowStride + u : (size_t)slot * frameStride + i] * cam.depth_factor;
-    float ur = -1.f, z = -1.f;
-    if (d > 0) { z = d; ur = kpsUn[(size_t)slot * maxKp + i].x - cam.bf / d; }
-    uRight[(size_t)slot * maxKp + i] = ur;
-    zDepth[(size_t)slot * maxKp + i] = z;
+    stereo_keypoint(kps, kpsUn, maxKp, slot, i, depth, frameStride, rowStride, w, h, cam, uRight, zDepth);
 }
 
 __device__ __forceinline__ int grid_cell(const drfe_keypoint& kp, const drfe_camera& cam, float invW, float invH)
@@ -44,6 +58,64 @@
     const int py = (int)roundf((kp.y - cam.min_y) * invH);
     if (px < 0 || px >= DRFE_GRID_COLS || py < 0 || py >= DRFE_GRID_ROWS) return -1;
     return px * DRFE_GRID_ROWS + py;
+}
+
+template <int NT, bool LDS_LIST, class IdxT>
+__device__ __forceinline__ void grid_body(const drfe_keypoint* K, int n, const drfe_camera& cam, float invW, float invH,
+                                          const float* UR, const uint4* D4, int* gOff, int* gIdx, uint4* cK, uint4* cD,
+                                          int* cnt, int* off, int* wtot, IdxT* list, int16_t* cellOf)
+{
+    static_assert(DRFE_GRID_CELLS % NT == 0 && NT % WAVE == 0, "cells are dealt evenly to the threads");
+    const int tid = threadIdx.x;
+    for (int c = tid; c < DRFE_GRID_CELLS; c += NT) cnt[c] = 0;
+    __syncthreads();
+    for (int i = tid; i < n; i += NT) {
+        const int c = grid_cell(K[i], cam, invW, invH);
+        if (LDS_LIST) cellOf[i] = (int16_t)c;
+        if (c >= 0) atomicAdd(&cnt[c], 1);
+    }
+    __syncthreads();
+    const int per = DRFE_GRID_CELLS / NT;
+    int s = 0;
+#pragma unroll
+    for (int k = 0; k < per; k++) s += cnt[tid * per + k];
+    const int incl = drfe_wave_incl_scan(s, tid & 63);
+    if ((tid & 63) == 63) wtot[tid >> 6] = incl;
+    __syncthreads();
+    int run = incl - s;
+    for (int w = 0; w < (tid >> 6); w++) run += wtot[w];
+#pragma unroll
+    for (int k = 0; k < per; k++) { off[tid * per + k] = run; run += cnt[tid * per + k]; }
+    if (tid == NT - 1) off[DRFE_GRID_CELLS] = run;
+    __syncthreads();
+    for (int c = tid; c <= DRFE_GRID_CELLS; c += NT) gOff[c] = off[c];
+    for (int c = tid; c < DRFE_GRID_CELLS; c += NT) cnt[c] = 0;
+    __syncthreads();
+    for (int i = tid; i < n; i += NT) {
+        const int c = LDS_LIST ? (int)cellOf[i] : grid_cell(K[i], cam, invW, invH);
+        if (c >= 0) list[off[c] + atomicAdd(&cnt[c], 1)] = (IdxT)i;
+    }
+    __syncthreads();
+    for (int c = tid; c < DRFE_GRID_CELLS; c += NT) {
+        const int b = off[c], e = off[c + 1];
+        for (int a = b + 1; a < e; a++) {
+            const IdxT v = list[a];
+            int j = a - 1;
+            while (j >= b && list[j] > v) { list[j + 1] = list[j]; j--; }
+            list[j + 1] = v;
+        }
+    }
+    __syncthreads();
+    const int nIn = off[DRFE_GRID_CELLS];
+    for (int p = tid; p < nIn; p += NT) {
+        const int idx = (int)list[p];
+        if (LDS_LIST) gIdx[p] = idx;
+        const drfe_keypoint kp = K[idx];
+        cK[p] = make_uint4(__float_as_uint(kp.x), __float_as_uint(kp.y), __float_as_uint(UR[idx]),
+                           (uint32_t)idx | ((uint32_t)kp.octave << 24));
+        cD[2 * p] = D4[2 * idx];
+        cD[2 * p + 1] = D4[2 * idx + 1];
+    }
 }
 
 __global__ __launch_bounds__(256) void k_grid(const drfe_keypoint* __restrict__ kps, const int* __restrict__ kpCount,
@@ -54,65 +126,13 @@
 {
     __shared__ int cnt[DRFE_GRID_CELLS];
     __shared__ int off[DRFE_GRID_CELLS + 1];
-    __shared__ int part[256];
-    const int slot = blockIdx.x, tid = threadIdx.x;
-    const int n = kpCount[slot];
-    const drfe_keypoint* K = kps + (size_t)slot * maxKp;
+    __shared__ int wtot[256 / WAVE];
+    const int slot = blockIdx.x;
     int* gIdx = gridIdx + (size_t)slot * maxKp;
-    int* gOff = gridOff + (size_t)slot * (DRFE_GRID_CELLS + 1);
-    for (int c = tid; c < DRFE_GRID_CELLS; c += 256) cnt[c] = 0;
-    __syncthreads();
-    for (int i = tid; i < n; i += 256) {
-        const int c = grid_cell(K[i], cam, invW, invH);
-        if (c >= 0) atomicAdd(&cnt[c], 1);
-    }
-    __syncthreads();
-    const int per = DRFE_GRID_CELLS / 256;
-    int s = 0;
-    for (int k = 0; k < per; k++) s += cnt[tid * per + k];
-    part[tid] = s;
-    __syncthreads();
-    for (int o = 1; o < 256; o <<= 1) {
-        const int v = (tid >= o) ? part[tid - o] : 0;
-        __syncthreads();
-        part[tid] += v;
-        __syncthreads();
-    }
-    int run = part[tid] - s;
-    for (int k = 0; k < per; k++) { off[tid * per + k] = run; run += cnt[tid * per + k]; }
-    if (tid == 255) off[DRFE_GRID_CELLS] = run;
-    __syncthreads();
-    for (int c = tid; c <= DRFE_GRID_CELLS; c += 256) gOff[c] = off[c];
-    for (int c = tid; c < DRFE_GRID_CELLS; c += 256) cnt[c] = 0;
-    __syncthreads();
-    for (int i = tid; i < n; i += 256) {
-        const int c = grid_cell(K[i], cam, invW, invH);
-        if (c >= 0) gIdx[off[c] + atomicAdd(&cnt[c], 1)] = i;
-    }
-    __syncthreads();
-    for (int c = tid; c < DRFE_GRID_CELLS; c += 256) {
-        const int b = off[c], e = off[c + 1];
-        for (int a = b + 1; a < e; a++) {
-            const int v = gIdx[a];
-            int j = a - 1;
-            while (j >= b && gIdx[j] > v) { gIdx[j + 1] = gIdx[j]; j--; }
-            gIdx[j + 1] = v;
-        }
-    }
-    __syncthreads();
-    const int nIn = off[DRFE_GRID_CELLS];
-    uint4* cK = cellKp + (size_t)slot * maxKp;
-    uint4* cD = cellDesc + (size_t)slot * maxKp * 2;
-    const uint4* D4 = reinterpret_cast<const uint4*>(desc + (size_t)slot * maxKp * 32);
-    const float* UR = uRight + (size_t)slot * maxKp;
-    for (int p = tid; p < nIn; p += 256) {
-        const int idx = gIdx[p];
-        const drfe_keypoint kp = K[idx];
-        cK[p] = make_uint4(__float_as_uint(kp.x), __float_as_uint(kp.y), __float_as_uint(UR[idx]),
-                           (uint32_t)idx | ((uint32_t)kp.octave << 24));
-        cD[2 * p] = D4[2 * idx];
-        cD[2 * p + 1] = D4[2 * idx + 1];
-    }
+    grid_body<256, false, int>(kps + (size_t)slot * maxKp, kpCount[slot], cam, invW, invH, uRight + (size_t)slot * maxKp,
+                               reinterpret_cast<const uint4*>(desc + (size_t)slot * maxKp * 32),
+                               gridOff + (size_t)slot * (DRFE_GRID_CELLS + 1), gIdx, cellKp + (size_t)slot * maxKp,
+                               cellDesc + (size_t)slot * maxKp * 2, cnt, off, wtot, gIdx, nullptr);
 }
 
 
@@ -123,6 +143,16 @@
         const float d = T[r * 4 + 0] * x[0] + T[r * 4 + 1] * x[1] + T[r * 4 + 2] * x[2];
         out[r] = d + T[r * 4 + 3];
     }
+}
+
+__device__ __forceinline__ void unproject_last(const drfe_keypoint& kp, float z, const drfe_camera& cam, const float* Twc, float world[3])
+{
+    const float invfx = 1.0f / cam.fx, invfy = 1.0f / cam.fy;
+    float p[3];
+    p[0] = (kp.x - cam.cx) * z * invfx;
+    p[1] = (kp.y - cam.cy) * z * invfy;
+    p[2] = z;
+    mat3_mul_add(Twc, p, world);
 }
 
 __global__ __launch_bounds__(256) void k_mappoints_last(const drfe_keypoint* __restrict__ kps,
@@ -142,20 +172,38 @@
     mp.obs_positive = 1;
     mp.pad[0] = mp.pad[1] = 0;
     mp.world[0] = mp.world[1] = mp.world[2] = 0.f;
-    if (z > 0) {
-        const float invfx = 1.0f / cam.fx, invfy = 1.0f / cam.fy;
-        const drfe_keypoint kp = kps[o];
-        float p[3];
-        p[0] = (kp.x - cam.cx) * z * invfx;
-        p[1] = (kp.y - cam.cy) * z * invfy;
-        p[2] = z;
-        mat3_mul_add(Twc + (size_t)slot * 16, p, mp.world);
-    }
+    if (z > 0) unproject_last(kps[o], z, cam, Twc + (size_t)slot * 16, mp.world);
     const uint32_t* d = reinterpret_cast<const uint32_t*>(desc + o * 32);
     uint32_t* md = reinterpret_cast<uint32_t*>(mp.desc);
 #pragma unroll
     for (int k = 0; k < 8; k++) md[k] = d[k];
     mps[o] = mp;
+}
+
+__device__ __forceinline__ void project_query(const float* Tcw, int forward, int backward, int valid, const float world[3], int oct,
+                                              const drfe_camera& cam, const float* scaleFactors, float th, MatchQuery& q)
+{
+    q.valid = 0;
+    q.u = q.v = q.radius = q.ur = q.thrR = 0.f;
+    q.minLevel = q.maxLevel = -1;
+    if (valid) {
+        float xc[3];
+        mat3_mul_add(Tcw, world, xc);
+        const float invzc = (float)(1.0 / (double)xc[2]);
+        if (!(invzc < 0)) {
+            const float u = cam.fx * xc[0] * invzc + cam.cx;
+            const float v = cam.fy * xc[1] * invzc + cam.cy;
+            if (!(u < cam.min_x || u > cam.max_x) && !(v < cam.min_y || v > cam.max_y)) {
+                const float radius = th * scaleFactors[oct];
+                q.u = u; q.v = v; q.radius = radius; q.thrR = radius;
+                q.ur = u - cam.bf * invzc;
+                if (forward) { q.minLevel = oct; q.maxLevel = -1; }
+                else if (backward) { q.minLevel = 0; q.maxLevel = oct; }
+                else { q.minLevel = oct - 1; q.maxLevel = oct + 1; }
+                q.valid = 1;
+            }
+        }
+    }
 }
 
 __global__ __launch_bounds__(256) void k_queries_last(const MatchPair* __restrict__ pairs,
@@ -170,33 +218,12 @@
     const int nLast = P.mpSlot >= 0 ? kpCount[P.lastSlot] : P.nQueries;
     if (i >= nLast) return;
     MatchQuery q;
-    q.valid = 0;
-    q.u = q.v = q.radius = q.ur = q.thrR = 0.f;
-    q.minLevel = q.maxLevel = -1;
-    q.obs = 0;
     const drfe_map_point mp = mps[(size_t)P.mpBase + i];
 #pragma unroll
     for (int k = 0; k < 8; k++) q.desc[k] = reinterpret_cast<const uint32_t*>(mp.desc)[k];
     q.obs = mp.obs_positive;
-    if (mp.valid) {
-        float xc[3];
-        mat3_mul_add(P.Tcw, mp.world, xc);
-        const float invzc = (float)(1.0 / (double)xc[2]);
-        if (!(invzc < 0)) {
-            const float u = cam.fx * xc[0] * invzc + cam.cx;
-            const float v = cam.fy * xc[1] * invzc + cam.cy;
-            if (!(u < cam.min_x || u > cam.max_x) && !(v < cam.min_y || v > cam.max_y)) {
-                const int oct = kps[(size_t)P.lastSlot * maxKp + i].octave;
-                const float radius = th * scaleFactors[oct];
-                q.u = u; q.v = v; q.radius = radius; q.thrR = radius;
-                q.ur = u - cam.bf * invzc;
-                if (P.forward) { q.minLevel = oct; q.maxLevel = -1; }
-                else if (P.backward) { q.minLevel = 0; q.maxLevel = oct; }
-                else { q.minLevel = oct - 1; q.maxLevel = oct + 1; }
-                q.valid = 1;
-            }
-        }
-    }
+    project_query(P.Tcw, P.forward, P.backward, mp.valid, mp.world, mp.valid ? kps[(size_t)P.lastSlot * maxKp + i].octave : 0, cam,
+                  scaleFactors, th, q);
     queries[(size_t)P.queryBase + i] = q;
 }
 
@@ -212,8 +239,8 @@
     return !(minX >= DRFE_GRID_COLS || maxX < 0 || minY >= DRFE_GRID_ROWS || maxY < 0);
 }
 
-__device__ __forceinline__ bool window_candidate(const MatchQuery& q, bool bCheckLevels, const uint4* __restrict__ cK,
-                                                 const uint4* __restrict__ cD, int p, int sq, uint64_t q0, uint64_t q1,
+__device__ __forceinline__ bool window_candidate(const MatchQuery& q, bool bCheckLevels, const uint4* cK,
+                                                 const uint4* cD, int p, int sq, uint64_t q0, uint64_t q1,
                                                  uint64_t q2, uint64_t q3, uint32_t& key, uint32_t& id)
 {
     const uint4 k4 = cK[p];
@@ -240,9 +267,8 @@
 }
 
 __device__ void window_query_wave(const MatchQuery& q, size_t qo, int lane, int nMinCellX, int nMaxCellX, int nMinCellY, int nMaxCellY,
-                                  const int* __restrict__ gOff, const uint4* __restrict__ cK, const uint4* __restrict__ cD,
-                                  uint32_t* __restrict__ candIdx, uint32_t* __restrict__ candKey, int* __restrict__ candCnt,
-                                  uint2* __restrict__ candBest, int* __restrict__ status)
+                                  const int* gOff, const uint4* cK, const uint4* cD, uint32_t* candIdx, uint32_t* candKey,
+                                  int* candCnt, uint2* candBest, int* status)
 {
     const bool bCheckLevels = (q.minLevel > 0) || (q.maxLevel >= 0);
     uint32_t* oIdx = candIdx + qo * DRFE_MATCH_MAX_CAND;
@@ -297,34 +323,26 @@
 #define WQ_THREADS 64
 #endif
 #define WQ_PER_BLOCK (WQ_THREADS / WAVE * 4)
-__global__ __launch_bounds__(WQ_THREADS) void k_window_candidates(const MatchPair* __restrict__ pairs,
-                                                           const MatchQuery* __restrict__ queries,
-                                                           const int* __restrict__ kpCount, int maxKp,
-                                                           const int* __restrict__ gridOff,
-                                                           const uint4* __restrict__ cellKp,
-                                                           const uint4* __restrict__ cellDesc, drfe_camera cam,
-                                                           float invW, float invH,
-                                                           uint32_t* __restrict__ candIdx,
-                                                           uint32_t* __restrict__ candKey,
-                                                           int* __restrict__ candCnt, uint2* __restrict__ candBest,
-                                                           int* __restrict__ status, uint32_t gxMagic)
-{
-    __shared__ int sTab[WQ_THREADS / WAVE][4][WQ_TAB];
-    int bx, by;
-    drfe_xcd_swizzle_2d(gxMagic, bx, by);
-    const MatchPair P = pairs[by];
-    const int wv = __builtin_amdgcn_readfirstlane((int)(threadIdx.x >> 6)), lane = threadIdx.x & 63;
+__device__ __forceinline__ MatchQuery window_load_query(const MatchQuery* queries, size_t qo, const uint32_t* qDesc, int i)
+{
+    MatchQuery q = queries[qo];
+    if (qDesc) {
+        const uint4 a = reinterpret_cast<const uint4*>(qDesc)[2 * (size_t)i], b = reinterpret_cast<const uint4*>(qDesc)[2 * (size_t)i + 1];
+        q.desc[0] = a.x; q.desc[1] = a.y; q.desc[2] = a.z; q.desc[3] = a.w;
+        q.desc[4] = b.x; q.desc[5] = b.y; q.desc[6] = b.z; q.desc[7] = b.w;
+    }
+    return q;
+}
+
+__device__ __forceinline__ void window_quartet(int qbase, int nQ, int queryBase, int lane, const MatchQuery* queries, const uint32_t* qDesc,
+                                               const int* gOff, const uint4* cK, const uint4* cD, const drfe_camera& cam,
+                                               float invW, float invH, uint32_t* candIdx, uint32_t* candKey, int* candCnt,
+                                               uint2* candBest, int* status, int (*sTab)[WQ_TAB])
+{
     const int g = lane >> 4, l = lane & 15;
-    const int qbase = (bx * (WQ_THREADS / WAVE) + wv) * 4;
-    const int nQ = P.mpSlot >= 0 ? kpCount[P.lastSlot] : P.nQueries;
-    if (qbase >= nQ) return;
-    const int cur = P.curSlot;
-    const int* gOff = gridOff + (size_t)cur * (DRFE_GRID_CELLS + 1);
-    const uint4* cK = cellKp + (size_t)cur * maxKp;
-    const uint4* cD = cellDesc + (size_t)cur * maxKp * 2;
     const bool have = qbase + g < nQ;
-    const size_t qo = (size_t)P.queryBase + (have ? qbase + g : qbase);
-    const MatchQuery q = queries[qo];
+    const size_t qo = (size_t)queryBase + (have ? qbase + g : qbase);
+    const MatchQuery q = window_load_query(queries, qo, qDesc, have ? qbase + g : qbase);
     int nMinCellX = 0, nMaxCellX = 0, nMinCellY = 0, nMaxCellY = 0;
     const bool inRange = have && q.valid && window_cells(q, cam, invW, invH, nMinCellX, nMaxCellX, nMinCellY, nMaxCellY);
     const int ncol = nMaxCellX - nMinCellX + 1;
@@ -346,7 +364,7 @@
         const int excl = incl - runN;
         const int n = small ? runN : 0;
         for (int k = 0; __any(k < n); k++)
-            if (k < n) sTab[wv][g][excl + k] = runB + k;
+            if (k < n) sTab[g][excl + k] = runB + k;
     }
     const bool bCheckLevels = (q.minLevel > 0) || (q.maxLevel >= 0);
     const uint64_t q0 = (uint64_t)q.desc[0] | ((uint64_t)q.desc[1] << 32), q1 = (uint64_t)q.desc[2] | ((uint64_t)q.desc[3] << 32),
@@ -360,7 +378,7 @@
         const int sq = s0 + l;
         bool pass = false;
         uint32_t key = 0xFFFFFFFFu, id = 0;
-        if (sq < Tg) pass = window_candidate(q, bCheckLevels, cK, cD, sTab[wv][g][sq], sq, q0, q1, q2, q3, key, id);
+        if (sq < Tg) pass = window_candidate(q, bCheckLevels, cK, cD, sTab[g][sq], sq, q0, q1, q2, q3, key, id);
         const uint32_t m16 = (uint32_t)(__ballot(pass) >> (g * 16)) & 0xFFFFu;
         const int pos = nOut + __popc(m16 & ((1u << l) - 1u));
         if (pass) {
@@ -385,46 +403,60 @@
     while (wide) {
         const int gg = (__ffsll((long long)wide) - 1) >> 4;
         wide &= wide - 1;
-        const size_t qw = (size_t)P.queryBase + qbase + gg;
-        const MatchQuery qq = queries[qw];
+        const size_t qw = (size_t)queryBase + qbase + gg;
+        const MatchQuery qq = window_load_query(queries, qw, qDesc, qbase + gg);
         int x0, x1, y0, y1;
         window_cells(qq, cam, invW, invH, x0, x1, y0, y1);
         window_query_wave(qq, qw, lane, x0, x1, y0, y1, gOff, cK, cD, candIdx, candKey, candCnt, candBest, status);
     }
 }
 
+__global__ __launch_bounds__(WQ_THREADS) void k_window_candidates(const MatchPair* __restrict__ pairs,
+                                                           const MatchQuery* __restrict__ queries,
+                                                           const int* __restrict__ kpCount, int maxKp,
+                                                           const int* __restrict__ gridOff,
+                                                           const uint4* __restrict__ cellKp,
+                                                           const uint4* __restrict__ cellDesc, drfe_camera cam,
+                                                           float invW, float invH,
+                                                           uint32_t* __restrict__ candIdx,
+                                                           uint32_t* __restrict__ candKey,
+                                                           int* __restrict__ candCnt, uint2* __restrict__ candBest,
+                                                           int* __restrict__ status, uint32_t gxMagic)
+{
+    __shared__ int sTab[WQ_THREADS / WAVE][4][WQ_TAB];
+    int bx, by;
+    drfe_xcd_swizzle_2d(gxMagic, bx, by);
+    const MatchPair P = pairs[by];
+    const int wv = __builtin_amdgcn_readfirstlane((int)(threadIdx.x >> 6)), lane = threadIdx.x & 63;
+    const int qbase = (bx * (WQ_THREADS / WAVE) + wv) * 4;
+    const int nQ = P.mpSlot >= 0 ? kpCount[P.lastSlot] : P.nQueries;
+    if (qbase >= nQ) return;
+    const int cur = P.curSlot;
+    window_quartet(qbase, nQ, P.queryBase, lane, queries, nullptr, gridOff + (size_t)cur * (DRFE_GRID_CELLS + 1),
+                   cellKp + (size_t)cur * maxKp, cellDesc + (size_t)cur * maxKp * 2, cam, invW, invH, candIdx, candKey, candCnt,
+                   candBest, status, sTab[wv]);
+}
+
 
 __device__ __forceinline__ uint32_t wave_min_u32(uint32_t v) { return drfe_wave_min_u32(v); }
 
 #define RS_THREADS 512
 #define RS_MAX_T 8
 static_assert(RS_THREADS * RS_MAX_T == DRFE_MATCH_LAST_MAX_QUERIES, "the C-ABI checks this limit before launching");
-__global__ __launch_bounds__(RS_THREADS) void k_resolve_last(const MatchPair* __restrict__ pairs,
-                                                             const MatchQuery* __restrict__ queries,
-                                                             const drfe_keypoint* __restrict__ kps,
-                                                             const int* __restrict__ kpCount, int maxKp,
-                                                             const uint32_t* __restrict__ candIdx,
-                                                             const uint32_t* __restrict__ candKey,
-                                                             const int* __restrict__ candCnt,
-                                                             const uint2* __restrict__ candBest, int checkOri,
-                                                             int* __restrict__ match ,
-                                                             const uint8_t* __restrict__ initObs,
-                                                             int* __restrict__ matchCount,
-                                                             uint16_t* __restrict__ histScratch )
-{
-    extern __shared__ int rs_smem[];
-    int* owner = rs_smem;
-    unsigned char* claim = reinterpret_cast<unsigned char*>(rs_smem + maxKp);
+__device__ __forceinline__ void resolve_last_body(int pairIdx, int curSlot, int lastSlot, int queryBase, int nQ,
+                                                  const MatchQuery* queries, const drfe_keypoint* kps, const int* kpCount, int maxKp,
+                                                  const uint32_t* candIdx, const uint32_t* candKey, const int* candCnt,
+                                                  const uint2* candBest, int checkOri, int* match, const uint8_t* initObs,
+                                                  int* matchCount, uint16_t* histScratch, int* owner, unsigned char* claim)
+{
     __shared__ int hist[30];
     __shared__ int sNm, sEnt, sInd[3], sChanged[3];
-    const MatchPair P = pairs[blockIdx.x];
     const int tid = threadIdx.x;
-    const int nQ = P.mpSlot >= 0 ? kpCount[P.lastSlot] : P.nQueries;
-    const int nCur = kpCount[P.curSlot];
-    int* M = match + (size_t)P.curSlot * maxKp;
-    const drfe_keypoint* Kc = kps + (size_t)P.curSlot * maxKp;
-    const drfe_keypoint* Kl = kps + (size_t)P.lastSlot * maxKp;
-    uint16_t* hs = histScratch + (size_t)blockIdx.x * 2 * maxKp;
+    const int nCur = kpCount[curSlot];
+    int* M = match + (size_t)curSlot * maxKp;
+    const drfe_keypoint* Kc = kps + (size_t)curSlot * maxKp;
+    const drfe_keypoint* Kl = kps + (size_t)lastSlot * maxKp;
+    uint16_t* hs = histScratch + (size_t)pairIdx * 2 * maxKp;
     for (int i = tid; i < nCur; i += RS_THREADS) {
         unsigned char c = 0;
         if (M[i] >= 0) c = 1 | ((initObs ? initObs[i] : 1) ? 2 : 0);
@@ -440,7 +472,7 @@
         const int i = tid + t * RS_THREADS;
         cnt[t] = 0; obs[t] = 0; bKey[t] = 0xFFFFFFFFu; bIdx[t] = 0; pKey[t] = 0xFFFFFFFFu; pIdx[t] = 0;
         if (i < nQ) {
-            const size_t qo = (size_t)P.queryBase + i;
+            const size_t qo = (size_t)queryBase + i;
             cnt[t] = candCnt[qo];
             if (cnt[t] > 0) { const uint2 b = candBest[qo]; bKey[t] = b.x; bIdx[t] = b.y; obs[t] = queries[qo].obs; }
         }
@@ -463,7 +495,7 @@
             const int kb = (int)(bIdx[t] & 0xFFFFFF);
             if ((claim[kb] & 3) != 3 && owner[kb] >= i) { key = bKey[t]; idx = bIdx[t]; }
             else {
-                const size_t qo = ((size_t)P.queryBase + i) * DRFE_MATCH_MAX_CAND;
+                const size_t qo = ((size_t)queryBase + i) * DRFE_MATCH_MAX_CAND;
                 for (int j0 = 0; j0 < cnt[t]; j0 += 8) {
                     const uint4 ka = *reinterpret_cast<const uint4*>(candKey + qo + j0);
                     const uint4 kb2 = *reinterpret_cast<const uint4*>(candKey + qo + j0 + 4);
@@ -530,7 +562,91 @@
         }
         __syncthreads();
     }
-    if (tid == 0) matchCount[P.curSlot] = sNm;
+    if (tid == 0) matchCount[curSlot] = sNm;
+}
+
+__global__ __launch_bounds__(RS_THREADS) void k_resolve_last(const MatchPair* __restrict__ pairs,
+                                                             const MatchQuery* __restrict__ queries,
+                                                             const drfe_keypoint* __restrict__ kps,
+                                                             const int* __restrict__ kpCount, int maxKp,
+                                                             const uint32_t* __restrict__ candIdx,
+                                                             const uint32_t* __restrict__ candKey,
+                                                             const int* __restrict__ candCnt,
+                                                             const uint2* __restrict__ candBest, int checkOri,
+                                                             int* __restrict__ match ,
+                                                             const uint8_t* __restrict__ initObs,
+                                                             int* __restrict__ matchCount,
+                                                             uint16_t* __restrict__ histScratch )
+{
+    extern __shared__ int rs_smem[];
+    const MatchPair P = pairs[blockIdx.x];
+    resolve_last_body(blockIdx.x, P.curSlot, P.lastSlot, P.queryBase, P.mpSlot >= 0 ? kpCount[P.lastSlot] : P.nQueries, queries, kps,
+                      kpCount, maxKp, candIdx, candKey, candCnt, candBest, checkOri, match, initObs, matchCount, histScratch,
+                      rs_smem ,
+                      reinterpret_cast<unsigned char*>(rs_smem + maxKp) );
+}
+
+
+static_assert(DRFE_TAIL_FUSED_THREADS == RS_THREADS, "the resolve phase is k_resolve_last's body");
+__global__ __launch_bounds__(DRFE_TAIL_FUSED_THREADS) void k_tail_fused(
+    const drfe_keypoint* __restrict__ kps, const drfe_keypoint* __restrict__ kpsUn, const int* __restrict__ kpCount, int maxKp,
+    const uint8_t* __restrict__ desc, const uint16_t* __restrict__ depth, size_t frameStride, size_t rowStride, int w, int h,
+    drfe_camera cam, float invW, float invH, float* uRight, float* zDepth, int* gridOff, int* gridIdx, uint4* cellKp, uint4* cellDesc,
+    const MatchPair* __restrict__ pairs, const float* __restrict__ Twc , const float* __restrict__ scaleFactors,
+    float th, int checkOri, MatchQuery* queries, uint32_t* candIdx, uint32_t* candKey, int* candCnt, uint2* candBest, int* match,
+    int* matchCount, uint16_t* histScratch, int* status)
+{
+    constexpr int NT = DRFE_TAIL_FUSED_THREADS;
+    extern __shared__ int tf_smem[];
+    const int k = blockIdx.x, tid = threadIdx.x;
+    const int n = kpCount[k];
+    for (int i = tid; i < n; i += NT) stereo_keypoint(kps, kpsUn, maxKp, k, i, depth, frameStride, rowStride, w, h, cam, uRight, zDepth);
+    __syncthreads();
+    int* gOff = gridOff + (size_t)k * (DRFE_GRID_CELLS + 1);
+    uint4* cK = cellKp + (size_t)k * maxKp;
+    uint4* cD = cellDesc + (size_t)k * maxKp * 2;
+    {
+        int* cnt = tf_smem;
+        int* off = cnt + DRFE_GRID_CELLS;
+        int* wtot = off + DRFE_GRID_CELLS + 4;
+        uint16_t* list = reinterpret_cast<uint16_t*>(wtot + NT / WAVE);
+        int16_t* cellOf = reinterpret_cast<int16_t*>(list + maxKp);
+        grid_body<NT, true, uint16_t>(kpsUn + (size_t)k * maxKp, n, cam, invW, invH, uRight + (size_t)k * maxKp,
+                                      reinterpret_cast<const uint4*>(desc + (size_t)k * maxKp * 32), gOff, gridIdx + (size_t)k * maxKp, cK, cD,
+                                      cnt, off, wtot, list, cellOf);
+    }
+    for (int i = tid; i < maxKp; i += NT) match[(size_t)k * maxKp + i] = -1;
+    if (tid == 0) matchCount[k] = 0;
+    if (k == 0) return;
+    const MatchPair P = pairs[k - 1];
+    const int last = P.lastSlot;
+    const int nLast = kpCount[last];
+    for (int i = tid; i < nLast; i += NT) {
+        const size_t o = (size_t)last * maxKp + i;
+        const float z = stereo_depth(kps[o], last, i, depth, frameStride, rowStride, w, h, cam);
+        const drfe_keypoint kpU = kpsUn[o];
+        const int valid = z > 0 ? 1 : 0;
+        float world[3] = {0.f, 0.f, 0.f};
+        if (valid) unproject_last(kpU, z, cam, Twc + (size_t)last * 16, world);
+        MatchQuery q;
+        project_query(P.Tcw, P.forward, P.backward, valid, world, kpU.octave, cam, scaleFactors, th, q);
+        MatchQuery* qp = queries + (size_t)P.queryBase + i;
+        qp->u = q.u; qp->v = q.v; qp->radius = q.radius; qp->ur = q.ur; qp->thrR = q.thrR;
+        qp->minLevel = q.minLevel; qp->maxLevel = q.maxLevel; qp->valid = q.valid;
+        qp->obs = 1;
+    }
+    __syncthreads();
+    {
+        int (*sTab)[4][WQ_TAB] = reinterpret_cast<int (*)[4][WQ_TAB]>(tf_smem);
+        const int wv = __builtin_amdgcn_readfirstlane(tid >> 6), lane = tid & 63;
+        const uint32_t* qDesc = reinterpret_cast<const uint32_t*>(desc + (size_t)last * maxKp * 32);
+        for (int qbase = wv * 4; qbase < nLast; qbase += NT / WAVE * 4)
+            window_quartet(qbase, nLast, P.queryBase, lane, queries, qDesc, gOff, cK, cD, cam, invW, invH, candIdx, candKey, candCnt,
+                           candBest, status, sTab[wv]);
+    }
+    __syncthreads();
+    resolve_last_body(k - 1, P.curSlot, last, P.queryBase, nLast, queries, kpsUn, kpCount, maxKp, candIdx, candKey, candCnt, candBest,
+                      checkOri, match, nullptr, matchCount, histScratch, tf_smem, reinterpret_cast<unsigned char*>(tf_smem + maxKp));
 }
 
 __global__ __launch_bounds__(WAVE) void k_resolve_map(const MatchPair* __restrict__ pairs,
@@ -773,6 +889,29 @@
 {
     hipLaunchKernelGGL(k_mappoints_last, dim3((c->maxKp + 255) / 256, nframes), dim3(256), 0, s, drfe_kps_un(c), c->d_desc,
                        c->d_kpCount, c->maxKp, c->d_depth, cam, d_Twc, mb.d_mps);
+    return hipGetLastError();
+}
+
+hipError_t drfe_launch_tail_fused(drfe_ctx* c, const MatchBuffers& mb, const uint16_t* d_depth, size_t frameStride, size_t rowStride,
+                                  const drfe_camera& cam, float th, int checkOri, int nframes, hipStream_t s)
+{
+    const size_t lds = drfe_tail_fused_lds(c->maxKp);
+    if (!lds) return hipErrorInvalidValue;
+    const float invW = (float)DRFE_GRID_COLS / (float)(cam.max_x - cam.min_x);
+    const float invH = (float)DRFE_GRID_ROWS / (float)(cam.max_y - cam.min_y);
+    prof_begin(c, DRFE_STAGE_GLUE, s);
+    if (c->dist.enabled)
+        hipLaunchKernelGGL(k_undistort, dim3((c->maxKp + 255) / 256, nframes), dim3(256), 0, s, c->d_kps, c->d_kpCount,
+                           c->maxKp, c->dist, c->d_kpsUn);
+    (void)drfe_launch_fill_i32(c->d_status + 2, 1, 0, s);
+    prof_end(c, DRFE_STAGE_GLUE, s);
+    prof_begin(c, DRFE_STAGE_MATCH, s);
+    hipLaunchKernelGGL(k_tail_fused, dim3(nframes), dim3(DRFE_TAIL_FUSED_THREADS), lds, s, c->d_kps, drfe_kps_un(c), c->d_kpCount,
+                       c->maxKp, c->d_desc, d_depth, frameStride, rowStride, c->geom.imgW, c->geom.imgH, cam, invW, invH, c->d_uRight,
+                       c->d_depth, c->d_gridOff, c->d_gridIdx, c->d_cellKp, c->d_cellDesc, mb.d_pairs, c->d_poses, mb.d_scale, th,
+                       checkOri, mb.d_queries, mb.d_candIdx, mb.d_candKey, mb.d_candCnt, mb.d_candBest, c->d_match, c->d_matchCount,
+                       mb.d_hist, c->d_status + 2);
+    prof_end(c, DRFE_STAGE_MATCH, s);
     return hipGetLastError();
 }
 
diff --git a/dr_slam_amd/lib.py b/dr_slam_amd/lib.py
--- a/dr_slam_amd/lib.py
+++ b/dr_slam_amd/lib.py
@@ -30,7 +30,7 @@
     "drfe_search_by_bow", "drfe_search_by_bow_kf", "drfe_search_for_triangulation", "drfe_lsd_extract", "drfe_lsd_extract_batch", "drfe_lsd_stages", "drfe_lines_is_good", "drfe_lsd_search_by_descriptor", "drfe_lsd_search_for_triangulation", "drfe_lsd_search_by_projection_last",
     "drfe_lsd_search_by_projection_map", "drfe_plane_voxel_grid", "drfe_plane_refit", "drfe_planes_ahc_postprocess",
     "drfe_planes_cape_postprocess", "drfe_surface_normals", "drfe_surface_normals_batch", "drfe_surface_normals_download", "drfe_batch_download_async", "drfe_orb_fast_partition", "drfe_lsd_segments_host", "drfe_orb_keypoint_pixels_async", "drfe_gather_keypoint_depth",
-    "drfe_frame_stereo_grid_batch_kpdepth", "drfe_planes_ahc_post_batch", "drfe_planes_ahc_from_blocks", "drfe_debug_ahc_trials", "drfe_debug_order_sort", "drfe_search_for_initialization", "drfe_lsd_fuse_search_sim3", "drfe_lsd_search_by_projection_kf",
+    "drfe_frame_stereo_grid_batch_kpdepth", "drfe_planes_ahc_post_batch", "drfe_planes_ahc_from_blocks", "drfe_debug_ahc_trials", "drfe_debug_order_sort", "drfe_debug_tail_fused_lds_bytes", "drfe_debug_tail_fused_batch", "drfe_search_for_initialization", "drfe_lsd_fuse_search_sim3", "drfe_lsd_search_by_projection_kf",
     "drfe_lsd_search_by_sim3", "drfe_frame_submit", "drfe_frame_collect", "drfe_pipeline_create", "drfe_pipeline_destroy",
     "drfe_pipeline_depth", "drfe_pipeline_context", "drfe_pipeline_last_error", "drfe_pipeline_submit", "drfe_pipeline_sync",
     "drfe_lsd_configure", "drfe_lsd_configure_rect", "drfe_shard_unique_id", "drfe_shard_create", "drfe_shard_destroy", "drfe_shard_broadcast", "drfe_shard_reduce_report", "drfe_shard_sequences_of_rank", "drfe_shard_last_error", "drfe_planes_configure_cape", "drfe_planes_cape_stats", "drfe_lsd_configure_nfa", "drfe_lsd_stats", "drfe_lsd_segments_host_mode", "drfe_debug_cr_sincos", "drfe_debug_device_order_sort", "drfe_debug_device_order_sort_depth", "drfe_batch_status_async", "drfe_batch_check", "drfe_frame_submit_tracked", "drfe_frame_collect_tracked", "drfe_planes_cape_batch", "drfe_planes_configure", "drfe_planes_configure_extractor", "drfe_planes_ahc_stats", "drfe_planes_configure_refit", "drfe_planes_refit_stats", "drfe_frame_load", "drfe_bow_transform_slot", "drfe_long_kernel_clock", "drfe_long_kernel_ms",
@@ -354,6 +354,8 @@
     L.drfe_planes_ahc_post_batch.argtypes = [vp, vp, sz, i32, i32, sz, i32, vp, f32, f32, f64, vp, i32, vp, vp, vp, vp, vp, i32]
     L.drfe_debug_ahc_trials.argtypes = [vp, vp, i32, i32, vp]
     L.drfe_debug_order_sort.argtypes = [vp, sz, i32, i32, i32, C.c_uint32]
+    L.drfe_debug_tail_fused_lds_bytes.argtypes = [i32]
+    L.drfe_debug_tail_fused_batch.argtypes = [vp, vp, sz, sz, vp, vp, C.POINTER(Camera), f32, i32, i32, i32]
     L.drfe_planes_ahc_from_blocks.argtypes = [vp, vp, vp, i32, i32, sz, vp, f32, vp, i32, C.POINTER(i32), vp, vp, vp]
     L.drfe_planes_cape_postprocess.argtypes = [vp, vp, i32, i32, sz, vp, vp, vp, i32, f32, f64, vp, vp, vp, i32,
                                                C.POINTER(i32), C.POINTER(i32)]
diff --git a/include/drfe_debug.h b/include/drfe_debug.h
--- a/include/drfe_debug.h
+++ b/include/drfe_debug.h
@@ -35,6 +35,9 @@
 int drfe_debug_pose_opt_ldlt(const double* A, const double* b, double* x, int32_t* positive);
 int drfe_debug_pose_opt_plane_error(int kind, const float* meas, const float* world, const float* Tcw, double* e);
 int drfe_debug_pose_opt_hand_back(drfe_ctx* ctx, int every);
+int drfe_debug_tail_fused_lds_bytes(int max_keypoints);
+int drfe_debug_tail_fused_batch(drfe_ctx* ctx, const uint16_t* d_depth, size_t frame_stride, size_t row_stride, const float* Tcw,
+                                const float* Twc, const drfe_camera* cam, float th, int mono, int check_ori, int nframes);
 
 #ifdef __cplusplus
 }
```

Result: no change. 281,100 frames/s, median of 2 (-0.2%).
